# antonilo/unsupervised_detection

Measured on AMD Instinct MI355X. Metric: frame-pairs/sec per adversarial step, DAVIS 480p batch4, 1/2/4/8 GPU, higher is better.
Workload: dtype f32

## Files before the change

### include/udet.h

```cpp
#ifndef UDET_H
#define UDET_H
#include <stddef.h>
#ifdef __cplusplus
extern "C" {
#endif

#define UDET_OK 0
#define UDET_ERR_SHAPE (-1)
#define UDET_ERR_ALIGN (-2)
#define UDET_ERR_HIP (-3)
#define UDET_ERR_UNSUPPORTED (-4)
#define UDET_ERR_ARG (-5)
#define UDET_ERR_OVERFLOW (-6)

#define UDET_ACT_NONE 0
#define UDET_ACT_LEAKY 1
#define UDET_ACT_ELU 2

int udet_version(void);
const char* udet_last_error(void);


int udet_warp(const float* image, const float* flow, float flow_scale, float* out, int n, int h, int w, int c,
              void* stream);
// ... 108 lines not shown
                        int radius, float* q, void* workspace, size_t workspace_bytes, void* stream);

size_t udet_post_propagate_workspace_bytes(int total_frames, int n_seq);
int udet_post_propagate_sequences(const float* masks, const float* flow_prev, const float* flow_next, int n_seq, const int* seq_first,
                                  const int* seq_len, int total_frames, int h, int w, float w_s, float w_r, float* avg_f, float* avg_b,
                                  void* workspace, size_t workspace_bytes, void* stream);
int udet_post_select_unary(const float* pred, const float* avg_f, const float* avg_b, const float* gt, int n, int hw, int* choice,
                           double* scores, float* soft, float* unary, void* stream);

#define UDET_SOFT_SCORE_GEOM 16
size_t udet_post_soft_score_workspace_bytes(int n, int ns, int nc, int h, int w);
int udet_post_soft_score_batch(const float* masks, int n, int ns, int nc, int h, int w, const int* geom, const int* coef, double san_t,
                               double* pred_mask, void* workspace, size_t workspace_bytes, void* stream);

#define UDET_HISTOGRAM_BUCKETS 1551
size_t udet_flow_to_image_workspace_bytes(int n);
int udet_flow_to_image(const float* flow, const float* mask, const double* stats8, float threshold, int n, int h, int w,
                       unsigned char* rgb, void* workspace, size_t workspace_bytes, void* stream);
int udet_overlay_mask(const float* image, const float* mask, const double* stats8, float threshold, int n, int h, int w,
                      unsigned char* out, int oh, int ow, void* stream);
int udet_histogram_limits(double* limits, int n);
size_t udet_grad_histogram_workspace_bytes(int nseg);
int udet_grad_histogram(const float* g, const long long* seg_offsets, int nseg, double* stats, unsigned* counts, void* workspace,
                        size_t workspace_bytes, void* stream);

#define UDET_OVERLAY_MAX_EDGE 8
int udet_overlay_native_ragged(const unsigned char* image_rgb, const unsigned char* mask, int n, const long long* offsets,
                               const int* hw, int max_h, int max_w, size_t total_pixels, float alpha, float beta,
                               unsigned mask_rgb, int edge, unsigned edge_rgb, unsigned char* out_rgb, void* stream);

size_t udet_conv2d_workspace_bytes(int n, int h, int w, int cin, int cout, int kh, int kw, int upsample2x);
int udet_conv2d(const float* x, const float* w_hwio, const float* bias, float* y, int n, int h, int w, int cin, int cout,
                int kh, int kw, int stride, int dilation, int upsample2x, int act, float alpha, void* workspace,
                size_t workspace_bytes, void* stream);
int udet_conv2d_backward_data(const float* dy, const float* y_saved, const float* w_hwio, float* dx, int n, int h, int w,
                              int cin, int cout, int kh, int kw, int stride, int dilation, int act, float alpha,
                              void* workspace, size_t workspace_bytes, void* stream);
int udet_conv2d_backward_filter(const float* x, const float* dy, const float* y_saved, float* dw_hwio, float* dbias, int n,
                                int h, int w, int cin, int cout, int kh, int kw, int stride, int dilation, int upsample2x,
                                int act, float alpha, void* workspace, size_t workspace_bytes, void* stream);
int udet_conv2d_transpose4x4s2(const float* x, const float* w_hwoi, const float* bias, float* y, int n, int h, int w,
                               int cin, int cout, void* workspace, size_t workspace_bytes, void* stream);


size_t udet_stage_workspace_bytes(int n);
int udet_flow_normalize(const float* flow, float* out, int n, int h, int w, void* workspace, size_t workspace_bytes, void* stream);
int udet_charbonnier_loss(const float* gt_flows, const float* pred_flows, const float* masks, int mask_channels, int n, int h, int w,
                          float cbn, float* out, void* workspace, size_t workspace_bytes, void* stream);
int udet_losses_forward(const float* flow, const float* mask, const float* pred3, int b, int h, int w, float cbn, float epsilon,
                        float* losses8, float* coef, void* workspace, size_t workspace_bytes, void* stream);
int udet_losses_backward(const float* flow, const float* mask, const float* pred3, const float* coef, int which, int b, int h, int w,
                         float cbn, float* dpred, float* dmask, void* stream);
int udet_clip_or_noise(float* g, size_t n, float clip, const float* flag2, unsigned long long seed, long step, void* stream);
int udet_adam_step(float* w, const float* g, float* m, float* v, size_t n, float lr, float beta1, float beta2, float eps, long t,
                   void* stream);

typedef struct udet_plan udet_plan;
typedef struct {
  int batch;
  int in_h, in_w;
  int img_h, img_w;
  float flow_normalizer;
  float cbn;
  float epsilon;
  float lr, beta1, beta2, adam_eps;
  float clip;
  unsigned long long noise_seed;
  int conv_fp16;
} udet_config;

int udet_plan_create(const udet_config* cfg, udet_plan** out);
void udet_plan_destroy(udet_plan* plan);
size_t udet_workspace_bytes(const udet_plan* plan);
int udet_plan_init(udet_plan* plan, void* workspace, void* stream);

int udet_param_count(int net);
size_t udet_param_total(int net);
int udet_param_info(int net, int index, const char** name, int* rank, int* shape4, size_t* offset_floats);
int udet_buffer_count(const udet_plan* plan);
int udet_buffer_info(const udet_plan* plan, int index, const char** name, size_t* offset_bytes, int* dims_nhw_ld);

int udet_pack_pwc(udet_plan* plan, const float* w_pwc, void* workspace, void* stream);
int udet_pack_trainable(udet_plan* plan, const float* w_gen, const float* w_rec, void* workspace, void* stream);

int udet_pwc_forward(udet_plan* plan, const float* img1, const float* img2, void* workspace, void* stream);
int udet_forward(udet_plan* plan, const float* img1, const float* img2, int ncalls, void* workspace, void* stream);
int udet_prefetch_flow(udet_plan* plan, const float* img1, const float* img2, void* workspace, void* stream);
int udet_forward_prefetched(udet_plan* plan, int ncalls, void* workspace, void* stream);
int udet_prefetch_consume(udet_plan* plan, void* workspace, void* stream);
int udet_forward_from_flow(udet_plan* plan, int ncalls, void* workspace, void* stream);
int udet_generator_forward(udet_plan* plan, void* workspace, void* stream);
int udet_generator_layers(udet_plan* plan, void* workspace, void* stream);
int udet_recover_forward(udet_plan* plan, int n, void* workspace, void* stream);
int udet_backward(udet_plan* plan, int which, const float* w_gen, const float* w_rec, float* g_gen, float* g_rec,
                  void* workspace, void* stream);
int udet_stream_wait_grads(udet_plan* plan, int net, void* stream);
int udet_generator_backward(udet_plan* plan, const float* w_gen, float* g_gen, void* workspace, void* stream);
int udet_recover_backward(udet_plan* plan, const float* w_rec, float* g_rec, void* workspace, void* stream);
int udet_grad_absmean(udet_plan* plan, int net, const float* g, float* out2, void* workspace, void* stream);
int udet_apply(udet_plan* plan, int net, float* w, float* g, float* m, float* v, void* workspace, void* stream);
long udet_fp16_overflow_count(udet_plan* plan);
long udet_get_adam_step(const udet_plan* plan);
void udet_set_adam_step(udet_plan* plan, long t);
int udet_train_step(udet_plan* plan, int which, const float* img1, const float* img2, float* w_gen, float* w_rec,
                    float* g_gen, float* g_rec, float* m_gen, float* v_gen, float* m_rec, float* v_rec, void* workspace,
                    void* stream);

int udet_autotune(udet_plan* plan, const float* w_gen, const float* w_rec, float* g_gen, float* g_rec, void* workspace,
                  void* stream);
int udet_tuned_shapes(void);
int udet_tune_save(const char* path);
int udet_tune_load(const char* path);
int udet_tune_rejected(void);
int udet_profile_begin(udet_plan* plan);
int udet_profile_end(udet_plan* plan, double* out, int ncat, void* stream);

int udet_plan_set_concurrent(udet_plan* plan, int on);

int udet_plan_lane_queues(udet_plan* plan, void* stream, int* queue);
int udet_plan_pin_lanes(udet_plan* plan, void* stream, void* const* side_streams, int n);

#define UDET_INSTANCE_WRAP 252
#define UDET_INSTANCE_UNASSIGNED 255
size_t udet_track_instance_maps_workspace_bytes(size_t total_pixels, int n, int k);
int udet_track_instance_maps_ragged(const int* labels, int n, const long long* offsets, const int* hw, int max_h, int max_w,
                                    size_t total_pixels, const long long* dets, const long long* counts, int k, const int* ids,
                                    const unsigned char* gt, unsigned char* map, long long* row_gt, long long* frame_stats,
                                    void* workspace, size_t workspace_bytes, void* stream);

int udet_overlay_instances_ragged(const unsigned char* image_rgb, const unsigned char* map, int n, const long long* offsets, const int* hw,
                                  int max_h, int max_w, size_t total_pixels, float alpha, float beta, const unsigned* palette,
                                  int palette_size, unsigned other_rgb, int edge, unsigned char* out_rgb, void* stream);

size_t udet_follow_tracks_workspace_bytes(size_t total_pixels, int n, int k);
int udet_follow_tracks_ragged(const int* labels, int n, const long long* offsets, const int* hw, int max_h, int max_w,
                              long long total_pixels, const long long* dets, const long long* counts, int k,
                              const unsigned long long* keep, const unsigned char* gt, unsigned char* selected, long long* stats,
                              void* workspace, size_t workspace_bytes, void* stream);

#define UDET_MAX_OBJECTS 32
size_t udet_track_object_overlaps_workspace_bytes(size_t total_pixels, int n, int k);
int udet_track_object_overlaps_ragged(const int* labels, int n, const long long* offsets, const int* hw, int max_h, int max_w,
                                      size_t total_pixels, const long long* dets, const long long* counts, int k,
                                      const unsigned char* objects, int num_objects, long long* row_obj, long long* obj_area,
                                      long long* frame_stats, void* workspace, size_t workspace_bytes, void* stream);

#ifdef __cplusplus
}
#endif
#endif
```

### include/udet_debug.h

```cpp
#ifndef UDET_DEBUG_H
#define UDET_DEBUG_H
#include <stddef.h>
#ifdef __cplusplus
extern "C" {
#endif
void udet_debug_force_conv(int bm, int bn, int ks);
void udet_debug_conv_fp16(int on);
void udet_debug_conv_fp16_grad_scale(float s);
void udet_debug_force_wgrad(int nsplit, int dma);
int udet_debug_last_wgrad(void);
int udet_debug_last_wgrad_reduce(void);
int udet_debug_conv2d_backward_filter_ex(const float* x, int ldx, int x_coff, const float* dy, int ldy, int y_coff, const float* y_saved, int act,
                                         float alpha, const float* w, const float* b, const float* gamma, float bn_c, float* dw, float* db,
                                         float* dgamma, float* dbeta, int n, int h, int wd, int cin, int cout, int k, int stride, int dilation,
                                         int up, void* workspace, size_t workspace_bytes, void* stream);
void udet_debug_upb_min_pixels(long v);
void udet_debug_set_tuning(int on);
void udet_debug_force_pair(int on);
int udet_debug_last_pair(void);
int udet_debug_conv2d_pair(const float* xa, const float* xb, const float* wa, const float* wb, const float* ba, const float* bb, float* ya, float* yb,
                           int na, int nb, int h, int w, int cin, int cout, int k, int stride, int dilation, int act, float alpha, void* workspace,
                           size_t workspace_bytes, void* stream);
#define UDET_DEBUG_UPCONV_WSETS_OFFSET 6400
size_t udet_debug_upconv_lowres_workspace_bytes(int ldx, int cin, int cout);
int udet_debug_upconv_lowres_fwd(const float* x, int ldx, const float* w, const float* bias, int act, float alpha, float* y, int ldy, int y_coff,
                                 float* xhat, int n, int h, int wd, int cin, int cout, int split, void* workspace, size_t workspace_bytes,
                                 void* stream);
int udet_debug_upconv_lowres_bwd(const float* dy, int ldy, int y_coff, const float* w, float* dx, int ldx, float* dxhat, int n, int h, int wd,
                                 int cin, int cout, void* workspace, size_t workspace_bytes, void* stream);
int udet_debug_upconv_tables(int h, int w, int backward, int* nseg, int* seg, int* seg_tap, int* taps, int taps_cap, int* ntaps);
int udet_debug_max_segs(void);
int udet_debug_launch_resize_bilinear_fwd(const float* x, int ldx, int x_coff, int n, int h, int w, float* y, int ldy, int y_coff, int oh, int ow,
                                          int c, float mul, float div, void* stream);
int udet_debug_launch_resize_bilinear_bwd(const float* dy, int ldy, int y_coff, int n, int oh, int ow, float* dx, int ldx, int x_coff, int h, int w,
                                          int c, int accumulate, void* stream);
int udet_debug_launch_share_samples(float* buf, long p, int ld, int coff, int c, int copies, void* stream);
int udet_debug_launch_fold_samples(float* buf, long p, int ld, int coff, int c, int copies, void* stream);
int udet_debug_launch_emit_du(const float* d, const float* a, float* u, long p, int ld, int coff, int c, int act, float alpha, void* stream);
int udet_debug_launch_pack_pwc_input(const float* i1, const float* i2, float* x8, long p, void* stream);
size_t udet_debug_gen_input_workspace_bytes(int b);
int udet_debug_launch_gen_input(const float* img, const float* f, float* gin, int b, long hw, void* workspace, size_t workspace_bytes, void* stream);
int udet_debug_launch_mask_rec_inputs(const float* logits, const float* f, float* mask, float* fin, long p, int ncalls, void* stream);
int udet_debug_launch_pack_imgin(const float* img, float* imgin, long p, int ncalls, void* stream);
int udet_debug_launch_mask_bwd(const float* dmask, const float* dfin, const float* f, const float* mask, float* dlogits, long p, void* stream);
typedef struct udet_debug_conv_ex {
  int form;
  int n, h, wd, cin, cout, k, stride, dilation, up;
  int kc, k_split, k_gap;
  const float* x;
  int ldx, x_coff;
  const float* xa;
  int xact;
  float xalpha;
  const float* w;
  const float* bias;
  int act;
  float alpha;
  float* y;
  int ldy, y_coff;
  const float* res;
  int ldres, res_coff;
  float* y2;
  int ldy2, y2_coff;
  int accumulate;
  float* uo;
  int ldu, u_coff;
  const float* ua;
  int ldua, ua_coff, uact;
  float ualpha;
  int u_c0, u_c1;
  int pack_job;
} udet_debug_conv_ex;
size_t udet_debug_conv2d_ex_workspace_bytes(const udet_debug_conv_ex* args);
int udet_debug_conv2d_ex(const udet_debug_conv_ex* args, void* workspace, size_t workspace_bytes, void* stream);
size_t udet_debug_conv2d_pair_ex_workspace_bytes(const udet_debug_conv_ex* a, const udet_debug_conv_ex* b);
int udet_debug_conv2d_pair_ex(const udet_debug_conv_ex* a, const udet_debug_conv_ex* b, void* workspace, size_t workspace_bytes, void* stream);
int udet_debug_last_conv(void);
#ifdef __cplusplus
}
#endif
#endif
```

### unsupervised_detection_amd/_devel.py

```python
from __future__ import annotations

import ctypes
import os

from ._ffi import check as _check, lib as _lib

_PATH = os.path.join(os.path.dirname(os.path.abspath(__file__)), "libudet_debug.so")
if not os.path.exists(_PATH):
    raise RuntimeError(f"{_PATH} is missing: build it with `make -C unsupervised_detection_amd/csrc`")
dbg = ctypes.CDLL(_PATH, mode=ctypes.RTLD_GLOBAL)
dbg.udet_debug_force_conv.restype = None
dbg.udet_debug_force_conv.argtypes = [ctypes.c_int, ctypes.c_int, ctypes.c_int]
dbg.udet_debug_last_conv.restype = ctypes.c_int
dbg.udet_debug_last_conv.argtypes = []
dbg.udet_debug_conv_fp16.restype = None
dbg.udet_debug_conv_fp16.argtypes = [ctypes.c_int]
dbg.udet_debug_conv_fp16_grad_scale.restype = None
dbg.udet_debug_conv_fp16_grad_scale.argtypes = [ctypes.c_float]
dbg.udet_debug_force_wgrad.restype = None
dbg.udet_debug_force_wgrad.argtypes = [ctypes.c_int, ctypes.c_int]
dbg.udet_debug_upb_min_pixels.restype = None
dbg.udet_debug_upb_min_pixels.argtypes = [ctypes.c_long]
dbg.udet_debug_set_tuning.restype = None
dbg.udet_debug_set_tuning.argtypes = [ctypes.c_int]
dbg.udet_debug_last_wgrad.restype = ctypes.c_int
dbg.udet_debug_last_wgrad.argtypes = []
dbg.udet_debug_force_pair.restype = None
dbg.udet_debug_force_pair.argtypes = [ctypes.c_int]
dbg.udet_debug_last_pair.restype = ctypes.c_int
dbg.udet_debug_last_pair.argtypes = []
dbg.udet_debug_conv2d_pair.restype = ctypes.c_int
dbg.udet_debug_conv2d_pair.argtypes = [ctypes.c_void_p] * 8 + [ctypes.c_int] * 10 + [ctypes.c_float, ctypes.c_void_p, ctypes.c_size_t, ctypes.c_void_p]
dbg.udet_debug_last_wgrad_reduce.restype = ctypes.c_int
dbg.udet_debug_last_wgrad_reduce.argtypes = []
_p, _i, _f = ctypes.c_void_p, ctypes.c_int, ctypes.c_float
dbg.udet_debug_conv2d_backward_filter_ex.restype = ctypes.c_int
dbg.udet_debug_conv2d_backward_filter_ex.argtypes = ([_p, _i, _i, _p, _i, _i, _p, _i, _f, _p, _p, _p, _f, _p, _p, _p, _p] + [_i] * 9
                                                     + [_p, ctypes.c_size_t, _p])
UPCONV_WSETS_OFFSET = 6400
dbg.udet_debug_upconv_lowres_workspace_bytes.restype = ctypes.c_size_t
dbg.udet_debug_upconv_lowres_workspace_bytes.argtypes = [_i, _i, _i]
dbg.udet_debug_upconv_lowres_fwd.restype = ctypes.c_int
dbg.udet_debug_upconv_lowres_fwd.argtypes = [_p, _i, _p, _p, _i, _f, _p, _i, _i, _p] + [_i] * 6 + [_p, ctypes.c_size_t, _p]
dbg.udet_debug_upconv_lowres_bwd.restype = ctypes.c_int
dbg.udet_debug_upconv_lowres_bwd.argtypes = [_p, _i, _i, _p, _p, _i, _p] + [_i] * 5 + [_p, ctypes.c_size_t, _p]
dbg.udet_debug_upconv_tables.restype = ctypes.c_int
dbg.udet_debug_upconv_tables.argtypes = [_i, _i, _i] + [_p] * 4 + [_i, _p]
dbg.udet_debug_max_segs.restype = ctypes.c_int
dbg.udet_debug_max_segs.argtypes = []
_l = ctypes.c_long
for _name, _args in (("resize_bilinear_fwd", [_p, _i, _i, _i, _i, _i, _p, _i, _i, _i, _i, _i, _f, _f, _p]),
                     ("resize_bilinear_bwd", [_p, _i, _i, _i, _i, _i, _p, _i, _i, _i, _i, _i, _i, _p]),
                     ("share_samples", [_p, _l, _i, _i, _i, _i, _p]),
                     ("fold_samples", [_p, _l, _i, _i, _i, _i, _p]),
                     ("emit_du", [_p, _p, _p, _l, _i, _i, _i, _i, _f, _p]),
                     ("pack_pwc_input", [_p, _p, _p, _l, _p]),
                     ("gen_input", [_p, _p, _p, _i, _l, _p, ctypes.c_size_t, _p]),
                     ("mask_rec_inputs", [_p, _p, _p, _p, _l, _i, _p]),
                     ("pack_imgin", [_p, _p, _l, _i, _p]),
                     ("mask_bwd", [_p, _p, _p, _p, _p, _l, _p])):
    _fn = getattr(dbg, "udet_debug_launch_" + _name)
    _fn.restype = ctypes.c_int
    _fn.argtypes = _args
dbg.udet_debug_gen_input_workspace_bytes.restype = ctypes.c_size_t
dbg.udet_debug_gen_input_workspace_bytes.argtypes = [_i]


class ConvEx(ctypes.Structure):
    _fields_ = ([("form", _i)] + [(k, _i) for k in ("n", "h", "wd", "cin", "cout", "k", "stride", "dilation", "up", "kc", "k_split", "k_gap")]
                + [("x", _p), ("ldx", _i), ("x_coff", _i), ("xa", _p), ("xact", _i), ("xalpha", _f), ("w", _p), ("bias", _p), ("act", _i),
                   ("alpha", _f), ("y", _p), ("ldy", _i), ("y_coff", _i), ("res", _p), ("ldres", _i), ("res_coff", _i), ("y2", _p),
                   ("ldy2", _i), ("y2_coff", _i), ("accumulate", _i), ("uo", _p), ("ldu", _i), ("u_coff", _i), ("ua", _p), ("ldua", _i),
                   ("ua_coff", _i), ("uact", _i), ("ualpha", _f), ("u_c0", _i), ("u_c1", _i), ("pack_job", _i)])


dbg.udet_debug_conv2d_ex_workspace_bytes.restype = ctypes.c_size_t
dbg.udet_debug_conv2d_ex_workspace_bytes.argtypes = [ctypes.POINTER(ConvEx)]
dbg.udet_debug_conv2d_ex.restype = ctypes.c_int
dbg.udet_debug_conv2d_ex.argtypes = [ctypes.POINTER(ConvEx), _p, ctypes.c_size_t, _p]


dbg.udet_debug_conv2d_pair_ex_workspace_bytes.restype = ctypes.c_size_t
dbg.udet_debug_conv2d_pair_ex_workspace_bytes.argtypes = [ctypes.POINTER(ConvEx), ctypes.POINTER(ConvEx)]
dbg.udet_debug_conv2d_pair_ex.restype = ctypes.c_int
dbg.udet_debug_conv2d_pair_ex.argtypes = [ctypes.POINTER(ConvEx), ctypes.POINTER(ConvEx), _p, ctypes.c_size_t, _p]


def _workspace_and_stream(workspace, stream):
    if workspace is None or isinstance(workspace, tuple):
        ptr, nbytes = workspace or (None, 0)
    else:
        ptr, nbytes = workspace.data_ptr(), workspace.numel() * workspace.element_size()
    if stream is None:
        import torch
        stream = torch.cuda.current_stream().cuda_stream if torch.cuda.is_available() else None
    return ptr, nbytes, stream


def conv2d_pair_ex(a_fields, b_fields, workspace=None, stream=None):
    a, b = (None if f is None else ctypes.byref(conv_ex_args(**f)) for f in (a_fields, b_fields))
    _check(dbg.udet_debug_conv2d_pair_ex(a, b, *_workspace_and_stream(workspace, stream)))


def conv2d_pair_ex_workspace_bytes(a_fields, b_fields) -> int:
    a, b = (None if f is None else ctypes.byref(conv_ex_args(**f)) for f in (a_fields, b_fields))
    return int(dbg.udet_debug_conv2d_pair_ex_workspace_bytes(a, b))


def conv2d_ex(workspace=None, stream=None, **fields):
    a = conv_ex_args(**fields)
    _check(dbg.udet_debug_conv2d_ex(ctypes.byref(a), *_workspace_and_stream(workspace, stream)))


def conv_ex_args(**fields) -> ConvEx:
    a = ConvEx()
    for k, v in fields.items():
        if isinstance(v, tuple):
            v = v[0].data_ptr() + v[1] * v[0].element_size()
        elif hasattr(v, "data_ptr"):
            v = v.data_ptr()
        setattr(a, k, v)
    return a


def conv2d_ex_workspace_bytes(**fields) -> int:
    return int(dbg.udet_debug_conv2d_ex_workspace_bytes(ctypes.byref(conv_ex_args(**fields))))


def launch(name: str, *args):
    import torch
    raw = [a.data_ptr() if isinstance(a, torch.Tensor) else a for a in args]
    _check(getattr(dbg, "udet_debug_launch_" + name)(*raw, torch.cuda.current_stream().cuda_stream))


def upconv_tables(h: int, w: int, backward: bool):
    cap = 1024
    nseg, ntaps = ctypes.c_int(0), ctypes.c_int(0)
    seg, seg_tap, taps = (ctypes.c_int * 64)(), (ctypes.c_int * 17)(), (ctypes.c_int * (3 * cap))()
    st = dbg.udet_debug_upconv_tables(h, w, 1 if backward else 0, ctypes.addressof(nseg), ctypes.addressof(seg), ctypes.addressof(seg_tap),
                                      ctypes.addressof(taps), cap, ctypes.addressof(ntaps))
    _check(st)
    ns, nt = nseg.value, ntaps.value
    return dict(nseg=ns, seg=[tuple(seg[4 * s:4 * s + 4]) for s in range(ns)], seg_tap=list(seg_tap[:ns + 1]),
                taps=[tuple(taps[3 * t:3 * t + 3]) for t in range(nt)])
```

### unsupervised_detection_amd/csrc/api_plan.hip

```cpp
#include <stdlib.h>
#include <string.h>

#include "conv_host.h"
#include "elementwise.h"
#include "plan.h"

using namespace udet;

struct udet_plan {
  Plan* p;
};

extern "C" {

int udet_plan_create(const udet_config* c, udet_plan** out) {
  if (!c || !out) { set_error("plan_create: null argument"); return UDET_ERR_ARG; }
  Config k;
  k.batch = c->batch; k.in_h = c->in_h; k.in_w = c->in_w; k.img_h = c->img_h; k.img_w = c->img_w;
  k.flow_normalizer = c->flow_normalizer; k.cbn = c->cbn; k.epsilon = c->epsilon;
  k.lr = c->lr; k.beta1 = c->beta1; k.beta2 = c->beta2; k.adam_eps = c->adam_eps; k.clip = c->clip;
  k.noise_seed = c->noise_seed;
  k.conv_fp16 = c->conv_fp16 ? 1 : 0;
  Plan* P = plan_build(k);
  if (!P) return UDET_ERR_SHAPE;
  *out = new udet_plan{P};
  return UDET_OK;
}
void udet_plan_destroy(udet_plan* h) {
  if (h) { delete h->p; delete h; }
}
size_t udet_workspace_bytes(const udet_plan* h) { return h->p->arena_floats * sizeof(float); }
int udet_plan_init(udet_plan* h, void* ws, void* stream) { return plan_init_workspace(h->p, (float*)ws, (hipStream_t)stream); }

int udet_param_count(int net) { return (net < 0 || net > 2) ? 0 : (int)net_params(net).p.size(); }
size_t udet_param_total(int net) { return (net < 0 || net > 2) ? 0 : net_params(net).total; }
int udet_param_info(int net, int i, const char** name, int* rank, int* shape, size_t* offset) {
  if (net < 0 || net > 2 || i < 0 || i >= (int)net_params(net).p.size()) { set_error("param_info: out of range"); return UDET_ERR_ARG; }
  const ParamDesc& d = net_params(net).p[i];
  *name = d.name.c_str(); *rank = d.rank; *offset = d.offset;
  for (int k = 0; k < 4; ++k) shape[k] = d.shape[k];
  return UDET_OK;
}
int udet_buffer_count(const udet_plan* h) { return (int)h->p->bufs.size(); }
int udet_buffer_info(const udet_plan* h, int i, const char** name, size_t* offset_bytes, int* dims) {
  if (i < 0 || i >= (int)h->p->bufs.size()) { set_error("buffer_info: out of range"); return UDET_ERR_ARG; }
  const Buf& b = h->p->bufs[i];
  *name = b.name.c_str(); *offset_bytes = b.off * sizeof(float);
  dims[0] = b.n; dims[1] = b.h; dims[2] = b.w; dims[3] = b.ld;
  return UDET_OK;
}
int udet_plan_set_concurrent(udet_plan* h, int on) {
  if (!h) { set_error("plan_set_concurrent: null plan"); return UDET_ERR_ARG; }
  if (on)
    if (h->p->cand.empty()) { set_error("plan_set_concurrent: the plan has no side streams"); return UDET_ERR_UNSUPPORTED; }
  h->p->concurrent = on != 0;
  return UDET_OK;
}
int udet_plan_lane_queues(udet_plan* h, void* stream, int* queue) {
  if (!h || !queue) { set_error("plan_lane_queues: null argument"); return UDET_ERR_ARG; }
  return plan_lane_queues(h->p, (hipStream_t)stream, queue);
}
int udet_plan_pin_lanes(udet_plan* h, void* stream, void* const* side_streams, int n) {
  if (!h || (n > 0 && !side_streams)) { set_error("plan_pin_lanes: null argument"); return UDET_ERR_ARG; }
  return plan_pin_lanes(h->p, (hipStream_t)stream, reinterpret_cast<hipStream_t const*>(side_streams), n);
}
long udet_fp16_overflow_count(udet_plan* h) {
  if (!h) return 0;
  (void)plan_check_overflow(h->p, true);
  return h->p->ovf_skipped;
}
long udet_get_adam_step(const udet_plan* h) {
  plan_settle_adam_step(h->p);
  return h->p->adam_t;
}
void udet_set_adam_step(udet_plan* h, long t) {
  plan_settle_adam_step(h->p);
  h->p->adam_t = t;
}

int udet_pack_pwc(udet_plan* h, const float* w_pwc, void* ws, void* stream) {
  return plan_pack_pwc(h->p, w_pwc, (float*)ws, (hipStream_t)stream);
}
int udet_pack_trainable(udet_plan* h, const float* w_gen, const float* w_rec, void* ws, void* stream) {
  return plan_pack_trainable(h->p, w_gen, w_rec, (float*)ws, (hipStream_t)stream);
}
int udet_pwc_forward(udet_plan* h, const float* img1, const float* img2, void* ws, void* stream) {
  return plan_pwc_forward(h->p, img1, img2, (float*)ws, (hipStream_t)stream);
}
int udet_forward_from_flow(udet_plan* h, int ncalls, void* ws, void* stream) {
  UDET_TRY(plan_check_overflow(h->p, false));
  if (ncalls < 0 || ncalls > 3) { set_error("forward: ncalls must be 0..3"); return UDET_ERR_ARG; }
  return plan_forward(h->p, nullptr, nullptr, ncalls, (float*)ws, (hipStream_t)stream);
}
int udet_generator_forward(udet_plan* h, void* ws, void* stream) {
  UDET_TRY(plan_generator_forward(h->p, (float*)ws, (hipStream_t)stream));
  return plan_recover_forward(h->p, 0, (float*)ws, (hipStream_t)stream);
}
int udet_generator_layers(udet_plan* h, void* ws, void* stream) {
  h->p->ev_next = 0;
  UDET_TRY(plan_generator_layers(h->p, (float*)ws, (hipStream_t)stream));
  return plan_recover_forward(h->p, 0, (float*)ws, (hipStream_t)stream);
}
int udet_recover_forward(udet_plan* h, int n, void* ws, void* stream) {
  if (n < 1 || n > 3) { set_error("recover_forward: n must be 1..3 (multiples of the plan batch)"); return UDET_ERR_ARG; }
  return plan_recover_forward(h->p, n, (float*)ws, (hipStream_t)stream, true);
}
int udet_forward(udet_plan* h, const float* img1, const float* img2, int ncalls, void* ws, void* stream) {
  UDET_TRY(plan_check_overflow(h->p, false));
  if (ncalls < 0 || ncalls > 3) { set_error("forward: ncalls must be 0..3"); return UDET_ERR_ARG; }
  if (!img1 || !img2) { set_error("forward: null image pointer"); return UDET_ERR_ARG; }
  return plan_forward(h->p, img1, img2, ncalls, (float*)ws, (hipStream_t)stream);
}
int udet_prefetch_flow(udet_plan* h, const float* img1, const float* img2, void* ws, void* stream) {
  if (!img1 || !img2) { set_error("prefetch_flow: null image pointer"); return UDET_ERR_ARG; }
  return plan_prefetch(h->p, img1, img2, (float*)ws, (hipStream_t)stream);
}
int udet_prefetch_consume(udet_plan* h, void* ws, void* stream) {
  return plan_prefetch_consume(h->p, (float*)ws, (hipStream_t)stream);
}
int udet_forward_prefetched(udet_plan* h, int ncalls, void* ws, void* stream) {
  UDET_TRY(plan_check_overflow(h->p, false));
  if (ncalls < 0 || ncalls > 3) { set_error("forward: ncalls must be 0..3"); return UDET_ERR_ARG; }
  return plan_forward(h->p, nullptr, nullptr, ncalls, (float*)ws, (hipStream_t)stream, true);
}
int udet_backward(udet_plan* h, int which, const float* w_gen, const float* w_rec, float* g_gen, float* g_rec, void* ws,
                  void* stream) {
  UDET_TRY(plan_check_overflow(h->p, false));
  if (which < 1 || which > 3) { set_error("backward: which must be 1 (generator), 2 (recover) or 3 (both)"); return UDET_ERR_ARG; }
  return plan_backward(h->p, which, w_gen, w_rec, g_gen, g_rec, (float*)ws, (hipStream_t)stream);
}
int udet_apply(udet_plan* h, int net, float* w, float* g, float* m, float* v, void* ws, void* stream) {
  return plan_apply(h->p, net, w, g, m, v, (float*)ws, (hipStream_t)stream);
}
int udet_train_step(udet_plan* h, int which, const float* img1, const float* img2, float* w_gen, float* w_rec, float* g_gen,
                    float* g_rec, float* m_gen, float* v_gen, float* m_rec, float* v_rec, void* ws, void* stream) {
  UDET_TRY(udet_pack_trainable(h, w_gen, w_rec, ws, stream));
  UDET_TRY(udet_forward(h, img1, img2, 3, ws, stream));
  UDET_TRY(udet_backward(h, which, w_gen, w_rec, g_gen, g_rec, ws, stream));
  if (which & 1) UDET_TRY(udet_apply(h, NET_GEN, w_gen, g_gen, m_gen, v_gen, ws, stream));
  if (which & 2) UDET_TRY(udet_apply(h, NET_REC, w_rec, g_rec, m_rec, v_rec, ws, stream));
  return UDET_OK;
}

int udet_autotune(udet_plan* h, const float* w_gen, const float* w_rec, float* g_gen, float* g_rec, void* ws_, void* stream) {
  Plan* P = h->p;
  float* ws = (float*)ws_;
  hipStream_t s = (hipStream_t)stream;
  if (!P->pwc_packed) { set_error("autotune: pack the PWC-Net and trainable weights first"); return UDET_ERR_ARG; }
  const size_t lo = P->packed_floats, hi = P->small_off;
  UDET_TRY(launch_fill_uniform(ws + lo, (long)(hi - lo), 0x5eedull, -0.5f, 0.5f, s));
  const size_t img_floats = (size_t)P->cfg.batch * P->cfg.in_h * P->cfg.in_w * 3;
  if (P->wgrad_floats < 2 * img_floats) { set_error("autotune: workspace too small for the probe images"); return UDET_ERR_ARG; }
  const float* img1 = ws + P->wgrad_off[0];
  const float* img2 = img1 + img_floats;
  const bool was_concurrent = P->concurrent;
  P->concurrent = false;
  conv_set_tuning(1);
  wgrad_set_tuning(1);
  int rc = udet_forward(h, img1, img2, 3, ws_, stream);
  if (rc == UDET_OK) rc = udet_backward(h, 3, w_gen, w_rec, g_gen, g_rec, ws_, stream);
  conv_set_tuning(0);
  wgrad_set_tuning(0);
  P->concurrent = was_concurrent;
  UDET_HIP(hipMemsetAsync(ws + lo, 0, (hi - lo) * sizeof(float), s));
  UDET_HIP(hipStreamSynchronize(s));
  return rc;
}
int udet_tuned_shapes(void) { return tuned_shapes(); }
int udet_tune_save(const char* path) {
  FILE* f = path ? fopen(path, "w") : nullptr;
  if (!f) { set_error("tune_save: cannot open %s", path ? path : "(null)"); return UDET_ERR_ARG; }
  fprintf(f, "udet-tune 2 abi %d\n", UDET_TUNE_ABI);
  tune_dump(f);
  fclose(f);
  return UDET_OK;
}
int udet_tune_load(const char* path) {
  FILE* f = path ? fopen(path, "r") : nullptr;
  if (!f) { set_error("tune_load: cannot open %s", path ? path : "(null)"); return UDET_ERR_ARG; }
  char line[256];
  int n = 0, ver = 0, abi = -1;
  if (!fgets(line, sizeof(line), f) || sscanf(line, "udet-tune %d abi %d", &ver, &abi) != 2 || ver != 2 || abi != UDET_TUNE_ABI) {
    fclose(f);
    set_error("tune_load: %s is not a udet-tune 2 file of this build (abi %d)", path, UDET_TUNE_ABI);
    return UDET_ERR_ARG;
  }
  while (fgets(line, sizeof(line), f)) n += tune_put_line(line) ? 1 : 0;
  fclose(f);
  return n;
}

int udet_profile_begin(udet_plan* h) {
  for (auto* r : h->p->prof) delete r;
  h->p->prof.clear();
  h->p->profiling = true;
  return UDET_OK;
}
int udet_profile_end(udet_plan* h, double* out, int ncat, void* stream) {
  Plan* P = h->p;
  P->profiling = false;
  g_launch_sink = nullptr;
  UDET_HIP(hipStreamSynchronize((hipStream_t)stream));
  for (int i = 0; i < ncat * 5; ++i) out[i] = 0.0;
  FILE* dump = nullptr;
  if (const char* path = getenv("UDET_PROF_DUMP")) dump = fopen(path, "a");
  for (auto* r : P->prof) {
    float wall = 0.f;
    (void)hipEventElapsedTime(&wall, r->a, r->b);
    double kern = 0.0;
    std::string each;
    for (int k = 0; k < r->sink.n; ++k) {
      float ms = 0.f;
      if (hipEventElapsedTime(&ms, r->kev[2 * k], r->kev[2 * k + 1]) == hipSuccess) kern += ms;
      char buf[32];
      snprintf(buf, sizeof(buf), "%s%.1f", k ? "+" : "", ms * 1e3f);
      each += buf;
      (void)hipEventDestroy(r->kev[2 * k]);
      (void)hipEventDestroy(r->kev[2 * k + 1]);
    }
    if (r->sink.n == 0) kern = wall;
    if (dump)
      fprintf(dump, "%d,%s,%.4f,%.4f,%.4f,%.4f,%d,%s,%.4f\n", r->cat, r->name.c_str(), kern, r->flops * 1e-9, r->bytes * 1e-6, wall, r->sink.n,
              each.c_str(), r->flops * r->mfma_scale * 1e-9);
    if (r->cat < ncat) {
      out[r->cat * 5 + 0] += 1.0;
      out[r->cat * 5 + 1] += kern;
      out[r->cat * 5 + 2] += r->flops;
      out[r->cat * 5 + 3] += r->bytes;
      out[r->cat * 5 + 4] += wall;
    }
    (void)hipEventDestroy(r->a);
    (void)hipEventDestroy(r->b);
    delete r;
  }
  if (dump) fclose(dump);
  P->prof.clear();
  return UDET_OK;
}

int udet_generator_backward(udet_plan* h, const float* w_gen, float* g_gen, void* ws, void* stream) {
  if (!w_gen || !g_gen) { set_error("generator_backward: null argument"); return UDET_ERR_ARG; }
  return plan_backward(h->p, 1, w_gen, nullptr, g_gen, nullptr, (float*)ws, (hipStream_t)stream);
}
int udet_recover_backward(udet_plan* h, const float* w_rec, float* g_rec, void* ws, void* stream) {
  if (!w_rec || !g_rec) { set_error("recover_backward: null argument"); return UDET_ERR_ARG; }
  return plan_backward(h->p, 2, nullptr, w_rec, nullptr, g_rec, (float*)ws, (hipStream_t)stream);
}
int udet_grad_absmean(udet_plan* h, int net, const float* g, float* out2, void* ws_, void* stream) {
  if ((net != NET_GEN && net != NET_REC) || !g || !out2) { set_error("grad_absmean: net must be 1 or 2, g / out2 non-null"); return UDET_ERR_ARG; }
  Plan* P = h->p;
  float* ws = (float*)ws_;
  const NetParams& np = net_params(net);
  const long* tab = reinterpret_cast<const long*>(ws + P->seg_off[net]);
  return launch_grad_absmean(g, tab, tab + np.p.size(), (int)np.p.size(), ws + P->small_off + 2048, 1e-5f, out2, (hipStream_t)stream);
}
int udet_stream_wait_grads(udet_plan* h, int net, void* stream) {
  if (net != NET_GEN && net != NET_REC) { set_error("stream_wait_grads: net must be 1 or 2"); return UDET_ERR_ARG; }
  if (!h->p->grad_ev[net]) { set_error("stream_wait_grads: no udet_backward has produced that gradient yet"); return UDET_ERR_ARG; }
  UDET_HIP(hipStreamWaitEvent((hipStream_t)stream, h->p->grad_ev[net], 0));
  return UDET_OK;
}
int udet_tune_rejected(void) { return conv_tune_rejected(); }

}
```

### unsupervised_detection_amd/csrc/common.h

```cpp
#pragma once
#include <hip/hip_runtime.h>
#include <hip/hip_ext.h>
#include <stdint.h>
#include <stdio.h>
#include <string>

#include "../../include/udet.h"

namespace udet {

void set_error(const char* fmt, ...);
int hip_fail(hipError_t e, const char* what);
#define UDET_HIP(x)                                   \
  do {                                                \
    hipError_t _e = (x);                              \
    if (_e != hipSuccess) return udet::hip_fail(_e, #x); \
  } while (0)
#define UDET_TRY(x)            \
  do {                         \
    int _s = (x);              \
    if (_s != 0) return _s;    \
  } while (0)

struct LaunchSink {
// ... 60 lines not shown
  for (int b = 0; b < nwg; ++b) {
    const int l = xcd_tile_order(b, nwg);
    if (l < 0 || l >= nwg || ((seen >> l) & 1)) return false;
    seen |= 1ull << l;
  }
  return true;
}
static_assert(xcd_tile_order_permutes(1) && xcd_tile_order_permutes(7) && xcd_tile_order_permutes(8), "xcd_tile_order");
static_assert(xcd_tile_order_permutes(9) && xcd_tile_order_permutes(13) && xcd_tile_order_permutes(64), "xcd_tile_order");
static_assert(xcd_tile_order(1, 13) == 2 && xcd_tile_order(8, 13) == 1 && xcd_tile_order(5, 13) == 10, "xcd 0..4 of 13 hold two tiles, 5..7 one");

struct ConvSeg {
  int oy, ox;
  int h, w;
  int prow0;
  FastDiv fd_hw, fd_w;
};
#define UDET_MAX_SEGS 16

struct ConvParams {
  const float* x;
  int ldx, x_coff;
  int N, H, W;
  int up_shift;
  const float* xa;
  int xact;
  float xalpha;
  const float* wp;
  int Kc, ldw;
  const float* bias;
  float* y;
  int ldy, y_coff, Cout;
  int OH, OW;
  int OHq, OWq;
  int osy, osx, ooy, oox;
  int isy, isx;
  int ntaps;
  ConvTap taps[UDET_MAX_TAPS];
  int ncls;
  int cls_tap[5];
  int nseg;
  ConvSeg seg[UDET_MAX_SEGS];
  int seg_tap[UDET_MAX_SEGS + 1];
  const ConvTap* tap_tab;
  int Mall;
  FastDiv fd_ohw, fd_ow;
  int kfast;
  const float* zero16;
  int act;
  float alpha;
  const float* res;
  int ldres, res_coff;
  float* y2;
  int ldy2, y2_coff;
  int accumulate;
  float* uo;
  int ldu, u_coff;
  const float* ua;
  int ldua, ua_coff, uact;
  float ualpha;
  int u_c0, u_c1;
  int ksplit;
  float* partial;
  size_t partial_cap;
  int ldp;
  int fold;
  int* tickets;
  int tail_full, tail_ks, tail_prow0;
  int f16;
  float f16_xscale;
  const float* wino_u;
  int wino_np;
  int kreal;
};
#define UDET_MAX_TICKETS 4096

int launch_conv(ConvParams& p, hipStream_t stream);
int launch_conv_pair(ConvParams& a, ConvParams& b, hipStream_t stream);
int launch_tap_gather(const ConvParams& g, const float* z, int ldz, hipStream_t stream);

struct PackJob {
  long src_off, dst_off, gamma_off, beta_off;
  long total;
  int T, R, C, Kc, ldw, k_split, k_gap, mode;
};

struct WgradParams {
  const float* x;
  int ldx, x_coff;
  int N, H, W, up_shift;
  int Cin;
  const float* dy;
  const float* ya;
  int ldy, y_coff, Cout;
  int yact;
  float yalpha;
  int OH, OW, isy, isx;
  int ycls, OHf, OWf;
  int ntaps;
  ConvTap taps[UDET_MAX_TAPS];
  float* dw;
  float* db;
  float* partial;
  size_t partial_floats;
  const float* zero16;
  int swapped, oCin, oCout, bias_m;
  int Cin4, Mpad;
  float* pbias;
  FastDiv fd_ohw, fd_ow;
  const float* w;
  const float* b;
  const float* gamma;
  float* dgamma;
  float* dbeta;
  float bn_c;
  int f16;
  float f16_yscale;
};
int launch_wgrad_T(WgradParams& p, int T, hipStream_t stream);
int launch_wgrad_up_T(const WgradParams& q, int H, int W, hipStream_t stream);
int launch_bn_finalize(float* dw, int T, int Cin, int Cout, const float* w, const float* b, const float* gamma, float bn_c, float* pd,
                       float* db, float* dgamma, float* dbeta, hipStream_t stream);
int launch_wgrad_up_combine(const float* deff, float* dw, int Cin, int Cout, hipStream_t stream);
size_t wgrad_partial_floats_needed(int T, int Cin, int Cout);

}
```

### unsupervised_detection_amd/csrc/conv_host.h

```cpp
#pragma once
#include "common.h"
namespace udet {
void same_pad(int in, int k, int s, int d, int* before, int* out);
void conv_setup_fwd(ConvParams& p, int N, int H, int W, int kh, int kw, int s, int d);
int conv_dgrad_classes(int s, int H, int W);
void conv_force_config(int bm, int bn, int ks);
bool conv_thin_n_ok(const ConvParams& p);
bool conv_thin_k_ok(const ConvParams& p);
int launch_conv_thin_n(const ConvParams& p, hipStream_t stream);
int launch_conv_thin_k(const ConvParams& p, hipStream_t stream);
bool conv_wino_geometry(const ConvParams& p, int* dil, int widx_at[9]);
bool conv_wino_ok(const ConvParams& p);
bool conv_wino_variant_ok(const ConvParams& p, int variant);
int conv_wino_np(int cout);
size_t conv_wino_floats(int Kc, int cout);
long conv_wino_workgroups(const ConvParams& p, int variant);
int conv_wino_max_ksplit(const ConvParams& p, int variant);
int launch_conv_wino(ConvParams& p, int variant, int ks, hipStream_t stream);
int launch_splitk_second_pass(const ConvParams& p, hipStream_t stream);
int launch_wino_pack(const float* src, float* dst, int R, int C, int Kc, int np, int k_split, int k_gap, int transposed, hipStream_t stream);
int launch_wino_from_packed(const ConvParams& p, float* dst, int np, hipStream_t stream);
void conv_debug_f16(int on);
int conv_debug_f16_on();
void conv_debug_f16_grad_scale(float s);
float conv_debug_f16_grad_scale_now();
int conv_last_config();
void conv_set_tuning(int on);
int tuned_shapes();
void tune_dump(FILE* f);
bool tune_put_line(const char* line);
int conv_tune_rejected();
void wgrad_set_tuning(int on);
bool wgrad_wino_ok(const WgradParams& p);
int wgrad_wino_slices(const WgradParams& p, int wanted);
int launch_wgrad_wino(const WgradParams& q, int slices, int ldn, hipStream_t stream);
int wgrad_last_config();
enum { WGRAD_RED_FUSED_BN = 1 << 26, WGRAD_RED_SEPARATE_BN = 1 << 27, WGRAD_RED_SWAPPED = 1 << 28, WGRAD_RED_CLASSES = 1 << 29 };
int wgrad_last_reduce();
void setup_up_fwd(ConvParams& p, int N, int H, int W);
void setup_up_dgrad(ConvParams& p, int N, int H, int W);
void wgrad_force(int nsplit, int dma);
void conv_force_pair(int on);
int conv_last_pair();
#define UDET_TUNE_ABI 6
bool conv_setup_dgrad(ConvParams& p, int cls, int N, int H, int W, int kh, int kw, int s, int d);
int launch_pack_weights(const float* src, float* dst, int T, int R, int C, int Kc, int ldw, int k_split, int k_gap,
                        int mode, const float* scale, hipStream_t stream);
int launch_pack_taps_into_n(const float* src, float* dst, int T, int R, int C, int Kc, int ldz, int k_split, int k_gap,
                            int transposed, hipStream_t stream);
int launch_pack_jobs(const PackJob* jobs_dev, int njobs, const float* wsrc, float* ws, float bn_c, hipStream_t stream);
int launch_fold_bn(const float* b, const float* gamma, const float* beta, float c, float* scale, float* bias_f, int n,
                   hipStream_t stream);
int launch_copy_channels(const float* src, int lds, int s_coff, float* dst, int ldd, int d_coff, long P, int C, float mul,
                         float add, hipStream_t stream);
int launch_warp(const float* img, const float* flow, int ldf, int f_coff, float flow_scale, float* out, int N, int H,
                int W, int C, int* dbg_idx, float* dbg_alpha, hipStream_t stream);
int launch_cost_volume(const float* c1, const float* wr, float* out, int ldo, int o_coff, int N, int H, int W, int C,
                       hipStream_t stream);
int launch_warp_cost_volume(const float* c1, const float* c2, const float* flow, int ldf, int f_coff, float flow_scale, float* out,
                            int ldo, int corr_coff, int c1_coff, float* warped_dbg, int N, int H, int W, int C, hipStream_t stream);
inline int round_up(int v, int m) { return (v + m - 1) / m * m; }
}
```

### unsupervised_detection_amd/csrc/conv_host.hip

```cpp
#include <string.h>

#include <stdint.h>

#include "common.h"
#include "conv_host.h"
#include "wino_pack.h"

namespace udet {

void same_pad(int in, int k, int s, int d, int* before, int* out) {
  const int o = (in + s - 1) / s;
  int total = (o - 1) * s + (k - 1) * d + 1 - in;
  if (total < 0) total = 0;
  *before = total / 2;
  *out = o;
}

static inline int floordiv2(int v) { return v >= 0 ? v / 2 : -((-v + 1) / 2); }

static void push_tap(ConvParams& p, int dy, int dx, int widx) {
  const int ymax = (p.OHq - 1) * p.isy + dy, xmax = (p.OWq - 1) * p.isx + dx;
  if (dy >= p.H || ymax < 0 || dx >= p.W || xmax < 0) return;
  p.taps[p.ntaps].dy = dy;
  p.taps[p.ntaps].dx = dx;
  p.taps[p.ntaps].widx = widx;
  ++p.ntaps;
}

void conv_setup_fwd(ConvParams& p, int N, int H, int W, int kh, int kw, int s, int d) {
  int pt, pl, oh, ow;
  same_pad(H, kh, s, d, &pt, &oh);
  same_pad(W, kw, s, d, &pl, &ow);
  p.N = N; p.H = H; p.W = W;
  p.OH = oh; p.OW = ow; p.OHq = oh; p.OWq = ow;
  p.osy = p.osx = 1; p.ooy = p.oox = 0;
  p.isy = p.isx = s;
  p.ntaps = 0;
  for (int ky = 0; ky < kh; ++ky)
    for (int kx = 0; kx < kw; ++kx) push_tap(p, ky * d - pt, kx * d - pl, ky * kw + kx);
}

int conv_dgrad_classes(int s, int H, int W) { return s == 1 ? 1 : ((H % 2 == 0 && W % 2 == 0) ? 1 : s * s); }

bool conv_setup_dgrad(ConvParams& p, int cls, int N, int H, int W, int kh, int kw, int s, int d) {
  int pt, pl, ohf, owf;
  same_pad(H, kh, s, d, &pt, &ohf);
  same_pad(W, kw, s, d, &pl, &owf);
  p.N = N; p.H = ohf; p.W = owf;
  p.OH = H; p.OW = W;
  p.isy = p.isx = 1;
  p.ntaps = 0;
  p.ncls = 1;
  if (s == 1) {
    p.OHq = H; p.OWq = W; p.osy = p.osx = 1; p.ooy = p.oox = 0;
    for (int ky = 0; ky < kh; ++ky)
      for (int kx = 0; kx < kw; ++kx) push_tap(p, pt - ky * d, pl - kx * d, ky * kw + kx);
    return p.ntaps > 0;
  }
  const bool merged = (H % 2 == 0 && W % 2 == 0);
  p.osy = p.osx = s;
  const int c_lo = merged ? 0 : cls, c_hi = merged ? 4 : cls + 1;
  for (int c = c_lo; c < c_hi; ++c) {
    const int py = c / s, px = c % s;
    p.ooy = py; p.oox = px;
    p.OHq = (H - py + s - 1) / s;
    p.OWq = (W - px + s - 1) / s;
    if (merged) p.cls_tap[c] = p.ntaps;
    if (p.OHq <= 0 || p.OWq <= 0) {
      if (!merged) return false;
      continue;
    }
    for (int ky = 0; ky < kh; ++ky) {
      const int vy = py + pt - ky * d;
      if (((vy % 2) + 2) % 2) continue;
      for (int kx = 0; kx < kw; ++kx) {
        const int vx = px + pl - kx * d;
        if (((vx % 2) + 2) % 2) continue;
        push_tap(p, floordiv2(vy), floordiv2(vx), ky * kw + kx);
      }
    }
  }
  if (merged) {
    p.ncls = 4;
    p.cls_tap[4] = p.ntaps;
    p.ooy = p.oox = 0;
    p.OHq = H / 2; p.OWq = W / 2;
  }
  return true;
}

__global__ __launch_bounds__(256) void pack_weights_kernel(const float* __restrict__ src, float* __restrict__ dst, int T,
                                                           int R, int C, int Kc, int ldw, int k_split, int k_gap,
                                                           int mode, const float* __restrict__ scale) {
  const long total = (long)T * Kc * ldw;
  for (long e = (long)blockIdx.x * 256 + threadIdx.x; e < total; e += (long)gridDim.x * 256) {
    const int n = (int)(e % ldw);
    const int k = (int)((e / ldw) % Kc);
    const int t = (int)(e / ((long)ldw * Kc));
    float v = 0.f;
    int ks = k;
    if (k >= k_split) ks = (k < k_split + k_gap) ? -1 : k - k_gap;
    const int r = mode == 0 ? ks : n, c = mode == 0 ? n : ks;
    if (r >= 0 && r < R && c >= 0 && c < C) {
      v = src[((long)t * R + r) * C + c];
      if (scale) v *= scale[c];
    }
    dst[e] = v;
  }
}

int launch_pack_weights(const float* src, float* dst, int T, int R, int C, int Kc, int ldw, int k_split, int k_gap,
                        int mode, const float* scale, hipStream_t stream) {
  const long total = (long)T * Kc * ldw;
  int nb = (int)((total + 255) / 256);
  if (nb > 2048) nb = 2048;
  UDET_LAUNCH(pack_weights_kernel, dim3(nb), dim3(256), 0, stream, src, dst, T, R, C, Kc, ldw, k_split, k_gap,
                     mode, scale);
  UDET_HIP(hipGetLastError());
  return UDET_OK;
}

__constant__ float UPB_MERGE[2][3][3][4] = {
    {{{.5f, 0.f, 0.f, 0.f}, {.5f, 1.f, .5f, 0.f}, {0.f, 0.f, .5f, 1.f}},
     {{.5f, 0.f, 0.f, 0.f}, {.5f, 1.f, 1.f, 0.f}, {0.f, 0.f, 0.f, 0.f}},
     {{0.f, 0.f, 0.f, 0.f}, {0.f, 0.f, .5f, 0.f}, {0.f, 0.f, -.5f, -1.f}}},
    {{{1.f, .5f, 0.f, 0.f}, {0.f, .5f, 1.f, .5f}, {0.f, 0.f, 0.f, .5f}},
     {{1.f, 1.f, 0.f, 0.f}, {0.f, 0.f, 0.f, 0.f}, {0.f, 0.f, 0.f, 0.f}},
     {{0.f, .5f, 0.f, 0.f}, {0.f, -.5f, -1.f, -.5f}, {0.f, 0.f, 0.f, -.5f}}}};

__global__ __launch_bounds__(256) void pack_jobs_kernel(const PackJob* __restrict__ jobs, const float* __restrict__ wsrc,
                                                        float* __restrict__ ws, float bn_c) {
  const PackJob j = jobs[blockIdx.y];
  const float* src = wsrc + j.src_off;
  float* dst = ws + j.dst_off;
  const float* gamma = j.gamma_off >= 0 ? wsrc + j.gamma_off : nullptr;
  if (j.mode == 2) {
    for (long e = (long)blockIdx.x * 256 + threadIdx.x; e < j.total; e += (long)gridDim.x * 256)
      dst[e] = gamma ? src[e] * (gamma[e] * bn_c) + wsrc[j.beta_off + e] : src[e];
    return;
  }
  if (j.mode == 9 || j.mode == 10) {
    const int rv = (int)(j.beta_off / 3), cv = (int)(j.beta_off % 3);
    for (long e = (long)blockIdx.x * 256 + threadIdx.x; e < j.total; e += (long)gridDim.x * 256) {
      const int n = (int)(e % j.ldw), k = (int)(e / j.ldw);
      int ks = k;
      if (k >= j.k_split) ks = (k < j.k_split + j.k_gap) ? -1 : k - j.k_gap;
      const int ci = j.mode == 9 ? ks : n, co = j.mode == 9 ? n : ks;
      const bool real = ci >= 0 && ci < j.R && co >= 0 && co < j.C;
      float w[4][4];
#pragma unroll
      for (int kk = 0; kk < 4; ++kk)
#pragma unroll
        for (int ll = 0; ll < 4; ++ll) w[kk][ll] = real ? src[((long)(kk * 4 + ll) * j.R + ci) * j.C + co] : 0.f;
      const long plane = (long)j.Kc * j.ldw;
#pragma unroll
      for (int py = 0; py < 2; ++py) {
        float t1[3][4];
#pragma unroll
        for (int a = 0; a < 3; ++a)
#pragma unroll
          for (int ll = 0; ll < 4; ++ll) {
            float v = 0.f;
#pragma unroll
            for (int kk = 0; kk < 4; ++kk) v += UPB_MERGE[py][rv][a][kk] * w[kk][ll];
            t1[a][ll] = v;
          }
#pragma unroll
        for (int px = 0; px < 2; ++px)
#pragma unroll
          for (int a = 0; a < 3; ++a)
#pragma unroll
            for (int bb = 0; bb < 3; ++bb) {
              float v = 0.f;
#pragma unroll
              for (int ll = 0; ll < 4; ++ll) v += UPB_MERGE[px][cv][bb][ll] * t1[a][ll];
              dst[(long)((py * 2 + px) * 9 + a * 3 + bb) * plane + e] = v;
            }
      }
    }
    return;
  }
  if (j.mode == 7 || j.mode == 8) {
    for (long e = (long)blockIdx.x * 256 + threadIdx.x; e < j.total; e += (long)gridDim.x * 256) wino_pack_item(j, src, gamma, bn_c, dst, e);
    return;
  }
  for (long e = (long)blockIdx.x * 256 + threadIdx.x; e < j.total; e += (long)gridDim.x * 256) {
    const int n = (int)(e % j.ldw);
    const int k = (int)((e / j.ldw) % j.Kc);
    int t = (int)(e / ((long)j.ldw * j.Kc));
    float v = 0.f;
    int ks = k;
    if (k >= j.k_split) ks = (k < j.k_split + j.k_gap) ? -1 : k - j.k_gap;
    int r = j.mode == 0 ? ks : n, c = j.mode == 0 ? n : ks;
    if (j.mode == 3 || j.mode == 4) {
      t = n / j.C;
      c = n - t * j.C;
      r = ks;
      if (t >= j.T) r = -1;
    }
    if (j.mode >= 5) {
      const int cls = t >> 2, ty = (t >> 1) & 1, tx = t & 1, py = cls >> 1, px = cls & 1;
      const int y0 = py == 0 ? (ty == 0 ? 0 : 1) : (ty == 0 ? 0 : 2), y1 = py == 0 ? (ty == 0 ? 0 : 2) : (ty == 0 ? 1 : 2);
      const int x0 = px == 0 ? (tx == 0 ? 0 : 1) : (tx == 0 ? 0 : 2), x1 = px == 0 ? (tx == 0 ? 0 : 2) : (tx == 0 ? 1 : 2);
      const int ci = j.mode == 5 ? ks : n, co = j.mode == 5 ? n : ks;
      if (ci >= 0 && ci < j.R && co >= 0 && co < j.C) {
        for (int ky = y0; ky <= y1; ++ky)
          for (int kx = x0; kx <= x1; ++kx) v += src[((long)(ky * 3 + kx) * j.R + ci) * j.C + co];
        if (gamma) v *= gamma[co] * bn_c;
      }
      dst[e] = v;
      continue;
    }
    if (r >= 0 && r < j.R && c >= 0 && c < j.C) {
      v = j.mode == 4 ? src[((long)t * j.C + c) * j.R + r] : src[((long)t * j.R + r) * j.C + c];
      if (gamma) v *= gamma[c] * bn_c;
    }
    dst[e] = v;
  }
}
int launch_pack_jobs(const PackJob* jobs_dev, int njobs, const float* wsrc, float* ws, float bn_c, hipStream_t stream) {
  if (njobs < 1) return UDET_OK;
  UDET_LAUNCH(pack_jobs_kernel, dim3(48, njobs), dim3(256), 0, stream, jobs_dev, wsrc, ws, bn_c);
  UDET_HIP(hipGetLastError());
  return UDET_OK;
}

__global__ __launch_bounds__(256) void pack_job_kernel(const PackJob j, const float* __restrict__ wsrc, float* __restrict__ ws) {
  const float* src = wsrc + j.src_off;
  float* dst = ws + j.dst_off;
  for (long e = (long)blockIdx.x * 256 + threadIdx.x; e < j.total; e += (long)gridDim.x * 256) {
    const int n = (int)(e % j.ldw);
    const int k = (int)((e / j.ldw) % j.Kc);
    int ks = k;
    if (k >= j.k_split) ks = (k < j.k_split + j.k_gap) ? -1 : k - j.k_gap;
    const int t = n / j.C, c = n - t * j.C;
    float v = 0.f;
    if (ks >= 0 && ks < j.R && t < j.T) v = j.mode == 4 ? src[((long)t * j.C + c) * j.R + ks] : src[((long)t * j.R + ks) * j.C + c];
    dst[e] = v;
  }
}
int launch_pack_taps_into_n(const float* src, float* dst, int T, int R, int C, int Kc, int ldz, int k_split, int k_gap,
                            int transposed, hipStream_t stream) {
  PackJob j;
  memset(&j, 0, sizeof(j));
  j.T = T; j.R = R; j.C = C; j.Kc = Kc; j.ldw = ldz; j.k_split = k_split; j.k_gap = k_gap;
  j.mode = transposed ? 4 : 3; j.total = (long)Kc * ldz; j.gamma_off = -1;
  int nb = (int)((j.total + 255) / 256);
  if (nb > 1024) nb = 1024;
  UDET_LAUNCH(pack_job_kernel, dim3(nb), dim3(256), 0, stream, j, src, dst);
  UDET_HIP(hipGetLastError());
  return UDET_OK;
}

__global__ __launch_bounds__(256) void tap_gather_kernel(const ConvParams g, const float* __restrict__ z, int ldz) {
  const long total = (long)g.N * g.OH * g.OW * g.Cout;
  for (long e = (long)blockIdx.x * 256 + threadIdx.x; e < total; e += (long)gridDim.x * 256) {
    const int co = (int)(e % g.Cout);
    const long pix = e / g.Cout;
    const int ox = (int)(pix % g.OW), oy = (int)((pix / g.OW) % g.OH), n = (int)(pix / ((long)g.OW * g.OH));
    int cls = 0, qy = oy, qx = ox;
    if (g.ncls > 1) {
      cls = (oy & 1) * 2 + (ox & 1);
      qy = oy >> 1;
      qx = ox >> 1;
    }
    float v = g.bias ? g.bias[co] : 0.f;
    const int t1 = g.cls_tap[cls + 1];
    for (int t0 = g.cls_tap[cls]; t0 < t1; t0 += 8) {
      float a[8];
#pragma unroll
      for (int u = 0; u < 8; ++u) {
        const int t = t0 + u < t1 ? t0 + u : t1 - 1;
        const int iy = qy + g.taps[t].dy, ix = qx + g.taps[t].dx;
        const bool ok = t0 + u < t1 && (unsigned)iy < (unsigned)g.H && (unsigned)ix < (unsigned)g.W;
        a[u] = ok ? z[((size_t)(n * g.H + iy) * g.W + ix) * ldz + g.taps[t].widx * g.Cout + co] : 0.f;
      }
#pragma unroll
      for (int u = 0; u < 8; ++u) v += a[u];
    }
    g.y[(size_t)pix * g.ldy + g.y_coff + co] = v;
  }
}
__global__ __launch_bounds__(256) void tap_gather2_kernel(const ConvParams g, const float* __restrict__ z, int ldz) {
  const long total = (long)g.N * g.OH * g.OW;
  for (long pix = (long)blockIdx.x * 256 + threadIdx.x; pix < total; pix += (long)gridDim.x * 256) {
    const int ox = (int)(pix % g.OW), oy = (int)((pix / g.OW) % g.OH), n = (int)(pix / ((long)g.OW * g.OH));
    int cls = 0, qy = oy, qx = ox;
    if (g.ncls > 1) {
      cls = (oy & 1) * 2 + (ox & 1);
      qy = oy >> 1;
      qx = ox >> 1;
    }
    float2 v = g.bias ? make_float2(g.bias[0], g.bias[1]) : make_float2(0.f, 0.f);
    const int t1 = g.cls_tap[cls + 1];
    for (int t0 = g.cls_tap[cls]; t0 < t1; t0 += 8) {
      float2 a[8];
#pragma unroll
      for (int u = 0; u < 8; ++u) {
        const int t = t0 + u < t1 ? t0 + u : t1 - 1;
        const int iy = qy + g.taps[t].dy, ix = qx + g.taps[t].dx;
        const bool ok = t0 + u < t1 && (unsigned)iy < (unsigned)g.H && (unsigned)ix < (unsigned)g.W;
        a[u] = ok ? *reinterpret_cast<const float2*>(z + ((size_t)(n * g.H + iy) * g.W + ix) * ldz + g.taps[t].widx * 2)
                  : make_float2(0.f, 0.f);
      }
#pragma unroll
      for (int u = 0; u < 8; ++u) {
        v.x += a[u].x;
// ... 65 lines not shown
```

### unsupervised_detection_amd/csrc/devel/api_debug.hip

```cpp
#include <string.h>

#include <vector>

#include "../../../include/udet_debug.h"
#include "../conv_host.h"
#include "../elementwise.h"
#include "../plan_run.h"

using namespace udet;

extern "C" {
int udet_debug_last_conv(void) { return conv_last_config(); }
void udet_debug_force_conv(int bm, int bn, int ks) { conv_force_config(bm, bn, ks); }
void udet_debug_conv_fp16(int on) { conv_debug_f16(on); }
void udet_debug_conv_fp16_grad_scale(float s) { conv_debug_f16_grad_scale(s); }
void udet_debug_force_wgrad(int nsplit, int dma) { wgrad_force(nsplit, dma); }
int udet_debug_last_wgrad(void) { return wgrad_last_config(); }
int udet_debug_last_wgrad_reduce(void) { return wgrad_last_reduce(); }
int udet_debug_conv2d_backward_filter_ex(const float* x, int ldx, int x_coff, const float* dy, int ldy, int y_coff, const float* y_saved, int act,
                                         float alpha, const float* w, const float* b, const float* gamma, float bn_c, float* dw, float* db,
                                         float* dgamma, float* dbeta, int n, int h, int wd, int cin, int cout, int k, int stride, int dilation,
                                         int up, void* workspace, size_t workspace_bytes, void* stream_) {
  hipStream_t stream = (hipStream_t)stream_;
  if (!x || !dy || !dw || n < 1 || h < 1 || wd < 1 || cin < 1 || cout < 1 || k < 1 || k * k > UDET_MAX_TAPS || dilation < 1 ||
// ... 437 lines not shown
  return glue_align(who, "buf", buf, v4 ? 16 : 4);
}
}
extern "C" {
int udet_debug_launch_resize_bilinear_fwd(const float* x, int ldx, int x_coff, int n, int h, int w, float* y, int ldy, int y_coff, int oh, int ow,
                                          int c, float mul, float div, void* stream) {
  const char* who = "debug_launch_resize_bilinear_fwd";
  if (!(div != 0.f)) { set_error("%s: div must not be 0", who); return UDET_ERR_ARG; }
  UDET_TRY(glue_resize_check(who, x, ldx, x_coff, y, ldy, y_coff, n, h, w, oh, ow, c));
  return launch_resize_bilinear_fwd(x, ldx, x_coff, n, h, w, y, ldy, y_coff, oh, ow, c, mul, div, (hipStream_t)stream);
}
int udet_debug_launch_resize_bilinear_bwd(const float* dy, int ldy, int y_coff, int n, int oh, int ow, float* dx, int ldx, int x_coff, int h, int w,
                                          int c, int accumulate, void* stream) {
  const char* who = "debug_launch_resize_bilinear_bwd";
  if (accumulate != 0 && accumulate != 1) { set_error("%s: accumulate must be 0 or 1", who); return UDET_ERR_ARG; }
  UDET_TRY(glue_resize_check(who, dy, ldy, y_coff, dx, ldx, x_coff, n, oh, ow, h, w, c));
  return launch_resize_bilinear_bwd(dy, ldy, y_coff, n, oh, ow, dx, ldx, x_coff, h, w, c, accumulate, (hipStream_t)stream);
}
int udet_debug_launch_share_samples(float* buf, long p, int ld, int coff, int c, int copies, void* stream) {
  UDET_TRY(glue_share_fold_check("debug_launch_share_samples", buf, p, ld, coff, c, copies));
  return launch_share_samples(buf, p, ld, coff, c, copies, (hipStream_t)stream);
}
int udet_debug_launch_fold_samples(float* buf, long p, int ld, int coff, int c, int copies, void* stream) {
  UDET_TRY(glue_share_fold_check("debug_launch_fold_samples", buf, p, ld, coff, c, copies));
  return launch_fold_samples(buf, p, ld, coff, c, copies, (hipStream_t)stream);
}
int udet_debug_launch_emit_du(const float* d, const float* a, float* u, long p, int ld, int coff, int c, int act, float alpha, void* stream) {
  const char* who = "debug_launch_emit_du";
  if (!d || !a || !u || (act != UDET_ACT_NONE && act != UDET_ACT_LEAKY && act != UDET_ACT_ELU)) { set_error("%s: bad argument", who); return UDET_ERR_ARG; }
  UDET_TRY(glue_window(who, "d / a / u", ld, coff, c));
  UDET_TRY(glue_pixels(who, p));
  if (glue_misaligned(d, 4) || glue_misaligned(a, 4) || glue_misaligned(u, 4)) { set_error("%s: misaligned pointer", who); return UDET_ERR_ALIGN; }
  return launch_emit_du(d, a, u, p, ld, coff, c, act, alpha, (hipStream_t)stream);
}
int udet_debug_launch_pack_pwc_input(const float* i1, const float* i2, float* x8, long p, void* stream) {
  const char* who = "debug_launch_pack_pwc_input";
  if (!i1 || !i2 || !x8) { set_error("%s: bad argument", who); return UDET_ERR_ARG; }
  UDET_TRY(glue_pixels(who, 2 * p));
  if (glue_misaligned(i1, 4) || glue_misaligned(i2, 4)) { set_error("%s: misaligned image pointer", who); return UDET_ERR_ALIGN; }
  UDET_TRY(glue_align(who, "x8", x8, 16));
  return launch_pack_pwc_input(i1, i2, x8, p, (hipStream_t)stream);
}
size_t udet_debug_gen_input_workspace_bytes(int b) { return b < 1 ? 0 : flow_stats_doubles(b) * sizeof(double); }
int udet_debug_launch_gen_input(const float* img, const float* f, float* gin, int b, long hw, void* workspace, size_t workspace_bytes, void* stream) {
  const char* who = "debug_launch_gen_input";
  if (!img || !f || !gin || b < 1 || b > 65535 || !workspace || workspace_bytes < udet_debug_gen_input_workspace_bytes(b)) {
    set_error("%s: bad argument (workspace: udet_debug_gen_input_workspace_bytes)", who);
    return UDET_ERR_ARG;
  }
  if (hw < 1) { set_error("%s: pixel count must be positive", who); return UDET_ERR_ARG; }
  if (hw >= GLUE_MAX_PIXELS / b) { set_error("%s: pixel count too large", who); return UDET_ERR_SHAPE; }
  UDET_TRY(glue_align(who, "img", img, 4));
  UDET_TRY(glue_align(who, "f", f, 8));
  UDET_TRY(glue_align(who, "gin", gin, 16));
  UDET_TRY(glue_align(who, "workspace", workspace, 8));
  return launch_gen_input(img, f, reinterpret_cast<double*>(workspace), gin, b, hw, (hipStream_t)stream);
}
int udet_debug_launch_mask_rec_inputs(const float* logits, const float* f, float* mask, float* fin, long p, int ncalls, void* stream) {
  const char* who = "debug_launch_mask_rec_inputs";
  if (!logits || !f || !mask || !fin || ncalls < 0 || ncalls > 3) { set_error("%s: bad argument (ncalls 0..3)", who); return UDET_ERR_ARG; }
  UDET_TRY(glue_pixels(who, 3 * p));
  if (glue_misaligned(logits, 4) || glue_misaligned(mask, 4)) { set_error("%s: misaligned pointer", who); return UDET_ERR_ALIGN; }
  UDET_TRY(glue_align(who, "f", f, 8));
  UDET_TRY(glue_align(who, "fin", fin, 16));
  return launch_mask_rec_inputs(logits, f, mask, fin, p, ncalls, (hipStream_t)stream);
}
int udet_debug_launch_pack_imgin(const float* img, float* imgin, long p, int ncalls, void* stream) {
  const char* who = "debug_launch_pack_imgin";
  if (!img || !imgin || ncalls < 0 || ncalls > 3) { set_error("%s: bad argument (ncalls 0..3)", who); return UDET_ERR_ARG; }
  UDET_TRY(glue_pixels(who, 3 * p));
  UDET_TRY(glue_align(who, "img", img, 4));
  UDET_TRY(glue_align(who, "imgin", imgin, 16));
  return launch_pack_imgin(img, imgin, p, ncalls, (hipStream_t)stream);
}
int udet_debug_launch_mask_bwd(const float* dmask, const float* dfin, const float* f, const float* mask, float* dlogits, long p, void* stream) {
  const char* who = "debug_launch_mask_bwd";
  if (!dmask || !dfin || !f || !mask || !dlogits) { set_error("%s: bad argument", who); return UDET_ERR_ARG; }
  UDET_TRY(glue_pixels(who, 2 * p));
  if (glue_misaligned(dmask, 4) || glue_misaligned(mask, 4) || glue_misaligned(dlogits, 4)) { set_error("%s: misaligned pointer", who); return UDET_ERR_ALIGN; }
  UDET_TRY(glue_align(who, "dfin", dfin, 16));
  UDET_TRY(glue_align(who, "f", f, 8));
  return launch_mask_bwd(dmask, dfin, f, mask, dlogits, p, (hipStream_t)stream);
}

void udet_debug_set_tuning(int on) {
  conv_set_tuning(on);
  wgrad_set_tuning(on);
}
}
```

### unsupervised_detection_amd/csrc/elementwise.h

```cpp
#pragma once
#include "common.h"
namespace udet {
int launch_resize_bilinear_fwd(const float* x, int ldx, int x_coff, int N, int H, int W, float* y, int ldy, int y_coff,
                               int OH, int OW, int C, float mul, float div, hipStream_t s);
int launch_resize_bilinear_bwd(const float* dy, int ldy, int y_coff, int N, int OH, int OW, float* dx, int ldx, int x_coff,
                               int H, int W, int C, int accumulate, hipStream_t s);
int launch_upb_ring(const float* x, int ld, int N, int H, int W, float* xh, hipStream_t s);
int launch_upb_ring_fold(const float* dxh, int ld, int N, int H, int W, float* dx, hipStream_t s);
int launch_share_samples(float* buf, long P, int ld, int coff, int C, int copies, hipStream_t s);
int launch_fold_samples(float* buf, long P, int ld, int coff, int C, int copies, hipStream_t s);
int launch_emit_du(const float* d, const float* a, float* u, long P, int ld, int coff, int C, int act, float alpha, hipStream_t s);
int launch_pack_pwc_input(const float* i1, const float* i2, float* x8, long P, hipStream_t s);
int launch_gen_input(const float* img, const float* f, double* part, float* gin, int B, long HW, hipStream_t s);
size_t flow_stats_doubles(int B);
int launch_mask_rec_inputs(const float* logits, const float* f, float* mask, float* fin, long P, int ncalls, hipStream_t s);
int launch_pack_imgin(const float* img, float* imgin, long P, int ncalls, hipStream_t s);
int launch_losses(const float* f, const float* mask, const float* pred, long HW, int B, float cbn, float eps,
                  float num_pixels, float* part, float* losses, float* coef, float* sums, hipStream_t s);
size_t loss_part_floats(int B);
int launch_rec_loss_bwd(const float* f, const float* mask, const float* pred, float* dpred, long BHW, float cbn,
                        float inv_np, hipStream_t s);
int launch_gen_loss_bwd(const float* f, const float* mask, const float* pred, const float* coef, float* dpred,
                        float* dmask, long HW, int B, float cbn, hipStream_t s);
int launch_mask_bwd(const float* dmask, const float* dfin, const float* f, const float* mask, float* dlogits, long P,
                    hipStream_t s);
int launch_grad_absmean(const float* g, const long* seg_off, const long* seg_len, int nvars, float* vmean, float thresh,
                        float* out, hipStream_t s);
int launch_adam(float* w, float* g, float* m, float* v, long n, float lr_t, float b1, float b2, float eps, float clip,
                const float* flag, uint64_t seed, uint64_t step, hipStream_t s, int mode = 0, const int* skip = nullptr);
int launch_nonfinite_count(const float* g, long n, int* out, hipStream_t s);
int launch_flow_normalize(const float* f, double* part, float* out, int B, long HW, hipStream_t s);
int launch_charbonnier(const float* gt, const float* pred, const float* mask, int mc, int B, long HW, float cbn, float* part,
                       float* out, hipStream_t s);
int launch_crop_flip_resize(const void* src, int src_u8, int nearest, int N, int H, int W, int C, const int* prm, float* dst, int OH,
                            int OW, float div, float add, hipStream_t s);
int launch_crop_flip_resize_ragged(const void* src, int src_u8, int nearest, int N, int C, const long long* offsets, const int* hw,
                                   const int* prm, float* dst, int OH, int OW, float div, float add, hipStream_t s);
int launch_mask_stats(const float* pred, const float* gt, int N, int H, int W, float threshold, float gt_threshold, double* out,
                      hipStream_t s);
int launch_boundary_stats(const float* pred, const float* gt, const double* stats8, int N, int H, int W, float threshold,
                          float gt_threshold, int radius, unsigned long long* counts4, unsigned char* bmap_pred,
                          unsigned char* bmap_gt, hipStream_t s);
size_t restore_workspace_bytes(int n);
int launch_restore_masks_ragged(const float* masks, int n, int mh, int mw, const long long* offsets, const int* tab, const int* coef,
                                int max_h, int max_w, unsigned char* out, int* amax, unsigned char* binary, double threshold,
                                void* workspace, hipStream_t s);
size_t components_workspace_bytes(size_t total_pixels, int n);
int launch_select_components_ragged(const unsigned char* binary, const unsigned char* gt, int n, const long long* offsets, const int* hw,
                                    int max_h, int max_w, size_t total_pixels, int connectivity, int mode, int* labels,
                                    unsigned char* selected, long long* info, void* workspace, hipStream_t s);
size_t component_boxes_workspace_bytes(size_t total_pixels, int n);
int launch_component_boxes_ragged(const int* labels, const unsigned char* score, int n, const long long* offsets, const int* hw, int max_h,
                                  int max_w, size_t total_pixels, int min_area, int k, long long* dets, long long* counts, void* workspace,
                                  hipStream_t s);
int launch_draw_boxes_ragged(unsigned char* rgb, int n, const long long* offsets, const int* hw, const long long* dets,
                             const long long* counts, int k, int thickness, unsigned colour, hipStream_t s);
size_t link_detections_workspace_bytes(size_t total_pixels, int carry_h, int carry_w);
int launch_link_detections_ragged(const int* labels, int n, const long long* offsets, const int* hw, int max_h, int max_w,
                                  size_t total_pixels, const long long* dets, const long long* counts, int k, const int* link,
                                  const int* carry_labels, int carry_h, int carry_w, const long long* carry_dets,
                                  const long long* carry_counts, const int* carry_ids, const int* carry_next_id, int min_iou_permille,
                                  long long* inter, int* match, int* ids, int* linked, int* seq_tracks, int* next_id, const int* disp,
                                  void* workspace, hipStream_t s);
size_t link_detections_gap_workspace_bytes(size_t total_pixels, int m, int hist_h, int hist_w);
int launch_link_detections_gap_ragged(const int* labels, int n, const long long* offsets, const int* hw, int max_h, int max_w,
                                      size_t total_pixels, const long long* dets, const long long* counts, int k, const int* link,
                                      int max_gap, int m, const int* hist_labels, int hist_h, int hist_w, const long long* hist_dets,
                                      const long long* hist_counts, const int* hist_ids, int* hist_open, const int* hist_next_id,
                                      int min_iou_permille, long long* inter, int* match, int* ids, int* linked, int* seq_tracks,
                                      int* next_id, long long* gap_inter, int* back, int* prev, int* open, const int* disp,
                                      void* workspace, hipStream_t s);
int launch_draw_track_boxes_ragged(unsigned char* rgb, int n, const long long* offsets, const int* hw, const long long* dets,
                                   const long long* counts, int k, const int* ids, int thickness, const unsigned* palette,
                                   int palette_size, hipStream_t s);
int launch_fill_uniform(float* x, long n, uint64_t seed, float lo, float hi, hipStream_t s);
}
```

### unsupervised_detection_amd/csrc/elementwise.hip

```cpp
#include "common.h"
#include "elementwise.h"

namespace udet {

static inline int grid_for(long total, int cap = 4096) {
  long nb = (total + 255) / 256;
  if (nb > cap) nb = cap;
  if (nb < 1) nb = 1;
  return (int)nb;
}

template <typename T>
__device__ __forceinline__ T wave_sum(T v) {
#pragma unroll
  for (int o = 32; o > 0; o >>= 1) v += __shfl_down(v, o, 64);
  return v;
}
template <typename T>
__device__ __forceinline__ T block_sum(T v, T* sm ) {
  v = wave_sum(v);
  __syncthreads();
  if ((threadIdx.x & 63) == 0) sm[threadIdx.x >> 6] = v;
  __syncthreads();
  return sm[0] + sm[1] + sm[2] + sm[3];
// ... 376 lines not shown
  for (long p = (long)blockIdx.x * 256 + threadIdx.x; p < HW; p += (long)gridDim.x * 256) {
    const long q = (long)n * HW + p;
    const float2 v = *reinterpret_cast<const float2*>(f + q * 2);
    *reinterpret_cast<float4*>(gin + q * 8) = make_float4(img[q * 3], img[q * 3 + 1], img[q * 3 + 2], (v.x - m0) / d0);
    *reinterpret_cast<float4*>(gin + q * 8 + 4) = make_float4((v.y - m1) / d1, 0.f, 0.f, 0.f);
  }
}
int launch_gen_input(const float* img, const float* f, double* part, float* gin, int B, long HW, hipStream_t s) {
  hipLaunchKernelGGL(flow_stats_kernel, dim3(FS_BLOCKS, B), dim3(256), 0, s, f, HW, part);
  hipLaunchKernelGGL(pack_gen_input_kernel, dim3(grid_for(HW, 256), B), dim3(256), 0, s, img, f, part, gin, HW);
  UDET_HIP(hipGetLastError());
  return UDET_OK;
}
size_t flow_stats_doubles(int B) { return (size_t)B * FS_BLOCKS * 4; }
__global__ __launch_bounds__(256) void flow_normalize_kernel(const float* __restrict__ f, const double* __restrict__ part,
                                                             float* __restrict__ out, long HW) {
  __shared__ float st[4];
  const int n = blockIdx.y;
  if (threadIdx.x < 2) {
    double s = 0, q = 0;
    for (int b = 0; b < FS_BLOCKS; ++b) {
      s += part[((long)n * FS_BLOCKS + b) * 4 + threadIdx.x];
      q += part[((long)n * FS_BLOCKS + b) * 4 + 2 + threadIdx.x];
    }
    const double mean = s / (double)HW, var = q / (double)HW - mean * mean;
    st[threadIdx.x] = (float)mean;
    st[2 + threadIdx.x] = sqrtf((float)var);
  }
  __syncthreads();
  const float m0 = st[0], m1 = st[1], d0 = st[2], d1 = st[3];
  for (long p = (long)blockIdx.x * 256 + threadIdx.x; p < HW; p += (long)gridDim.x * 256) {
    const long q = (long)n * HW + p;
    const float2 v = *reinterpret_cast<const float2*>(f + q * 2);
    *reinterpret_cast<float2*>(out + q * 2) = make_float2((v.x - m0) / d0, (v.y - m1) / d1);
  }
}
int launch_flow_normalize(const float* f, double* part, float* out, int B, long HW, hipStream_t s) {
  hipLaunchKernelGGL(flow_stats_kernel, dim3(FS_BLOCKS, B), dim3(256), 0, s, f, HW, part);
  hipLaunchKernelGGL(flow_normalize_kernel, dim3(grid_for(HW, 256), B), dim3(256), 0, s, f, part, out, HW);
  UDET_HIP(hipGetLastError());
  return UDET_OK;
}

__global__ __launch_bounds__(256) void mask_rec_inputs_kernel(const float* __restrict__ logits ,
                                                              const float* __restrict__ f, float* __restrict__ mask,
                                                              float* __restrict__ fin, long P, int ncalls) {
  for (long q = (long)blockIdx.x * 256 + threadIdx.x; q < P; q += (long)gridDim.x * 256) {
    const float l0 = logits[q * 8] / 10.f, l1 = logits[q * 8 + 1] / 10.f;
    const float mx = fmaxf(l0, l1);
    const float e0 = expf(l0 - mx), e1 = expf(l1 - mx);
    const float m = e0 / (e0 + e1);
    mask[q] = m;
    const float cm = 1.f - m;
    const float2 v = *reinterpret_cast<const float2*>(f + q * 2);
    const float a0 = 1.f - m, a1 = 1.f - cm;
    if (ncalls > 0) {
      *reinterpret_cast<float4*>(fin + q * 4) = make_float4(v.x * a0, v.y * a0, 1.f, a0);
    }
    if (ncalls > 1) {
      *reinterpret_cast<float4*>(fin + (P + q) * 4) = make_float4(v.x * a1, v.y * a1, 1.f, a1);
    }
    if (ncalls > 2) {
      *reinterpret_cast<float4*>(fin + (2 * P + q) * 4) = make_float4(0.f, 0.f, 1.f, 0.f);
    }
  }
}
int launch_mask_rec_inputs(const float* logits, const float* f, float* mask, float* fin, long P, int ncalls, hipStream_t s) {
  hipLaunchKernelGGL(mask_rec_inputs_kernel, dim3(grid_for(P)), dim3(256), 0, s, logits, f, mask, fin, P, ncalls);
  UDET_HIP(hipGetLastError());
  return UDET_OK;
}
__global__ __launch_bounds__(256) void pack_imgin_kernel(const float* __restrict__ img, float* __restrict__ imgin, long P,
                                                         int ncalls) {
  for (long q = (long)blockIdx.x * 256 + threadIdx.x; q < P; q += (long)gridDim.x * 256) {
    const float4 im = make_float4(img[q * 3], img[q * 3 + 1], img[q * 3 + 2], 0.f);
    for (int k = 0; k < ncalls; ++k) *reinterpret_cast<float4*>(imgin + (k * P + q) * 4) = im;
  }
}
int launch_pack_imgin(const float* img, float* imgin, long P, int ncalls, hipStream_t s) {
  hipLaunchKernelGGL(pack_imgin_kernel, dim3(grid_for(P)), dim3(256), 0, s, img, imgin, P, ncalls);
  UDET_HIP(hipGetLastError());
  return UDET_OK;
}

__device__ __forceinline__ float charb(float e, float cbn) {
  const float s = e * e + 0.001f * 0.001f;
  return cbn == 0.5f ? sqrtf(s) : powf(s, cbn);
}
__device__ __forceinline__ float charb_d(float e, float cbn) {
  const float s = e * e + 0.001f * 0.001f;
  return cbn == 0.5f ? e / sqrtf(s) : cbn * powf(s, cbn - 1.f) * 2.f * e;
}
#define LS_BLOCKS 64
__global__ __launch_bounds__(256) void loss_sums_kernel(const float* __restrict__ f, const float* __restrict__ mask,
                                                        const float* __restrict__ pred , long HW, int B,
                                                        float cbn, float* __restrict__ part ) {
  __shared__ float sm[4];
  const int n = blockIdx.y;
  float R = 0, Rc = 0, Pp = 0, Dr = 0, Dc = 0;
  for (long p = (long)blockIdx.x * 256 + threadIdx.x; p < HW; p += (long)gridDim.x * 256) {
    const long q = (long)n * HW + p;
    const float2 fl = *reinterpret_cast<const float2*>(f + q * 2);
    const float2 a = *reinterpret_cast<const float2*>(pred + q * 2);
    const float2 b = *reinterpret_cast<const float2*>(pred + ((long)B * HW + q) * 2);
    const float2 c = *reinterpret_cast<const float2*>(pred + ((long)2 * B * HW + q) * 2);
    const float m = mask[q], cm = 1.f - m;
    const float pa = charb(fl.x - a.x, cbn) + charb(fl.y - a.y, cbn);
    const float pb = charb(fl.x - b.x, cbn) + charb(fl.y - b.y, cbn);
    const float pc = charb(fl.x - c.x, cbn) + charb(fl.y - c.y, cbn);
    R += pa * m; Rc += pb * cm; Pp += pc; Dr += pc * m; Dc += pc * cm;
  }
  R = block_sum(R, sm); Rc = block_sum(Rc, sm); Pp = block_sum(Pp, sm); Dr = block_sum(Dr, sm); Dc = block_sum(Dc, sm);
  if (threadIdx.x == 0) {
    float* o = part + ((long)n * LS_BLOCKS + blockIdx.x) * 5;
    o[0] = R; o[1] = Rc; o[2] = Pp; o[3] = Dr; o[4] = Dc;
  }
}
__global__ void loss_finish_kernel(const float* __restrict__ part, int B, float eps, float num_pixels,
                                   float* __restrict__ losses, float* __restrict__ coef, float* __restrict__ sums) {
  if (threadIdx.x != 0 || blockIdx.x != 0) return;
  float red = 0.f, redc = 0.f, rs = 0.f;
  for (int b = 0; b < B; ++b) {
    float v[5] = {0, 0, 0, 0, 0};
    for (int k = 0; k < LS_BLOCKS; ++k)
      for (int j = 0; j < 5; ++j) v[j] += part[((long)b * LS_BLOCKS + k) * 5 + j];
    const float D = v[3] + eps, Dc = v[4] + eps;
    red += 1.f - v[0] / D;
    redc += 1.f - v[1] / Dc;
    rs += v[0] + v[1] + v[2];
    coef[b * 4 + 0] = -1.f / (B * D);
    coef[b * 4 + 1] = v[0] / (B * D * D);
    coef[b * 4 + 2] = -1.f / (B * Dc);
    coef[b * 4 + 3] = v[1] / (B * Dc * Dc);
    for (int j = 0; j < 5; ++j) sums[b * 5 + j] = v[j];
    if (b == 0) { losses[4] = v[0]; losses[5] = v[1]; losses[6] = D; losses[7] = Dc; }
  }
  red /= B; redc /= B;
  losses[0] = red + redc;
  losses[1] = rs / num_pixels;
  losses[2] = red;
  losses[3] = redc;
}
int launch_losses(const float* f, const float* mask, const float* pred, long HW, int B, float cbn, float eps,
                  float num_pixels, float* part, float* losses, float* coef, float* sums, hipStream_t s) {
  hipLaunchKernelGGL(loss_sums_kernel, dim3(LS_BLOCKS, B), dim3(256), 0, s, f, mask, pred, HW, B, cbn, part);
  hipLaunchKernelGGL(loss_finish_kernel, dim3(1), dim3(64), 0, s, part, B, eps, num_pixels, losses, coef, sums);
  UDET_HIP(hipGetLastError());
  return UDET_OK;
}
size_t loss_part_floats(int B) { return (size_t)B * LS_BLOCKS * 5; }

__global__ __launch_bounds__(256) void charbonnier_sum_kernel(const float* __restrict__ gt, const float* __restrict__ pred,
                                                              const float* __restrict__ mask, int mc, long HW, float cbn,
                                                              float* __restrict__ part ) {
  __shared__ float sm[4];
  const int n = blockIdx.y;
  float acc = 0.f;
  for (long p = (long)blockIdx.x * 256 + threadIdx.x; p < HW; p += (long)gridDim.x * 256) {
    const long q = (long)n * HW + p;
    const float2 a = *reinterpret_cast<const float2*>(gt + q * 2);
    const float2 b = *reinterpret_cast<const float2*>(pred + q * 2);
    const float m0 = mask ? mask[q * mc] : 1.f, m1 = mask ? mask[q * mc + (mc - 1)] : 1.f;
    acc += charb(a.x - b.x, cbn) * m0 + charb(a.y - b.y, cbn) * m1;
  }
  acc = block_sum(acc, sm);
  if (threadIdx.x == 0) part[(long)n * LS_BLOCKS + blockIdx.x] = acc;
}
__global__ void charbonnier_finish_kernel(const float* __restrict__ part, int B, float* __restrict__ out) {
  const int b = blockIdx.x * blockDim.x + threadIdx.x;
  if (b >= B) return;
  float v = 0.f;
  for (int k = 0; k < LS_BLOCKS; ++k) v += part[(long)b * LS_BLOCKS + k];
  out[b] = v;
}
int launch_charbonnier(const float* gt, const float* pred, const float* mask, int mc, int B, long HW, float cbn, float* part,
                       float* out, hipStream_t s) {
  hipLaunchKernelGGL(charbonnier_sum_kernel, dim3(LS_BLOCKS, B), dim3(256), 0, s, gt, pred, mask, mc, HW, cbn, part);
  hipLaunchKernelGGL(charbonnier_finish_kernel, dim3((B + 63) / 64), dim3(64), 0, s, part, B, out);
  UDET_HIP(hipGetLastError());
  return UDET_OK;
}

__global__ __launch_bounds__(256) void rec_loss_bwd_kernel(const float* __restrict__ f, const float* __restrict__ mask,
                                                           const float* __restrict__ pred, float* __restrict__ dpred,
                                                           long BHW, float cbn, float inv_np) {
  for (long q = (long)blockIdx.x * 256 + threadIdx.x; q < BHW; q += (long)gridDim.x * 256) {
    const float2 fl = *reinterpret_cast<const float2*>(f + q * 2);
    const float m = mask[q], cm = 1.f - m;
    const float2 a = *reinterpret_cast<const float2*>(pred + q * 2);
    const float2 b = *reinterpret_cast<const float2*>(pred + (BHW + q) * 2);
    const float2 c = *reinterpret_cast<const float2*>(pred + (2 * BHW + q) * 2);
    *reinterpret_cast<float2*>(dpred + q * 2) = make_float2(-charb_d(fl.x - a.x, cbn) * m * inv_np, -charb_d(fl.y - a.y, cbn) * m * inv_np);
    *reinterpret_cast<float2*>(dpred + (BHW + q) * 2) = make_float2(-charb_d(fl.x - b.x, cbn) * cm * inv_np, -charb_d(fl.y - b.y, cbn) * cm * inv_np);
    *reinterpret_cast<float2*>(dpred + (2 * BHW + q) * 2) = make_float2(-charb_d(fl.x - c.x, cbn) * inv_np, -charb_d(fl.y - c.y, cbn) * inv_np);
  }
}
int launch_rec_loss_bwd(const float* f, const float* mask, const float* pred, float* dpred, long BHW, float cbn,
                        float inv_np, hipStream_t s) {
  hipLaunchKernelGGL(rec_loss_bwd_kernel, dim3(grid_for(BHW)), dim3(256), 0, s, f, mask, pred, dpred, BHW, cbn, inv_np);
  UDET_HIP(hipGetLastError());
  return UDET_OK;
}

__global__ __launch_bounds__(256) void gen_loss_bwd_kernel(const float* __restrict__ f, const float* __restrict__ mask,
                                                           const float* __restrict__ pred, const float* __restrict__ coef,
                                                           float* __restrict__ dpred, float* __restrict__ dmask, long HW,
                                                           int B, float cbn) {
  const long BHW = (long)B * HW;
  for (long q = (long)blockIdx.x * 256 + threadIdx.x; q < BHW; q += (long)gridDim.x * 256) {
    const int n = (int)(q / HW);
    const float cR = coef[n * 4], cD = coef[n * 4 + 1], cRc = coef[n * 4 + 2], cDc = coef[n * 4 + 3];
    const float2 fl = *reinterpret_cast<const float2*>(f + q * 2);
    const float m = mask[q], cm = 1.f - m;
    const float2 a = *reinterpret_cast<const float2*>(pred + q * 2);
    const float2 b = *reinterpret_cast<const float2*>(pred + (BHW + q) * 2);
    const float2 c = *reinterpret_cast<const float2*>(pred + (2 * BHW + q) * 2);
    *reinterpret_cast<float2*>(dpred + q * 2) = make_float2(-cR * charb_d(fl.x - a.x, cbn) * m, -cR * charb_d(fl.y - a.y, cbn) * m);
    *reinterpret_cast<float2*>(dpred + (BHW + q) * 2) = make_float2(-cRc * charb_d(fl.x - b.x, cbn) * cm, -cRc * charb_d(fl.y - b.y, cbn) * cm);
    const float pa = charb(fl.x - a.x, cbn) + charb(fl.y - a.y, cbn);
    const float pb = charb(fl.x - b.x, cbn) + charb(fl.y - b.y, cbn);
    const float pc = charb(fl.x - c.x, cbn) + charb(fl.y - c.y, cbn);
    dmask[q] = cR * pa + cD * pc - cRc * pb - cDc * pc;
  }
}
int launch_gen_loss_bwd(const float* f, const float* mask, const float* pred, const float* coef, float* dpred,
                        float* dmask, long HW, int B, float cbn, hipStream_t s) {
  hipLaunchKernelGGL(gen_loss_bwd_kernel, dim3(grid_for((long)B * HW)), dim3(256), 0, s, f, mask, pred, coef, dpred, dmask,
                     HW, B, cbn);
  UDET_HIP(hipGetLastError());
  return UDET_OK;
}

__global__ __launch_bounds__(256) void mask_bwd_kernel(const float* __restrict__ dmask, const float* __restrict__ dfin,
                                                       const float* __restrict__ f, const float* __restrict__ mask,
                                                       float* __restrict__ dlogits , long P) {
  for (long q = (long)blockIdx.x * 256 + threadIdx.x; q < P; q += (long)gridDim.x * 256) {
    const float4 g0 = *reinterpret_cast<const float4*>(dfin + q * 4);
    const float4 g1 = *reinterpret_cast<const float4*>(dfin + (P + q) * 4);
    const float2 fl = *reinterpret_cast<const float2*>(f + q * 2);
    float dm = dmask[q];
    dm -= g0.x * fl.x + g0.y * fl.y + g0.w;
    dm += g1.x * fl.x + g1.y * fl.y + g1.w;
    const float m = mask[q];
    const float d0 = dm * m * (1.f - m) / 10.f;
    dlogits[q * 8] = d0;
    dlogits[q * 8 + 1] = -d0;
  }
}
int launch_mask_bwd(const float* dmask, const float* dfin, const float* f, const float* mask, float* dlogits, long P,
                    hipStream_t s) {
  hipLaunchKernelGGL(mask_bwd_kernel, dim3(grid_for(P)), dim3(256), 0, s, dmask, dfin, f, mask, dlogits, P);
  UDET_HIP(hipGetLastError());
  return UDET_OK;
}

#define GA_SPLIT 8
__global__ __launch_bounds__(256) void grad_absmean_kernel(const float* __restrict__ g, const long* __restrict__ seg_off,
                                                           const long* __restrict__ seg_len, float* __restrict__ vpart) {
  __shared__ float sm[4];
  const long off = seg_off[blockIdx.x], len = seg_len[blockIdx.x];
  const long b = len * blockIdx.y / GA_SPLIT, e = len * (blockIdx.y + 1) / GA_SPLIT;
  float s0 = 0.f, s1 = 0.f, s2 = 0.f, s3 = 0.f;
  long i = b + threadIdx.x;
  for (; i + 768 < e; i += 1024) {
    s0 += fabsf(g[off + i]);
    s1 += fabsf(g[off + i + 256]);
    s2 += fabsf(g[off + i + 512]);
    s3 += fabsf(g[off + i + 768]);
  }
  for (; i < e; i += 256) s0 += fabsf(g[off + i]);
  const float s = block_sum((s0 + s1) + (s2 + s3), sm);
  if (threadIdx.x == 0) vpart[blockIdx.x * GA_SPLIT + blockIdx.y] = s;
}
__global__ void grad_flag_kernel(const float* __restrict__ vpart, const long* __restrict__ seg_len, int nvars, float thresh,
                                 float* __restrict__ out ) {
  if (threadIdx.x == 0 && blockIdx.x == 0) {
    float s = 0.f;
    for (int i = 0; i < nvars; ++i) {
      float v = 0.f;
      for (int j = 0; j < GA_SPLIT; ++j) v += vpart[i * GA_SPLIT + j];
      s += v / (float)seg_len[i];
    }
    s /= (float)nvars;
    out[0] = s;
    out[1] = s < thresh ? 1.f : 0.f;
  }
}
int launch_grad_absmean(const float* g, const long* seg_off, const long* seg_len, int nvars, float* vmean, float thresh,
                        float* out, hipStream_t s) {
  hipLaunchKernelGGL(grad_absmean_kernel, dim3(nvars, GA_SPLIT), dim3(256), 0, s, g, seg_off, seg_len, vmean);
  hipLaunchKernelGGL(grad_flag_kernel, dim3(1), dim3(64), 0, s, vmean, seg_len, nvars, thresh, out);
  UDET_HIP(hipGetLastError());
  return UDET_OK;
}

__device__ __host__ __forceinline__ float udet_uniform01(uint64_t seed, uint64_t step, uint64_t idx) {
  uint64_t z = seed * 0x9E3779B97F4A7C15ull + step * 0xBF58476D1CE4E5B9ull + idx + 0x94D049BB133111EBull;
  z = (z ^ (z >> 30)) * 0xBF58476D1CE4E5B9ull;
  z = (z ^ (z >> 27)) * 0x94D049BB133111EBull;
  z = z ^ (z >> 31);
  return (float)(z >> 40) * (1.0f / 16777216.0f);
}

__global__ __launch_bounds__(256) void adam_kernel(float* __restrict__ w, float* __restrict__ g, float* __restrict__ m,
                                                   float* __restrict__ v, long n, float lr_t, float b1, float b2, float eps,
                                                   float clip, const float* __restrict__ flag, uint64_t seed,
                                                   uint64_t step, int mode, const int* __restrict__ skip) {
  if (skip && *skip != 0) return;
  const bool noise = flag && flag[1] != 0.f;
  for (long i = (long)blockIdx.x * 256 + threadIdx.x; i < n; i += (long)gridDim.x * 256) {
    float gi = g[i];
    if (mode != 2) {
      if (noise) gi = fabsf((udet_uniform01(seed, step, (uint64_t)i) * 2.f - 1.f) * clip);
      else gi = fminf(fmaxf(gi, -clip), clip);
      g[i] = gi;
      if (mode == 1) continue;
    }
    const float mi = m[i] + (gi - m[i]) * (1.f - b1);
    const float vi = v[i] + (gi * gi - v[i]) * (1.f - b2);
    m[i] = mi;
    v[i] = vi;
    w[i] = w[i] - lr_t * mi / (sqrtf(vi) + eps);
  }
}
__global__ __launch_bounds__(256) void fill_uniform_kernel(float* __restrict__ x, long n, uint64_t seed, float lo, float hi) {
  for (long i = (long)blockIdx.x * 256 + threadIdx.x; i < n; i += (long)gridDim.x * 256)
    x[i] = lo + (hi - lo) * udet_uniform01(seed, 0, (uint64_t)i);
}
int launch_fill_uniform(float* x, long n, uint64_t seed, float lo, float hi, hipStream_t s) {
  hipLaunchKernelGGL(fill_uniform_kernel, dim3(grid_for(n, 8192)), dim3(256), 0, s, x, n, seed, lo, hi);
  UDET_HIP(hipGetLastError());
  return UDET_OK;
}
__global__ __launch_bounds__(256) void mask_stats_kernel(const float* __restrict__ pred, const float* __restrict__ gt, int H, int W,
                                                         float threshold, float gt_threshold, double* __restrict__ out) {
  __shared__ double sm[4];
  const int n = blockIdx.x;
  const long HW = (long)H * W;
  double v[8] = {0, 0, 0, 0, 0, 0, 0, 0};
  for (long q = threadIdx.x; q < HW; q += 256) {
    const int y = (int)(q / W), x = (int)(q - (long)y * W);
    const float g = gt[n * HW + q];
    const bool pr = pred[n * HW + q] > threshold, gb = g > gt_threshold;
    const int strips = (y < 2) + (y >= H - 2) + (x < 2) + (x >= W - 2);
    const double a1 = fabs((double)g - 1.0), a0 = fabs((double)g);
    if (pr) {
      v[0] += strips; v[1] += 1.0; v[4] += a1; v[7] += a0;
      if (gb) v[3] += 1.0;
    } else {
      v[5] += a0; v[6] += a1;
    }
    if (gb) v[2] += 1.0;
  }
  for (int k = 0; k < 8; ++k) {
    const double s = block_sum(v[k], sm);
    if (threadIdx.x == 0) out[(long)n * 8 + k] = s;
    __syncthreads();
  }
}
int launch_mask_stats(const float* pred, const float* gt, int N, int H, int W, float threshold, float gt_threshold, double* out,
                      hipStream_t s) {
  hipLaunchKernelGGL(mask_stats_kernel, dim3(N), dim3(256), 0, s, pred, gt, H, W, threshold, gt_threshold, out);
  UDET_HIP(hipGetLastError());
  return UDET_OK;
}
int launch_adam(float* w, float* g, float* m, float* v, long n, float lr_t, float b1, float b2, float eps, float clip,
                const float* flag, uint64_t seed, uint64_t step, hipStream_t s, int mode, const int* skip) {
  hipLaunchKernelGGL(adam_kernel, dim3(grid_for(n, 2048)), dim3(256), 0, s, w, g, m, v, n, lr_t, b1, b2, eps, clip, flag, seed,
                     step, mode, skip);
  UDET_HIP(hipGetLastError());
  return UDET_OK;
}
__global__ __launch_bounds__(256) void nonfinite_count_kernel(const float* __restrict__ g, long n, int* __restrict__ out) {
  int c = 0;
  for (long i = (long)blockIdx.x * 256 + threadIdx.x; i < n; i += (long)gridDim.x * 256) c += !(fabsf(g[i]) <= 3.402823466e38f);
#pragma unroll
// ... 74 lines not shown
```

### unsupervised_detection_amd/csrc/plan.h

```cpp
#pragma once
#include <map>
#include <string>
#include <vector>

#include "common.h"

namespace udet {

struct ParamDesc {
  std::string name;
  int rank;
  int shape[4];
  size_t offset, count;
};
struct NetParams {
  std::vector<ParamDesc> p;
  size_t total = 0;
  int add(const std::string& name, int a, int b = 0, int c = 0, int d = 0);
  int find(const std::string& name) const;
};
enum { NET_PWC = 0, NET_GEN = 1, NET_REC = 2 };
const NetParams& net_params(int net);

struct Buf {
// ... 13 lines not shown
  float alpha = 0.f;
  int w_idx = -1, b_idx = -1, g_idx = -1, be_idx = -1;
  int Kc = 0, ldw = 0, k_split = 0, k_gap = 0;
  size_t wp_off = 0;
  int KcT = 0, ldwT = 0;
  size_t wpT_off = 0;
  size_t bias_f_off = 0, scale_off = 0;
  size_t wu_off = 0, wuT_off = 0;
  size_t wino_off = 0, winoT_off = 0;
  int wino_np = 0, winoT_np = 0;
  bool upb = false;
  bool upb_bwd = false;
  bool upb_split = false;
  int xhat = -1, src = -1;
  size_t wupb_off = 0, wupbT_off = 0;
  struct SegLaunch {
    int nseg = 0;
    ConvSeg seg[UDET_MAX_SEGS];
    int seg_tap[UDET_MAX_SEGS + 1];
    std::vector<ConvTap> taps;
    size_t tab_off = 0;
  } upb_f, upb_b;
  int x = -1, x_coff = 0, y = -1, y_coff = 0;
  int res = -1, res_coff = 0, y2 = -1;
  int H = 0, W = 0;
  bool col2im = false;
  int ldz = 0, zbuf = -1;
  size_t wz_off = 0;
  bool x_in_slab = false, y_fanned_out = false;
  std::string pair_name;
};

struct Resolved {
  struct {
    int pyr[7][3];
    int est[7][5], flow[7], ctx[7][7];
    int up_feat[7], up_flow[7];
  } pwc;
  struct {
    int enc[2][9];
    int deconv[6], flow[6], upflow[6];
  } rec;
  int image, flow, mask, pred, image_next, flow_next, d_mask, flow_full;
  int pwc_x8, pwc_rflow2, pwc_c[7], pwc_slab[7];
  int gen_in, gen_a17, gen_d[18], gen_u[18];
  int rec_imgin, rec_fin, rec_conv6, rec_concat[6], rec_r[7], rec_rf[6], rec_flow[6];
  struct Grad {
    int pred, fin, conv6, u_conv6;
    int flow[6], concat[6], u_concat[6], r[7], rf[6];
    int p[6];
    int enc_du[2][9];
    int enc_dx[2][9], enc_ux[2][9];
  } grad[2];
};

struct Config {
  int batch, in_h, in_w, img_h, img_w;
  float flow_normalizer, cbn, epsilon;
  float lr, beta1, beta2, adam_eps, clip;
  unsigned long long noise_seed;
  int conv_fp16 = 0;
};

struct Plan {
  Config cfg;
  std::vector<Buf> bufs;
  std::map<std::string, int> buf_by_name;
  std::vector<Layer> pwc, gen, rec;
  size_t packed_floats = 0;
  size_t arena_floats = 0;
  enum { NLANE = 6, NCAND = 8, MAXCAND = 32 };
  std::vector<hipStream_t> cand;
  struct Placement {
    hipStream_t main = nullptr;
    hipStream_t lane[NLANE] = {};
    int queue[NLANE] = {};
    int nqueues = 1;
  };
  std::vector<Placement> placements;
  int placed = -1;
  hipEvent_t prefetch_ev = nullptr;
  hipEvent_t grad_ev[3] = {nullptr, nullptr, nullptr};
  bool prefetch_pending = false;
  std::vector<hipEvent_t> ev_pool, ev_pool_prefetch;
  size_t ev_next = 0, ev_next_prefetch = 0;
  bool in_prefetch = false;
  bool concurrent = true;
  bool enc_a_shared = false;
  size_t scratch_off[NLANE] = {}, scratch_floats = 0;
  size_t wgrad_off[NLANE] = {}, wgrad_floats = 0;
  ~Plan();
  size_t small_off = 0;
  size_t ticket_off = 0;
  size_t seg_off[3] = {0, 0, 0};
  size_t jobs_off[3] = {0, 0, 0};
  int njobs[3] = {0, 0, 0};
  struct ProfRec {
    int cat; double flops, bytes; hipEvent_t a, b; std::string name;
    double mfma_scale = 1.0;
    enum { MAXK = 16 };
    hipEvent_t kev[2 * MAXK];
    LaunchSink sink;
  };
  bool profiling = false;
  std::vector<ProfRec*> prof;
  long adam_t = 0;
  int* ovf_host = nullptr;
  hipEvent_t ovf_ev[3] = {nullptr, nullptr, nullptr};
  bool ovf_pending[3] = {false, false, false};
  long ovf_skipped = 0;
  int ovf_report_values = 0, ovf_report_nets = 0;
  bool pwc_packed = false;
  Resolved R;
  int add_buf(const std::string& name, int n, int h, int w, int ld);
  const Buf& buf(int id) const { return bufs[id]; }
  int bid(const std::string& name) const;
};

#define UDET_PACKJOB_CAP(layers) (8 * (layers) + 32)
#define UDET_SMALL_NOISE 256
#define UDET_SMALL_OVF 300
#define UDET_SMALL_SUMS 1024
Plan* plan_build(const Config& cfg);
void plan_debug_upb_min_pixels(long v);
void build_upb_launches(Layer& L, int h, int w);
void upb_pack_jobs(const Layer& L, const PackJob& base, std::vector<PackJob>& jobs);
enum { UDET_KNOB_ENC_A_LANE = 0, UDET_KNOB_REC_DEC_WGRAD_LANE = 1, UDET_KNOB_REC_ENC_WGRAD_LANE = 2, UDET_KNOB_GEN_WGRAD_LATE = 3, UDET_KNOB_NO_WGRAD_WINO = 6, UDET_KNOB_SKIP = 7, UDET_KNOB_NO_PAIRS = 8, UDET_KNOB_COUNT = 12 };
#ifdef UDET_EXPERIMENT
void plan_debug_knob(int id, long v);
long plan_knob(int id);
#else
constexpr long plan_knob(int) { return 0; }
#endif

int plan_init_workspace(Plan* P, float* ws, hipStream_t s);
int plan_pack_pwc(Plan* P, const float* w_pwc, float* ws, hipStream_t s);
int plan_pack_trainable(Plan* P, const float* w_gen, const float* w_rec, float* ws, hipStream_t s);
int plan_pwc_forward(Plan* P, const float* img1, const float* img2, float* ws, hipStream_t s);
int plan_forward(Plan* P, const float* img1, const float* img2, int ncalls, float* ws, hipStream_t s, bool prefetched = false);
int plan_prefetch(Plan* P, const float* img1, const float* img2, float* ws, hipStream_t s);
int plan_prefetch_consume(Plan* P, float* ws, hipStream_t s);
int plan_generator_forward(Plan* P, float* ws, hipStream_t s);
int plan_generator_layers(Plan* P, float* ws, hipStream_t s);
int plan_recover_forward(Plan* P, int ncalls, float* ws, hipStream_t s, bool inputs_prepacked = false, bool skip_enc_a = false, bool enc_a_input_packed = false);
int plan_losses(Plan* P, float* ws, hipStream_t s);
int plan_backward(Plan* P, int which, const float* w_gen, const float* w_rec, float* g_gen, float* g_rec, float* ws, hipStream_t s);
int plan_apply(Plan* P, int net, float* w, float* g, float* m, float* v, float* ws, hipStream_t s);
int plan_check_overflow(Plan* P, bool wait);
void plan_settle_adam_step(Plan* P);
int plan_lane_queues(Plan* P, hipStream_t s, int* queue);
int plan_pin_lanes(Plan* P, hipStream_t main, hipStream_t const* streams, int n);
enum { PROF_CONV_FWD = 0, PROF_CONV_DGRAD = 1, PROF_CONV_WGRAD = 2, PROF_WARP = 3, PROF_CORR = 4, PROF_NCAT = 5 };
void prof_begin(Plan* P, int cat, double flops, double bytes, hipStream_t s, const char* name = "");
void prof_end(Plan* P, hipStream_t s);

}
```

### unsupervised_detection_amd/csrc/plan_build.hip

```cpp
#include <stdarg.h>
#include <stdlib.h>
#include <string.h>

#include "conv_host.h"
#include "elementwise.h"
#include "plan.h"

namespace udet {

int NetParams::add(const std::string& name, int a, int b, int c, int d) {
  ParamDesc q;
  q.name = name;
  q.shape[0] = a; q.shape[1] = b; q.shape[2] = c; q.shape[3] = d;
  q.rank = d ? 4 : (c ? 3 : (b ? 2 : 1));
  q.count = (size_t)a * (b ? b : 1) * (c ? c : 1) * (d ? d : 1);
  q.offset = total;
  total += q.count;
  p.push_back(q);
  return (int)p.size() - 1;
}
int NetParams::find(const std::string& name) const {
  for (size_t i = 0; i < p.size(); ++i)
    if (p[i].name == name) return (int)i;
  return -1;
// ... 61 lines not shown
    {"conv13_upsample", 128, 64, 3, 1, 1, true, ACT_ELU}, {"conv14", 64, 64, 3, 1, 1, false, ACT_ELU},
    {"conv15_upsample", 64, 32, 3, 1, 1, true, ACT_ELU},  {"conv16", 32, 16, 3, 1, 1, false, ACT_ELU},
    {"conv17", 16, 2, 3, 1, 1, false, ACT_NONE}};

static NetParams build_gen_params() {
  NetParams n;
  for (int i = 0; i < 17; ++i) {
    const GenSpec& g = GEN[i];
    const std::string pre = g.up ? S("MaskNet/%s/%s_conv", g.name, g.name) : S("MaskNet/%s", g.name);
    n.add(pre + "/kernel", g.k, g.k, g.cin, g.cout);
    n.add(pre + "/bias", g.cout);
    n.add(S("MaskNet/%s/bn/gamma", g.name), g.cout);
    n.add(S("MaskNet/%s/bn/beta", g.name), g.cout);
  }
  return n;
}

struct EncSpec { const char* suf; int cin, cout, k, s; };
static const EncSpec ENC[9] = {{"conv1", 0, 16, 7, 2},   {"conv2", 16, 32, 5, 2},   {"conv3", 32, 64, 5, 2},
                               {"conv31", 64, 64, 3, 1}, {"conv4", 64, 128, 3, 2},  {"conv41", 128, 128, 3, 1},
                               {"conv5", 128, 128, 3, 2}, {"conv51", 128, 128, 3, 1}, {"conv6", 128, 128, 3, 2}};
struct DecSpec { const char* name; int k, cin, cout; };
static const DecSpec DEC[14] = {{"deconv5", 4, 256, 128}, {"flow5", 3, 384, 2},   {"deconv4", 4, 384, 128}, {"upflow4", 4, 2, 2},
                                {"flow4", 3, 386, 2},     {"deconv3", 4, 386, 64}, {"upflow3", 4, 2, 2},     {"flow3", 3, 194, 2},
                                {"deconv2", 4, 194, 32},  {"upflow2", 4, 2, 2},    {"flow2", 3, 98, 2},      {"deconv1", 4, 98, 16},
                                {"upflow1", 4, 2, 2},     {"flow1", 5, 50, 2}};

static NetParams build_rec_params() {
  NetParams n;
  for (int e = 0; e < 2; ++e)
    for (int i = 0; i < 9; ++i) {
      const int ci = ENC[i].cin ? ENC[i].cin : (e == 0 ? 3 : 4);
      n.add(S("FlownetS/%c%s/weights", e == 0 ? 'a' : 'b', ENC[i].suf), ENC[i].k, ENC[i].k, ci, ENC[i].cout);
      n.add(S("FlownetS/%c%s/biases", e == 0 ? 'a' : 'b', ENC[i].suf), ENC[i].cout);
    }
  for (int i = 0; i < 14; ++i) {
    n.add(S("FlownetS/%s/weights", DEC[i].name), DEC[i].k, DEC[i].k, DEC[i].cin, DEC[i].cout);
    n.add(S("FlownetS/%s/biases", DEC[i].name), DEC[i].cout);
  }
  return n;
}

const NetParams& net_params(int net) {
  static const NetParams pwc = build_pwc_params(), gen = build_gen_params(), rec = build_rec_params();
  return net == NET_PWC ? pwc : (net == NET_GEN ? gen : rec);
}

int Plan::add_buf(const std::string& name, int n, int h, int w, int ld) {
  Buf b;
  b.name = name; b.n = n; b.h = h; b.w = w; b.ld = ld; b.off = 0;
  bufs.push_back(b);
  buf_by_name[name] = (int)bufs.size() - 1;
  return (int)bufs.size() - 1;
}
int Plan::bid(const std::string& name) const {
  auto it = buf_by_name.find(name);
  return it == buf_by_name.end() ? -1 : it->second;
}

static Layer mk_layer(int net, const std::string& name, const std::string& wname, const std::string& bname, int k, int cin,
                      int cout, int stride, int dil, int act, float alpha) {
  Layer L;
  L.name = name; L.net = net;
  L.kh = L.kw = k; L.cin = cin; L.cout = cout; L.stride = stride; L.dil = dil;
  L.act = act; L.alpha = alpha;
  const NetParams& np = net_params(net);
  L.w_idx = np.find(wname);
  L.b_idx = np.find(bname);
  L.Kc = round_up(cin, cin <= 4 ? 4 : 8);
  L.ldw = round_up(cout, 4);
  L.k_split = L.Kc;
  L.k_gap = 0;
  return L;
}

static size_t align64(size_t v) { return (v + 63) & ~(size_t)63; }

Plan::~Plan() {
  for (auto& st : cand)
    if (st) (void)hipStreamDestroy(st);
  for (auto& e : ev_pool) (void)hipEventDestroy(e);
  for (auto& e : ev_pool_prefetch) (void)hipEventDestroy(e);
  if (prefetch_ev) (void)hipEventDestroy(prefetch_ev);
  for (auto* r : prof) delete r;
  for (auto& ev : grad_ev)
    if (ev) (void)hipEventDestroy(ev);
  for (auto& ev : ovf_ev)
    if (ev) (void)hipEventDestroy(ev);
  if (ovf_host) (void)hipHostFree(ovf_host);
}

static long g_upb_bwd_min = 8192;
void plan_debug_upb_min_pixels(long v) { g_upb_bwd_min = v < 0 ? 8192 : v; }
#ifdef UDET_EXPERIMENT
static long g_knob[UDET_KNOB_COUNT] = {};
void plan_debug_knob(int id, long v) { if (id >= 0 && id < UDET_KNOB_COUNT) g_knob[id] = v; }
long plan_knob(int id) { return id >= 0 && id < UDET_KNOB_COUNT ? g_knob[id] : 0; }
extern "C" void udet_exp_knob(int id, long v) { plan_debug_knob(id, v); }
#endif

static inline bool upb_used(int parity, int last, int a) { return !last || (parity == 0 ? a < 2 : a < 1); }
void build_upb_launches(Layer& L, int h, int w) {
  Layer::SegLaunch& F = L.upb_f;
  F.nseg = 0; F.taps.clear();
  for (int r = 0; r < 4; ++r) {
    const int rv = r & 1, cv = r >> 1;
    const int r0 = rv ? h - 1 : 0, c0 = cv ? w - 1 : 0, nr = rv ? 1 : h - 1, nc = cv ? 1 : w - 1;
    for (int c = 0; c < 4; ++c) {
      const int py = c >> 1, px = c & 1;
      ConvSeg& g = F.seg[F.nseg];
      memset(&g, 0, sizeof(g));
      g.oy = 2 * r0 + py; g.ox = 2 * c0 + px; g.h = nr; g.w = nc;
      F.seg_tap[F.nseg++] = (int)F.taps.size();
      for (int a = 0; a < 3; ++a)
        for (int b = 0; b < 3; ++b) {
          if (!upb_used(py, rv, a) || !upb_used(px, cv, b)) continue;
          F.taps.push_back(ConvTap{r0 + a + py, c0 + b + px, r * 36 + 9 * c + 3 * a + b});
        }
    }
  }
  F.seg_tap[F.nseg] = (int)F.taps.size();
  Layer::SegLaunch& B = L.upb_b;
  B.nseg = 0; B.taps.clear();
  struct Combo { int p, a, last; };
  auto combos = [](int grp, std::vector<Combo>& out) {
    out.clear();
    for (int p = 0; p < 2; ++p)
      for (int a = 0; a < 3; ++a) {
        int last = 0;
        if (grp > 0) {
          const int rp = grp - 1;
          if (p + a < rp) continue;
          last = (p + a == rp);
        }
        if (upb_used(p, last, a)) out.push_back(Combo{p, a, last});
      }
  };
  std::vector<Combo> rc, cc;
  for (int gr = 0; gr < 4; ++gr)
    for (int gc = 0; gc < 4; ++gc) {
      const int R0 = gr == 0 ? 0 : h - 2 + gr, C0 = gc == 0 ? 0 : w - 2 + gc;
      ConvSeg& g = B.seg[B.nseg];
      memset(&g, 0, sizeof(g));
      g.oy = R0; g.ox = C0; g.h = gr == 0 ? h - 1 : 1; g.w = gc == 0 ? w - 1 : 1;
      B.seg_tap[B.nseg++] = (int)B.taps.size();
      combos(gr, rc);
      combos(gc, cc);
      for (const Combo& y : rc)
        for (const Combo& x : cc)
          B.taps.push_back(ConvTap{2 * R0 - y.p - 2 * y.a, 2 * C0 - x.p - 2 * x.a, (y.last + 2 * x.last) * 36 + 9 * (2 * y.p + x.p) + 3 * y.a + x.a});
    }
  B.seg_tap[B.nseg] = (int)B.taps.size();
}

namespace {
struct Lookup {
  const Plan* P;
  bool ok = true;
  int miss(const char* kind, const std::string& name) {
    if (ok) set_error("plan_build: no %s '%s'", kind, name.c_str());
    ok = false;
    return -1;
  }
  int buf(const std::string& name) {
    const int id = P->bid(name);
    return id >= 0 ? id : miss("buffer", name);
// ... 425 lines not shown
```

### unsupervised_detection_amd/csrc/plan_pack.hip

```cpp
#include <string.h>

#include "conv_host.h"
#include "plan_run.h"

namespace udet {

void upb_pack_jobs(const Layer& L, const PackJob& base, std::vector<PackJob>& jobs) {
  PackJob j = base;
  for (int r = 0; r < 4; ++r) {
    j.T = 36; j.gamma_off = -1;
    j.dst_off = (long)(L.wupb_off + (size_t)r * 36 * L.Kc * L.ldw); j.R = L.cin; j.C = L.cout; j.Kc = L.Kc; j.ldw = L.ldw; j.k_split = L.k_split; j.k_gap = L.k_gap;
    j.mode = 9; j.beta_off = (long)((r & 1) * 3 + (r >> 1)); j.total = (long)L.Kc * L.ldw;
    jobs.push_back(j);
    if (L.upb_bwd) {
      j.dst_off = (long)(L.wupbT_off + (size_t)r * 36 * L.KcT * L.ldwT); j.Kc = L.KcT; j.ldw = L.ldwT; j.k_split = L.KcT; j.k_gap = 0;
      j.mode = 10; j.total = (long)L.KcT * L.ldwT;
      jobs.push_back(j);
    }
  }
}

int plan_init_workspace(Plan* P, float* ws, hipStream_t s) {
  UDET_HIP(hipMemsetAsync(ws, 0, P->arena_floats * sizeof(float), s));
  for (int net = 1; net <= 2; ++net) {
    const NetParams& np = net_params(net);
    std::vector<long> tab(2 * np.p.size());
    for (size_t i = 0; i < np.p.size(); ++i) {
      tab[i] = (long)np.p[i].offset;
      tab[np.p.size() + i] = (long)np.p[i].count;
    }
    UDET_HIP(hipMemcpyAsync(ws + P->seg_off[net], tab.data(), tab.size() * sizeof(long), hipMemcpyHostToDevice, s));
    UDET_HIP(hipStreamSynchronize(s));
  }
  for (int net = 1; net <= 2; ++net) {
    const NetParams& np = net_params(net);
    const std::vector<Layer>& layers = net == NET_GEN ? P->gen : P->rec;
    std::vector<PackJob> jobs;
    for (const auto& L : layers) {
      const int T = L.kh * L.kw;
      const long goff = L.g_idx >= 0 ? (long)np.p[L.g_idx].offset : -1, beoff = L.be_idx >= 0 ? (long)np.p[L.be_idx].offset : -1;
      PackJob j;
      memset(&j, 0, sizeof(j));
      j.src_off = (long)np.p[L.w_idx].offset; j.gamma_off = goff; j.beta_off = beoff;
      j.T = T;
      j.dst_off = (long)L.wp_off; j.R = L.cin; j.C = L.cout; j.Kc = L.Kc; j.ldw = L.ldw; j.k_split = L.k_split; j.k_gap = L.k_gap;
      j.mode = 0; j.total = (long)T * L.Kc * L.ldw;
      jobs.push_back(j);
      j.dst_off = (long)L.wpT_off; j.Kc = L.KcT; j.ldw = L.ldwT; j.k_split = L.KcT; j.k_gap = 0;
      j.mode = 1; j.total = (long)T * L.KcT * L.ldwT;
      jobs.push_back(j);
      if (L.col2im) {
        j.dst_off = (long)L.wz_off; j.R = L.cin; j.C = L.cout; j.Kc = L.Kc; j.ldw = L.ldz; j.k_split = L.k_split; j.k_gap = L.k_gap;
        j.mode = 3; j.total = (long)L.Kc * L.ldz;
        jobs.push_back(j);
      }
      if (L.up) {
        j.T = 16;
        j.dst_off = (long)L.wu_off; j.R = L.cin; j.C = L.cout; j.Kc = L.Kc; j.ldw = L.ldw; j.k_split = L.Kc; j.k_gap = 0;
        j.mode = 5; j.total = (long)16 * L.Kc * L.ldw;
        jobs.push_back(j);
        j.dst_off = (long)L.wuT_off; j.Kc = L.KcT; j.ldw = L.ldwT; j.k_split = L.KcT; j.k_gap = 0;
        j.mode = 6; j.total = (long)16 * L.KcT * L.ldwT;
        jobs.push_back(j);
        j.T = T;
      }
      if (L.upb) upb_pack_jobs(L, j, jobs);
      if (L.wino_off) {
        j.dst_off = (long)L.wino_off; j.R = L.cin; j.C = L.cout; j.Kc = L.Kc; j.ldw = L.wino_np; j.k_split = L.k_split; j.k_gap = L.k_gap;
        j.mode = 7; j.total = (long)(L.Kc / 8) * 2 * L.wino_np;
        jobs.push_back(j);
      }
      if (L.winoT_off) {
        j.dst_off = (long)L.winoT_off; j.R = L.cin; j.C = L.cout; j.Kc = L.KcT; j.ldw = L.winoT_np; j.k_split = L.KcT; j.k_gap = 0;
        j.mode = 8; j.total = (long)(L.KcT / 8) * 2 * L.winoT_np;
        jobs.push_back(j);
      }
      j.src_off = (long)np.p[L.b_idx].offset; j.dst_off = (long)L.bias_f_off; j.mode = 2; j.total = L.cout;
      jobs.push_back(j);
    }
    if (jobs.size() > UDET_PACKJOB_CAP(layers.size())) {
      set_error("plan_init: %zu weight re-layout jobs for %zu layers exceed the table's %zu entries", jobs.size(), layers.size(),
                (size_t)UDET_PACKJOB_CAP(layers.size()));
      return UDET_ERR_ARG;
    }
    P->njobs[net] = (int)jobs.size();
    UDET_HIP(hipMemcpyAsync(ws + P->jobs_off[net], jobs.data(), jobs.size() * sizeof(PackJob), hipMemcpyHostToDevice, s));
    UDET_HIP(hipStreamSynchronize(s));
  }
  for (const auto& L : P->rec)
    if (L.upb)
      for (const Layer::SegLaunch* g : {&L.upb_f, &L.upb_b})
        if (g == &L.upb_f || L.upb_bwd)
          UDET_HIP(hipMemcpyAsync(ws + g->tab_off, g->taps.data(), g->taps.size() * sizeof(ConvTap), hipMemcpyHostToDevice, s));
  UDET_HIP(hipStreamSynchronize(s));
  P->pwc_packed = false;
  return UDET_OK;
}

static int pack_layer(const Layer& L, const float* w_flat, float* ws, const float* scale, bool trainable, hipStream_t s) {
  const NetParams& np = net_params(L.net);
  const float* w = w_flat + np.p[L.w_idx].offset;
  const int T = L.kh * L.kw;
  if (L.transposed)
    UDET_TRY(launch_pack_weights(w, ws + L.wp_off, T, L.cout, L.cin, L.Kc, L.ldw, L.k_split, L.k_gap, 1, nullptr, s));
  else
    UDET_TRY(launch_pack_weights(w, ws + L.wp_off, T, L.cin, L.cout, L.Kc, L.ldw, L.k_split, L.k_gap, 0, scale, s));
  if (trainable)
    UDET_TRY(launch_pack_weights(w, ws + L.wpT_off, T, L.cin, L.cout, L.KcT, L.ldwT, L.KcT, 0, 1, scale, s));
  if (L.col2im)
    UDET_TRY(launch_pack_taps_into_n(w, ws + L.wz_off, T, L.cin, L.cout, L.Kc, L.ldz, L.k_split, L.k_gap, L.transposed ? 1 : 0, s));
  if (L.wino_off && !trainable)
    UDET_TRY(launch_wino_pack(w, ws + L.wino_off, L.cin, L.cout, L.Kc, L.wino_np, L.k_split, L.k_gap, 0, s));
  return UDET_OK;
}

int plan_pack_pwc(Plan* P, const float* w, float* ws, hipStream_t s) {
  const NetParams& np = net_params(NET_PWC);
  for (const auto& L : P->pwc) {
    UDET_TRY(pack_layer(L, w, ws, nullptr, false, s));
    UDET_TRY(launch_copy_channels(w + np.p[L.b_idx].offset, L.cout, 0, ws + L.bias_f_off, L.cout, 0, 1, L.cout, 1.f, 0.f, s));
  }
  P->pwc_packed = true;
  return UDET_OK;
}

int plan_pack_trainable(Plan* P, const float* w_gen, const float* w_rec, float* ws, hipStream_t s) {
  if (w_gen)
    UDET_TRY(launch_pack_jobs(reinterpret_cast<const PackJob*>(ws + P->jobs_off[NET_GEN]), P->njobs[NET_GEN], w_gen, ws, BN_C, s));
  if (w_rec)
    UDET_TRY(launch_pack_jobs(reinterpret_cast<const PackJob*>(ws + P->jobs_off[NET_REC]), P->njobs[NET_REC], w_rec, ws, BN_C, s));
  return UDET_OK;
}

}
```

### unsupervised_detection_amd/csrc/plan_step.hip

```cpp
#include "conv_host.h"
#include "elementwise.h"
#include "plan_run.h"

namespace udet {

static const int PWC_CH[7] = {0, 16, 32, 64, 96, 128, 196};
static const char* const WARP_NAME[7] = {"", "", "warp_costvol2", "warp_costvol3", "warp_costvol4", "warp_costvol5", "warp_costvol6"};

static int pwc_forward_on(Plan* P, const float* img1, const float* img2, float* ws, const Lane& L0, const Lane& LH) {
  if (!P->pwc_packed) {
    set_error("pwc_forward: call udet_pack_pwc first");
    return UDET_ERR_ARG;
  }
  const Config& c = P->cfg;
  const Resolved& R = P->R;
  const int B = c.batch;
  hipStream_t s = L0.s;
  auto fwd = [&](int layer, int N, const Lane& ln) { return run_fwd(P, P->pwc[layer], N, ws, ln); };
  UDET_TRY(launch_pack_pwc_input(img1, img2, ws + P->buf(R.pwc_x8).off, (long)B * c.in_h * c.in_w, s));
  for (int l = 1; l <= 6; ++l)
    for (int j = 0; j < 3; ++j) UDET_TRY(fwd(R.pwc.pyr[l][j], 2 * B, L0));
  for (int l = 6; l >= 2; --l) {
    const int h = c.in_h >> l, w = c.in_w >> l, C = PWC_CH[l];
    const Buf& cb = P->buf(R.pwc_c[l]);
// ... 75 lines not shown
}
static int dec_src(const Resolved& R, int k) { return k == 5 ? R.rec_conv6 : R.rec_concat[k + 1]; }

static int share_enc_a_output(Plan* P, const Layer& L, int ncalls, float* ws, hipStream_t s) {
  const Buf& y = P->buf(L.y);
  if (ncalls > 1 && L.y_fanned_out) return launch_share_samples(ws + y.off, (long)P->cfg.batch * y.h * y.w, y.ld, L.y_coff, L.cout, ncalls, s);
  return UDET_OK;
}
static int plan_rec_image_branch(Plan* P, int ncalls, float* ws, const Lane& ln, bool with_layers = true) {
  const Config& c = P->cfg;
  if (ncalls < 1) return UDET_OK;
  const long Ppix = (long)c.batch * c.img_h * c.img_w;
  UDET_TRY(launch_pack_imgin(ws + P->buf(P->R.image).off, ws + P->buf(P->R.rec_imgin).off, Ppix, 1, ln.s));
  if (!with_layers) return UDET_OK;
  for (int i = 0; i < 9; ++i) {
    const Layer& L = P->rec[P->R.rec.enc[0][i]];
    UDET_TRY(run_fwd(P, L, c.batch, ws, ln));
    UDET_TRY(share_enc_a_output(P, L, ncalls, ws, ln.s));
  }
  P->enc_a_shared = true;
  return UDET_OK;
}

int plan_recover_forward(Plan* P, int ncalls, float* ws, hipStream_t s, bool inputs_prepacked, bool skip_enc_a, bool enc_a_input_packed) {
  const Config& c = P->cfg;
  const Resolved& R = P->R;
  const int B = c.batch, N = ncalls * B;
  const long Ppix = (long)B * c.img_h * c.img_w;
  const Lane L0 = lane_of(P, s, 0);
  if (!inputs_prepacked)
    UDET_TRY(launch_mask_rec_inputs(ws + P->buf(R.gen_a17).off, ws + P->buf(R.flow).off, ws + P->buf(R.mask).off, ws + P->buf(R.rec_fin).off,
                                    Ppix, ncalls, s));
  if (ncalls < 1) return UDET_OK;
  auto enc = [&](int e, int i) -> const Layer& { return P->rec[R.rec.enc[e][i]]; };
  if (!skip_enc_a && pairs_on(P)) {
    if (!inputs_prepacked && !enc_a_input_packed) UDET_TRY(plan_rec_image_branch(P, ncalls, ws, L0, false));
    for (int i = 0; i < 9; ++i) {
      const Layer& La = enc(0, i);
      UDET_TRY(run_fwd_pair(P, La, inputs_prepacked ? N : B, enc(1, i), N, ws, L0));
      if (!inputs_prepacked) UDET_TRY(share_enc_a_output(P, La, ncalls, ws, s));
    }
    P->enc_a_shared = !inputs_prepacked;
  } else {
    if (!skip_enc_a) {
      if (inputs_prepacked) {
        for (int i = 0; i < 9; ++i) UDET_TRY(run_fwd(P, enc(0, i), N, ws, L0));
        P->enc_a_shared = false;
      } else {
        UDET_TRY(plan_rec_image_branch(P, ncalls, ws, L0));
      }
    }
    for (int i = 0; i < 9; ++i) UDET_TRY(run_fwd(P, enc(1, i), N, ws, L0));
  }
  for (int k = 5; k >= 1; --k) {
    const Layer& dcl = P->rec[R.rec.deconv[k]];
    if (!dcl.upb) UDET_TRY(rec_resize(P, dec_src(R, k), R.rec_r[k + 1], N, ws, s));
    UDET_TRY(run_fwd(P, dcl, N, ws, L0));
    if (k < 5) {
      UDET_TRY(rec_resize(P, R.rec_flow[k + 1], R.rec_rf[k + 1], N, ws, s));
      UDET_TRY(run_fwd(P, P->rec[R.rec.upflow[k]], N, ws, L0));
    }
    UDET_TRY(run_fwd(P, P->rec[R.rec.flow[k]], N, ws, L0));
  }
  const Buf& f1 = P->buf(R.rec_flow[1]);
  return launch_resize_bilinear_fwd(ws + f1.off, f1.ld, 0, N, f1.h, f1.w, ws + P->buf(R.pred).off, 2, 0, c.img_h, c.img_w, 2, 1.f, 1.f, s);
}

int plan_losses(Plan* P, float* ws, hipStream_t s) {
  const Config& c = P->cfg;
  float* sm = ws + P->small_off;
  const long HW = (long)c.img_h * c.img_w;
  return launch_losses(ws + P->buf(P->R.flow).off, ws + P->buf(P->R.mask).off, ws + P->buf(P->R.pred).off, HW,
                       c.batch, c.cbn, c.epsilon, (float)(c.img_w * c.img_h * c.batch), sm + 8192, sm, sm + 16, sm + UDET_SMALL_SUMS, s);
}

int plan_prefetch_consume(Plan* P, float* ws, hipStream_t s) {
  if (!P->prefetch_pending) {
    set_error("forward_prefetched: no udet_prefetch_flow is pending");
    return UDET_ERR_ARG;
  }
  (void)hipStreamWaitEvent(s, P->prefetch_ev, 0);
  P->prefetch_pending = false;
  const Buf &fn = P->buf(P->R.flow_next), &in = P->buf(P->R.image_next);
  UDET_HIP(hipMemcpyAsync(ws + P->buf(P->R.flow).off, ws + fn.off, fn.floats() * sizeof(float), hipMemcpyDeviceToDevice, s));
  UDET_HIP(hipMemcpyAsync(ws + P->buf(P->R.image).off, ws + in.off, in.floats() * sizeof(float), hipMemcpyDeviceToDevice, s));
  return UDET_OK;
}

int plan_forward(Plan* P, const float* img1, const float* img2, int ncalls, float* ws, hipStream_t s, bool prefetched) {
  P->ev_next = 0;
  const Lane L0 = lane_of(P, s, 0), LI = lane_of(P, s, 1);
  if (prefetched) {
    UDET_TRY(plan_prefetch_consume(P, ws, s));
    img1 = img2 = nullptr;
  } else if (img1 && P->prefetch_pending) {
    (void)hipStreamWaitEvent(s, P->prefetch_ev, 0);
  }
  order_after(P, L0, LI);
  if (img1) UDET_TRY(plan_prepare_image(P, img1, P->R.image, ws, LI.s));
  hipEvent_t e_img = nullptr;
  if (LI.s != L0.s) {
    e_img = next_event(P);
    (void)hipEventRecord(e_img, LI.s);
  }
  const bool paired = pairs_on(P);
  UDET_TRY(plan_rec_image_branch(P, ncalls, ws, LI, !paired));
  if (img1) {
    UDET_TRY(pwc_forward_on(P, img1, img2, ws, L0, lane_of(P, s, 2)));
    UDET_TRY(plan_prepare_flow(P, P->R.flow, ws, s));
  }
  if (e_img) (void)hipStreamWaitEvent(s, e_img, 0);
  UDET_TRY(plan_generator_forward(P, ws, s));
  order_after(P, LI, L0);
  UDET_TRY(plan_recover_forward(P, ncalls, ws, s, false, !paired, paired));
  if (ncalls == 3) UDET_TRY(plan_losses(P, ws, s));
  return UDET_OK;
}

static int rec_backward(Plan* P, int N, const Resolved::Grad& G, bool with_wgrad, bool need_dfin, const float* w_rec, float* g_rec, float* ws,
                        const Lane& LD, const Lane& LW, const Lane* LAp = nullptr, const Lane* LWdecp = nullptr) {
  const Config& c = P->cfg;
  const Resolved& R = P->R;
  hipStream_t s = LD.s;
  const Lane LWdec = LWdecp ? *LWdecp : LW;
  auto wgrad_on = [&](const Lane& lw, const Layer& L, int dy, bool is_du, int n) -> int {
    order_after(P, LD, lw);
    return run_wgrad(P, L, n < 0 ? N : n, dy, is_du, w_rec, g_rec, ws, lw);
  };
  auto wgrad = [&](const Layer& L, int dy, bool is_du, int n = -1) -> int { return wgrad_on(LW, L, dy, is_du, n); };
  auto wgrad_dec = [&](const Layer& L, int dy, bool is_du) -> int { return wgrad_on(LWdec, L, dy, is_du, -1); };
  const Lane LA = LAp ? *LAp : LD;
  const bool a_own_lane = LA.s != LD.s;
  const int ncopies = N / c.batch;
  const bool a_shared = P->enc_a_shared && ncopies > 1;
  const Emit none;
  const float LEAK = 0.2f;
  {
    const Buf& df1 = P->buf(G.flow[1]);
    UDET_TRY(launch_resize_bilinear_bwd(ws + P->buf(G.pred).off, 2, 0, N, c.img_h, c.img_w, ws + df1.off, df1.ld, 0, df1.h, df1.w, 2, 0, s));
  }
  for (int k = 1; k <= 5; ++k) {
    const int dconcat = G.concat[k], uconcat = G.u_concat[k];
    const Layer* fl = &P->rec[R.rec.flow[k]];
    const Layer* dc = &P->rec[R.rec.deconv[k]];
    Emit em;
    em.ubuf = uconcat; em.abuf = fl->x; em.c0 = 0; em.c1 = dc->cout; em.act = ACT_LEAKY; em.alpha = LEAK;
    UDET_TRY(run_dgrad(P, *fl, N, G.flow[k], false, dconcat, 0, k == 1 ? 0 : 1, -1, em, ws, LD));
    if (with_wgrad) UDET_TRY(wgrad_dec(*fl, G.flow[k], false));
    if (k < 5) {
      const Layer* uf = &P->rec[R.rec.upflow[k]];
      if (with_wgrad) UDET_TRY(wgrad_dec(*uf, dconcat, false));
      UDET_TRY(run_dgrad(P, *uf, N, dconcat, false, G.rf[k + 1], 0, 0, -1, none, ws, LD));
      const Buf &drf = P->buf(G.rf[k + 1]), &dfn = P->buf(G.flow[k + 1]);
      UDET_TRY(launch_resize_bilinear_bwd(ws + drf.off, drf.ld, 0, N, drf.h, drf.w, ws + dfn.off, dfn.ld, 0, dfn.h, dfn.w, drf.ld, 0, s));
    }
    if (with_wgrad) {
      if (dc->upb) {
        order_after(P, LD, LWdec);
        UDET_TRY(rec_resize(P, dec_src(R, k), R.rec_r[k + 1], N, ws, LWdec.s));
      }
      UDET_TRY(wgrad_dec(*dc, uconcat, true));
    }
    if (dc->upb_bwd) {
      UDET_TRY(run_dgrad_upb(P, *dc, N, uconcat, G.p[k + 1], G.concat[k + 1], ws, LD));
      continue;
    }
    const int dr = G.r[k + 1];
    UDET_TRY(run_dgrad(P, *dc, N, uconcat, true, dr, 0, 0, -1, none, ws, LD));
    const Buf& bdr = P->buf(dr);
    const Buf& dsrc = P->buf(k == 5 ? G.conv6 : G.concat[k + 1]);
    UDET_TRY(launch_resize_bilinear_bwd(ws + bdr.off, bdr.ld, 0, N, bdr.h, bdr.w, ws + dsrc.off, dsrc.ld, 0, dsrc.h, dsrc.w,
                                        bdr.ld, 0, s));
  }
  {
    const Buf &d6 = P->buf(G.conv6), &a6 = P->buf(R.rec_conv6), &u6 = P->buf(G.u_conv6);
    UDET_TRY(launch_emit_du(ws + d6.off, ws + a6.off, ws + u6.off, (long)N * d6.h * d6.w, d6.ld, 0, d6.ld, ACT_LEAKY, LEAK, s));
  }
  if (a_own_lane) order_after(P, LD, LA);
  const bool pair_enc = pairs_on(P, 1) && with_wgrad && !a_own_lane;
  for (int i = 8; i >= 0; --i) {
    DgradJob job[2];
    int njob = 0;
    for (int e = 0; e < 2; ++e) {
      if (e == 0 && !with_wgrad) continue;
      const Layer* L = &P->rec[R.rec.enc[e][i]];
      const int du = G.enc_du[e][i];
      const bool shared = e == 0 && a_shared;
      const int Ne = shared ? c.batch : N;
      const bool own = e == 0 && a_own_lane;
      const Lane& LE = own ? LA : LD;
      hipStream_t se = LE.s;
      if (shared && i == 8) {
        const Buf& u = P->buf(du);
        UDET_TRY(launch_fold_samples(ws + u.off, (long)c.batch * u.h * u.w, u.ld, L->y_coff, L->cout, ncopies, se));
      }
      if (with_wgrad) {
// ... 114 lines not shown
```

### unsupervised_detection_amd/engine.py

```python
from __future__ import annotations

import ctypes
from dataclasses import dataclass

import torch

from ._ffi import c_f, c_i, c_p, c_sz, check, lib
from .weights import NET_GEN, NET_REC


class _Cfg(ctypes.Structure):
    _fields_ = [("batch", c_i), ("in_h", c_i), ("in_w", c_i), ("img_h", c_i), ("img_w", c_i), ("flow_normalizer", c_f),
                ("cbn", c_f), ("epsilon", c_f), ("lr", c_f), ("beta1", c_f), ("beta2", c_f), ("adam_eps", c_f), ("clip", c_f),
                ("noise_seed", ctypes.c_ulonglong), ("conv_fp16", c_i)]


lib.udet_plan_create.restype = c_i
lib.udet_plan_create.argtypes = [ctypes.POINTER(_Cfg), ctypes.POINTER(c_p)]
lib.udet_plan_destroy.restype = None
lib.udet_plan_destroy.argtypes = [c_p]
lib.udet_workspace_bytes.restype = c_sz
lib.udet_workspace_bytes.argtypes = [c_p]
lib.udet_plan_init.restype = c_i
lib.udet_plan_init.argtypes = [c_p, c_p, c_p]
lib.udet_buffer_count.restype = c_i
lib.udet_buffer_count.argtypes = [c_p]
lib.udet_buffer_info.restype = c_i
lib.udet_buffer_info.argtypes = [c_p, c_i, ctypes.POINTER(ctypes.c_char_p), ctypes.POINTER(c_sz), ctypes.POINTER(c_i)]
lib.udet_plan_set_concurrent.restype = c_i
lib.udet_plan_set_concurrent.argtypes = [c_p, c_i]
lib.udet_plan_lane_queues.restype = c_i
lib.udet_plan_lane_queues.argtypes = [c_p, c_p, ctypes.POINTER(c_i)]
lib.udet_plan_pin_lanes.restype = c_i
lib.udet_plan_pin_lanes.argtypes = [c_p, c_p, ctypes.POINTER(c_p), c_i]
lib.udet_fp16_overflow_count.restype = ctypes.c_long
lib.udet_fp16_overflow_count.argtypes = [c_p]
lib.udet_get_adam_step.restype = ctypes.c_long
lib.udet_get_adam_step.argtypes = [c_p]
lib.udet_set_adam_step.restype = None
lib.udet_set_adam_step.argtypes = [c_p, ctypes.c_long]
for _n, _a in (("udet_pack_pwc", [c_p, c_p, c_p, c_p]), ("udet_pack_trainable", [c_p, c_p, c_p, c_p, c_p]),
               ("udet_pwc_forward", [c_p, c_p, c_p, c_p, c_p]), ("udet_forward", [c_p, c_p, c_p, c_i, c_p, c_p]),
               ("udet_forward_from_flow", [c_p, c_i, c_p, c_p]), ("udet_generator_forward", [c_p, c_p, c_p]),
               ("udet_recover_forward", [c_p, c_i, c_p, c_p]),
               ("udet_prefetch_flow", [c_p, c_p, c_p, c_p, c_p]), ("udet_forward_prefetched", [c_p, c_i, c_p, c_p]),
               ("udet_prefetch_consume", [c_p, c_p, c_p]),
               ("udet_backward", [c_p, c_i, c_p, c_p, c_p, c_p, c_p, c_p]),
               ("udet_apply", [c_p, c_i, c_p, c_p, c_p, c_p, c_p, c_p]),
               ("udet_train_step", [c_p, c_i] + [c_p] * 12)):
    getattr(lib, _n).restype = c_i
    getattr(lib, _n).argtypes = _a

lib.udet_autotune.restype = c_i
lib.udet_autotune.argtypes = [c_p] * 7
lib.udet_tuned_shapes.restype = c_i
lib.udet_tuned_shapes.argtypes = []
lib.udet_profile_begin.restype = c_i
lib.udet_profile_begin.argtypes = [c_p]
lib.udet_profile_end.restype = c_i
lib.udet_profile_end.argtypes = [c_p, ctypes.POINTER(ctypes.c_double), c_i, c_p]

GEN, REC, BOTH = 1, 2, 3
LOSS_KEYS = ("generator", "recover", "red_rate", "red_rate_compl", "reconstruction_loss", "reconstruction_compl_loss",
             "denominator_red_rate", "denominator_red_rate_compl")


@dataclass
class EngineConfig:
    batch_size: int = 4
    in_height: int = 384
    in_width: int = 640
    img_height: int = 192
    img_width: int = 384
    flow_normalizer: float = 80.0
    cbn: float = 0.5
    epsilon: float = 75.0
    beta1: float = 0.9
    lr: float = 1e-4
    beta2: float = 0.999
    adam_eps: float = 1e-8
    clip: float = 0.2
    noise_seed: int = 8964
    conv_fp16: bool = False


def _ptr(t):
    if t is None:
        return None
    if not (t.is_cuda and t.dtype == torch.float32 and t.is_contiguous()):
        raise ValueError("expected a contiguous float32 CUDA(HIP) tensor")
    return t.data_ptr()


class Engine:
    def __init__(self, cfg: EngineConfig, device="cuda"):
        if not torch.cuda.is_available():
            raise RuntimeError("unsupervised_detection_amd needs an MI355X (no CPU fallback exists)")
        self.cfg = cfg
        self.device = torch.device(device)
        c = _Cfg(cfg.batch_size, cfg.in_height, cfg.in_width, cfg.img_height, cfg.img_width, cfg.flow_normalizer, cfg.cbn,
                 cfg.epsilon, cfg.lr, cfg.beta1, cfg.beta2, cfg.adam_eps, cfg.clip, cfg.noise_seed, 1 if cfg.conv_fp16 else 0)
        h = c_p()
        check(lib.udet_plan_create(ctypes.byref(c), ctypes.byref(h)))
        self._h = h
        self.workspace_bytes = int(lib.udet_workspace_bytes(h))
        self.ws = torch.empty(self.workspace_bytes, dtype=torch.uint8, device=self.device)
        self._bufs = {}
        for i in range(lib.udet_buffer_count(h)):
            name = ctypes.c_char_p()
            off = c_sz()
            dims = (c_i * 4)()
            check(lib.udet_buffer_info(h, i, ctypes.byref(name), ctypes.byref(off), dims))
            self._bufs[name.value.decode()] = (off.value, tuple(dims))
        check(lib.udet_plan_init(h, self.ws.data_ptr(), self._stream()))

    def __del__(self):
        h = getattr(self, "_h", None)
        if h:
            lib.udet_plan_destroy(h)
            self._h = None

    @staticmethod
    def _stream():
        return torch.cuda.current_stream().cuda_stream

    def buffer_names(self):
        return list(self._bufs)

    def buffer(self, name: str) -> torch.Tensor:
        off, (n, h, w, ld) = self._bufs[name]
        cnt = n * h * w * ld
        return self.ws[off:off + 4 * cnt].view(torch.float32).view(n, h, w, ld)

    def pack_pwc(self, w_pwc):
        check(lib.udet_pack_pwc(self._h, _ptr(w_pwc), self.ws.data_ptr(), self._stream()))

    def pack_trainable(self, w_gen=None, w_rec=None):
        check(lib.udet_pack_trainable(self._h, _ptr(w_gen), _ptr(w_rec), self.ws.data_ptr(), self._stream()))

    def _check_pair(self, img1, img2):
        c = self.cfg
        want = (c.batch_size, c.in_height, c.in_width, 3)
        for name, t in (("img1", img1), ("img2", img2)):
            if tuple(t.shape) != want:
                raise ValueError("%s has shape %s, this plan takes %s (pad the last batch of a one-pass reader: "
                                 "learner.pad_batch)" % (name, tuple(t.shape), want))

    def pwc_forward(self, img1, img2):
        self._check_pair(img1, img2)
        check(lib.udet_pwc_forward(self._h, _ptr(img1), _ptr(img2), self.ws.data_ptr(), self._stream()))
        return self.buffer("flow_full")

    def forward(self, img1, img2, ncalls=3):
        self._check_pair(img1, img2)
        check(lib.udet_forward(self._h, _ptr(img1), _ptr(img2), ncalls, self.ws.data_ptr(), self._stream()))

    def prefetch_flow(self, img1, img2):
        self._check_pair(img1, img2)
        self._prefetch_keep = (img1, img2)
        check(lib.udet_prefetch_flow(self._h, _ptr(img1), _ptr(img2), self.ws.data_ptr(), self._stream()))

    def prefetch_consume(self):
        check(lib.udet_prefetch_consume(self._h, self.ws.data_ptr(), self._stream()))
        self._prefetch_keep = None

    def forward_in_place(self, ncalls=3):
        check(lib.udet_forward_from_flow(self._h, ncalls, self.ws.data_ptr(), self._stream()))

    def forward_prefetched(self, ncalls=3):
        check(lib.udet_forward_prefetched(self._h, ncalls, self.ws.data_ptr(), self._stream()))
        self._prefetch_keep = None

    def forward_from_flow(self, image, flow, ncalls=3):
        if tuple(image.shape) != tuple(self.buffer("image").shape) or tuple(flow.shape) != tuple(self.buffer("flow").shape):
            raise ValueError("image / flow must be %s / %s" % (tuple(self.buffer("image").shape), tuple(self.buffer("flow").shape)))
        self.buffer("image").copy_(image)
        self.buffer("flow").copy_(flow)
        check(lib.udet_forward_from_flow(self._h, ncalls, self.ws.data_ptr(), self._stream()))

    def losses(self):
        v = self.buffer("losses").view(-1).cpu().tolist()
        return dict(zip(LOSS_KEYS, v))

    def backward(self, which, w_gen, w_rec, g_gen, g_rec):
        check(lib.udet_backward(self._h, which, _ptr(w_gen), _ptr(w_rec), _ptr(g_gen), _ptr(g_rec), self.ws.data_ptr(),
                                self._stream()))

    def apply(self, net, w, g, m, v):
        check(lib.udet_apply(self._h, net, _ptr(w), _ptr(g), _ptr(m), _ptr(v), self.ws.data_ptr(), self._stream()))

    def train_step(self, which, img1, img2, w_gen, w_rec, g_gen, g_rec, m_gen, v_gen, m_rec, v_rec):
        self._check_pair(img1, img2)
        check(lib.udet_train_step(self._h, which, _ptr(img1), _ptr(img2), _ptr(w_gen), _ptr(w_rec), _ptr(g_gen), _ptr(g_rec),
                                  _ptr(m_gen), _ptr(v_gen), _ptr(m_rec), _ptr(v_rec), self.ws.data_ptr(), self._stream()))

    def autotune(self, w_gen, w_rec, g_gen, g_rec):
        check(lib.udet_autotune(self._h, _ptr(w_gen), _ptr(w_rec), _ptr(g_gen), _ptr(g_rec), self.ws.data_ptr(), self._stream()))
        return int(lib.udet_tuned_shapes())

    def profile(self, fn):
        cats = ("conv_fwd", "conv_dgrad", "conv_wgrad", "warp", "cost_volume")
        check(lib.udet_profile_begin(self._h))
        try:
            fn()
        finally:
            out = (ctypes.c_double * (5 * len(cats)))()
            check(lib.udet_profile_end(self._h, out, len(cats), self._stream()))
        return {c: dict(groups=out[5 * i], ms=out[5 * i + 1], flops=out[5 * i + 2], bytes=out[5 * i + 3], bracket_ms=out[5 * i + 4])
                for i, c in enumerate(cats)}

    def set_concurrent(self, on: bool):
        check(lib.udet_plan_set_concurrent(self._h, 1 if on else 0))

    def lane_queues(self):
        q = (c_i * 6)()
        n = int(lib.udet_plan_lane_queues(self._h, self._stream(), q))
        if n < 0:
            check(n)
        return n, [int(v) for v in q]

    def pin_lanes(self, side_streams):
        side_streams = list(side_streams)
# ... 15 lines not shown
```

### unsupervised_detection_amd/trainer.py

```python
from __future__ import annotations

import torch

from . import weights as W
from .engine import BOTH, GEN, REC, Engine


class TrainState:

    def __init__(self, engine: Engine, seed: int = 8964, w_pwc=None, w_gen=None, w_rec=None, autotune: bool = False):
        dev = engine.device
        self.engine = engine
        self.w_pwc = (w_pwc if w_pwc is not None else W.init_flat(W.NET_PWC, seed)).to(dev)
        self.w_gen = (w_gen if w_gen is not None else W.init_flat(W.NET_GEN, seed)).to(dev)
        self.w_rec = (w_rec if w_rec is not None else W.init_flat(W.NET_REC, seed)).to(dev)
        n_gen, n_rec = self.w_gen.numel(), self.w_rec.numel()
        off_rec = (n_gen + 63) // 64 * 64
        self.g_all = torch.zeros(off_rec + n_rec, dtype=torch.float32, device=dev)
        self.g_gen, self.g_rec = self.g_all[:n_gen], self.g_all[off_rec:off_rec + n_rec]
        self.m_gen, self.v_gen = torch.zeros_like(self.w_gen), torch.zeros_like(self.w_gen)
        self.m_rec, self.v_rec = torch.zeros_like(self.w_rec), torch.zeros_like(self.w_rec)
        engine.pack_pwc(self.w_pwc)
        engine.pack_trainable(self.w_gen, self.w_rec)
        self._dirty = 0
        if autotune:
            self.tuned_shapes = self._autotune_shared()

    def _autotune_shared(self) -> int:
        import os
        import tempfile

        import torch.distributed as dist

        from ._ffi import lib
        e = self.engine
        if not (dist.is_available() and dist.is_initialized()) or dist.get_world_size() == 1:
            return e.autotune(self.w_gen, self.w_rec, self.g_gen, self.g_rec)
        text, n = [None], 0
        fd, path = tempfile.mkstemp(prefix="udet_tune_", suffix=".txt")
        os.close(fd)
        try:
            if dist.get_rank() == 0:
                n = e.autotune(self.w_gen, self.w_rec, self.g_gen, self.g_rec)
                lib.udet_tune_save(path.encode())
                with open(path) as f:
                    text[0] = f.read()
            dist.broadcast_object_list(text, src=0)
            if dist.get_rank() != 0:
                with open(path, "w") as f:
                    f.write(text[0])
                n = int(lib.udet_tune_load(path.encode()))
                if n < 0:
                    n = e.autotune(self.w_gen, self.w_rec, self.g_gen, self.g_rec)
        finally:
            os.remove(path)
        return n


def flush_weights(st: TrainState):
    dirty = getattr(st, "_dirty", 0)
    if dirty:
        st.engine.pack_trainable(st.w_gen if dirty & GEN else None, st.w_rec if dirty & REC else None)
    st._dirty = 0


def _dp_active(group) -> bool:
    import os

    import torch.distributed as dist
    if group is False or not (dist.is_available() and dist.is_initialized()):
        return False
    return dist.get_world_size(group) > 1 or os.environ.get("UDET_DP_WORLD1") == "1"


def allreduce_mean_(t: torch.Tensor, group=None, async_op=False):
    import torch.distributed as dist
    if not _dp_active(group):
        return None
    work = dist.all_reduce(t, op=dist.ReduceOp.SUM, group=group, async_op=False)
    t.div_(dist.get_world_size(group))
    return work if async_op else None


def _exchange_gradients(st: TrainState, which: int, group):
    if not _dp_active(group):
        return
    e = st.engine
    if which != BOTH:
        allreduce_mean_(st.g_rec if which & REC else st.g_gen, group)
        return
    from ._ffi import check, lib
    comm = getattr(st, "_comm_stream", None)
    if comm is None:
        comm = st._comm_stream = torch.cuda.Stream(device=e.device)
    main = torch.cuda.current_stream(e.device)
    check(lib.udet_stream_wait_grads(e._h, W.NET_REC, comm.cuda_stream))
    with torch.cuda.stream(comm):
        allreduce_mean_(st.g_rec, group)
        done = comm.record_event()
    allreduce_mean_(st.g_gen, group)
    main.wait_event(done)


def exchange_alone(st: TrainState, group=None):
    if not _dp_active(group):
        return
    e = st.engine
    comm = getattr(st, "_comm_stream", None)
    if comm is None:
        comm = st._comm_stream = torch.cuda.Stream(device=e.device)
    main = torch.cuda.current_stream(e.device)
    comm.wait_stream(main)
    with torch.cuda.stream(comm):
        allreduce_mean_(st.g_rec, group)
        done = comm.record_event()
    allreduce_mean_(st.g_gen, group)
    main.wait_event(done)


def train_step(st: TrainState, img1, img2, which: int = BOTH, group=None, next_pair=None):
    e = st.engine
    flush_weights(st)

    def call(fn, *a):
        if not getattr(e.cfg, "conv_fp16", False):
            return fn(*a)
        from ._ffi import UdetOverflow
        for _ in range(4):
            try:
                return fn(*a)
            except UdetOverflow as ex:
                st.overflow_skipped = getattr(st, "overflow_skipped", 0) + 1
                import sys
                print("[udet] fp16 overflow: an optimizer update was dropped (%d so far): %s" % (st.overflow_skipped, ex), file=sys.stderr)
        return fn(*a)

    if getattr(st, "_prefetched", None) is not None:
        p1, p2 = st._prefetched
        if p1.data_ptr() != img1.data_ptr() or p2.data_ptr() != img2.data_ptr():
            raise ValueError("train_step: this step's pair is not the one prefetched by the previous call")
        e.prefetch_consume()
        st._prefetched = None
        if next_pair is not None:
            e.prefetch_flow(next_pair[0], next_pair[1])
            st._prefetched = (next_pair[0], next_pair[1])
        call(e.forward_in_place, 3)
    else:
        call(e.forward, img1, img2, 3)
        if next_pair is not None:
            e.prefetch_flow(next_pair[0], next_pair[1])
            st._prefetched = (next_pair[0], next_pair[1])
    call(e.backward, which, st.w_gen, st.w_rec, st.g_gen, st.g_rec)
    _exchange_gradients(st, which, group)
    if which & GEN:
        e.apply(W.NET_GEN, st.w_gen, st.g_gen, st.m_gen, st.v_gen)
    if which & REC:
        e.apply(W.NET_REC, st.w_rec, st.g_rec, st.m_rec, st.v_rec)
    st._dirty = which & (GEN | REC)
```

Baseline: 501.5.

## Defer trainable weight packing onto a side lane and flatten pack job grid

Splits the per-step weight re-layout so that only the generator's forward-needed pack jobs run on the main stream. The generator's backward layouts and the recover net's packs run on a side lane, joined by an event before their first consumer. The pack kernel now uses a flat, work-proportional block assignment with binary search over job start blocks instead of a fixed 48 blocks per job, and replaces per-element div/mod with incremental index walking. It also merges two device copies into one kernel and adds a loss-finish and grad-flag debug path. The risk is a missed join leaving a data race if a consumer path skips plan_pack_join.

Result: no change. 502.6, median of 6 (+0.2%).

```diff
diff --git a/include/udet.h b/include/udet.h
--- a/include/udet.h
+++ b/include/udet.h
@@ -214,6 +214,7 @@
 
 int udet_pack_pwc(udet_plan* plan, const float* w_pwc, void* workspace, void* stream);
 int udet_pack_trainable(udet_plan* plan, const float* w_gen, const float* w_rec, void* workspace, void* stream);
+int udet_pack_trainable_deferred(udet_plan* plan, const float* w_gen, const float* w_rec, void* workspace, void* stream);
 
 int udet_pwc_forward(udet_plan* plan, const float* img1, const float* img2, void* workspace, void* stream);
 int udet_forward(udet_plan* plan, const float* img1, const float* img2, int ncalls, void* workspace, void* stream);
diff --git a/include/udet_debug.h b/include/udet_debug.h
--- a/include/udet_debug.h
+++ b/include/udet_debug.h
@@ -1,6 +1,8 @@
 #ifndef UDET_DEBUG_H
 #define UDET_DEBUG_H
 #include <stddef.h>
+
+#include "udet.h"
 #ifdef __cplusplus
 extern "C" {
 #endif
@@ -43,6 +45,11 @@
 int udet_debug_launch_mask_rec_inputs(const float* logits, const float* f, float* mask, float* fin, long p, int ncalls, void* stream);
 int udet_debug_launch_pack_imgin(const float* img, float* imgin, long p, int ncalls, void* stream);
 int udet_debug_launch_mask_bwd(const float* dmask, const float* dfin, const float* f, const float* mask, float* dlogits, long p, void* stream);
+int udet_debug_loss_blocks(void);
+int udet_debug_launch_loss_finish(const float* part, int b, float eps, float num_pixels, float* losses, float* coef, float* sums, void* stream);
+int udet_debug_grad_absmean_split(void);
+int udet_debug_launch_grad_flag(const float* vpart, const long* seg_len, int nvars, float thresh, float* out2, void* stream);
+int udet_debug_pack_job_table(const udet_config* cfg, int net, int* mode, long* dst_off, int cap, int* n_group_a);
 typedef struct udet_debug_conv_ex {
   int form;
   int n, h, wd, cin, cout, k, stride, dilation, up;
diff --git a/unsupervised_detection_amd/_devel.py b/unsupervised_detection_amd/_devel.py
--- a/unsupervised_detection_amd/_devel.py
+++ b/unsupervised_detection_amd/_devel.py
@@ -64,6 +64,16 @@
     _fn.argtypes = _args
 dbg.udet_debug_gen_input_workspace_bytes.restype = ctypes.c_size_t
 dbg.udet_debug_gen_input_workspace_bytes.argtypes = [_i]
+for _name, _args in (("loss_finish", [_p, _i, _f, _f, _p, _p, _p, _p]), ("grad_flag", [_p, _p, _i, _f, _p, _p])):
+    _fn = getattr(dbg, "udet_debug_launch_" + _name)
+    _fn.restype = ctypes.c_int
+    _fn.argtypes = _args
+dbg.udet_debug_loss_blocks.restype = ctypes.c_int
+dbg.udet_debug_loss_blocks.argtypes = []
+dbg.udet_debug_grad_absmean_split.restype = ctypes.c_int
+dbg.udet_debug_grad_absmean_split.argtypes = []
+dbg.udet_debug_pack_job_table.restype = ctypes.c_int
+dbg.udet_debug_pack_job_table.argtypes = [_p, _i, _p, _p, _i, _p]
 
 
 class ConvEx(ctypes.Structure):
@@ -143,3 +153,15 @@
     ns, nt = nseg.value, ntaps.value
     return dict(nseg=ns, seg=[tuple(seg[4 * s:4 * s + 4]) for s in range(ns)], seg_tap=list(seg_tap[:ns + 1]),
                 taps=[tuple(taps[3 * t:3 * t + 3]) for t in range(nt)])
+
+
+def pack_job_table(cfg, net: int):
+    from .engine import _Cfg
+    c = _Cfg(cfg.batch_size, cfg.in_height, cfg.in_width, cfg.img_height, cfg.img_width, cfg.flow_normalizer, cfg.cbn,
+             cfg.epsilon, cfg.lr, cfg.beta1, cfg.beta2, cfg.adam_eps, cfg.clip, cfg.noise_seed, 1 if cfg.conv_fp16 else 0)
+    cap = 1024
+    mode, dst, na = (ctypes.c_int * cap)(), (ctypes.c_long * cap)(), ctypes.c_int(0)
+    n = dbg.udet_debug_pack_job_table(ctypes.addressof(c), net, ctypes.addressof(mode), ctypes.addressof(dst), cap, ctypes.addressof(na))
+    if n < 0:
+        _check(n)
+    return list(mode[:n]), list(dst[:n]), na.value
diff --git a/unsupervised_detection_amd/csrc/api_plan.hip b/unsupervised_detection_amd/csrc/api_plan.hip
--- a/unsupervised_detection_amd/csrc/api_plan.hip
+++ b/unsupervised_detection_amd/csrc/api_plan.hip
@@ -30,7 +30,10 @@
   if (h) { delete h->p; delete h; }
 }
 size_t udet_workspace_bytes(const udet_plan* h) { return h->p->arena_floats * sizeof(float); }
-int udet_plan_init(udet_plan* h, void* ws, void* stream) { return plan_init_workspace(h->p, (float*)ws, (hipStream_t)stream); }
+int udet_plan_init(udet_plan* h, void* ws, void* stream) {
+  plan_pack_join(h->p, (hipStream_t)stream);
+  return plan_init_workspace(h->p, (float*)ws, (hipStream_t)stream);
+}
 
 int udet_param_count(int net) { return (net < 0 || net > 2) ? 0 : (int)net_params(net).p.size(); }
 size_t udet_param_total(int net) { return (net < 0 || net > 2) ? 0 : net_params(net).total; }
@@ -84,7 +87,11 @@
 int udet_pack_trainable(udet_plan* h, const float* w_gen, const float* w_rec, void* ws, void* stream) {
   return plan_pack_trainable(h->p, w_gen, w_rec, (float*)ws, (hipStream_t)stream);
 }
+int udet_pack_trainable_deferred(udet_plan* h, const float* w_gen, const float* w_rec, void* ws, void* stream) {
+  return plan_pack_trainable_deferred(h->p, w_gen, w_rec, (float*)ws, (hipStream_t)stream);
+}
 int udet_pwc_forward(udet_plan* h, const float* img1, const float* img2, void* ws, void* stream) {
+  plan_pack_join(h->p, (hipStream_t)stream);
   return plan_pwc_forward(h->p, img1, img2, (float*)ws, (hipStream_t)stream);
 }
 int udet_forward_from_flow(udet_plan* h, int ncalls, void* ws, void* stream) {
@@ -93,16 +100,19 @@
   return plan_forward(h->p, nullptr, nullptr, ncalls, (float*)ws, (hipStream_t)stream);
 }
 int udet_generator_forward(udet_plan* h, void* ws, void* stream) {
+  plan_pack_join(h->p, (hipStream_t)stream);
   UDET_TRY(plan_generator_forward(h->p, (float*)ws, (hipStream_t)stream));
   return plan_recover_forward(h->p, 0, (float*)ws, (hipStream_t)stream);
 }
 int udet_generator_layers(udet_plan* h, void* ws, void* stream) {
   h->p->ev_next = 0;
+  plan_pack_join(h->p, (hipStream_t)stream);
   UDET_TRY(plan_generator_layers(h->p, (float*)ws, (hipStream_t)stream));
   return plan_recover_forward(h->p, 0, (float*)ws, (hipStream_t)stream);
 }
 int udet_recover_forward(udet_plan* h, int n, void* ws, void* stream) {
   if (n < 1 || n > 3) { set_error("recover_forward: n must be 1..3 (multiples of the plan batch)"); return UDET_ERR_ARG; }
+  plan_pack_join(h->p, (hipStream_t)stream);
   return plan_recover_forward(h->p, n, (float*)ws, (hipStream_t)stream, true);
 }
 int udet_forward(udet_plan* h, const float* img1, const float* img2, int ncalls, void* ws, void* stream) {
@@ -127,9 +137,11 @@
                   void* stream) {
   UDET_TRY(plan_check_overflow(h->p, false));
   if (which < 1 || which > 3) { set_error("backward: which must be 1 (generator), 2 (recover) or 3 (both)"); return UDET_ERR_ARG; }
+  plan_pack_join(h->p, (hipStream_t)stream);
   return plan_backward(h->p, which, w_gen, w_rec, g_gen, g_rec, (float*)ws, (hipStream_t)stream);
 }
 int udet_apply(udet_plan* h, int net, float* w, float* g, float* m, float* v, void* ws, void* stream) {
+  plan_pack_join(h->p, (hipStream_t)stream);
   return plan_apply(h->p, net, w, g, m, v, (float*)ws, (hipStream_t)stream);
 }
 int udet_train_step(udet_plan* h, int which, const float* img1, const float* img2, float* w_gen, float* w_rec, float* g_gen,
@@ -147,6 +159,7 @@
   float* ws = (float*)ws_;
   hipStream_t s = (hipStream_t)stream;
   if (!P->pwc_packed) { set_error("autotune: pack the PWC-Net and trainable weights first"); return UDET_ERR_ARG; }
+  plan_pack_join(P, s);
   const size_t lo = P->packed_floats, hi = P->small_off;
   UDET_TRY(launch_fill_uniform(ws + lo, (long)(hi - lo), 0x5eedull, -0.5f, 0.5f, s));
   const size_t img_floats = (size_t)P->cfg.batch * P->cfg.in_h * P->cfg.in_w * 3;
@@ -240,10 +253,12 @@
 
 int udet_generator_backward(udet_plan* h, const float* w_gen, float* g_gen, void* ws, void* stream) {
   if (!w_gen || !g_gen) { set_error("generator_backward: null argument"); return UDET_ERR_ARG; }
+  plan_pack_join(h->p, (hipStream_t)stream);
   return plan_backward(h->p, 1, w_gen, nullptr, g_gen, nullptr, (float*)ws, (hipStream_t)stream);
 }
 int udet_recover_backward(udet_plan* h, const float* w_rec, float* g_rec, void* ws, void* stream) {
   if (!w_rec || !g_rec) { set_error("recover_backward: null argument"); return UDET_ERR_ARG; }
+  plan_pack_join(h->p, (hipStream_t)stream);
   return plan_backward(h->p, 2, nullptr, w_rec, nullptr, g_rec, (float*)ws, (hipStream_t)stream);
 }
 int udet_grad_absmean(udet_plan* h, int net, const float* g, float* out2, void* ws_, void* stream) {
diff --git a/unsupervised_detection_amd/csrc/common.h b/unsupervised_detection_amd/csrc/common.h
--- a/unsupervised_detection_amd/csrc/common.h
+++ b/unsupervised_detection_amd/csrc/common.h
@@ -166,6 +166,7 @@
 struct PackJob {
   long src_off, dst_off, gamma_off, beta_off;
   long total;
+  int blk0, nblk;
   int T, R, C, Kc, ldw, k_split, k_gap, mode;
 };
 
diff --git a/unsupervised_detection_amd/csrc/conv_host.h b/unsupervised_detection_amd/csrc/conv_host.h
--- a/unsupervised_detection_amd/csrc/conv_host.h
+++ b/unsupervised_detection_amd/csrc/conv_host.h
@@ -48,7 +48,8 @@
                         int mode, const float* scale, hipStream_t stream);
 int launch_pack_taps_into_n(const float* src, float* dst, int T, int R, int C, int Kc, int ldz, int k_split, int k_gap,
                             int transposed, hipStream_t stream);
-int launch_pack_jobs(const PackJob* jobs_dev, int njobs, const float* wsrc, float* ws, float bn_c, hipStream_t stream);
+int launch_pack_jobs(const PackJob* jobs_dev, int njobs, const float* wsrc, float* ws, float bn_c, hipStream_t stream, int nblocks = 0);
+int pack_jobs_assign_blocks(PackJob* jobs, int n);
 int launch_fold_bn(const float* b, const float* gamma, const float* beta, float c, float* scale, float* bias_f, int n,
                    hipStream_t stream);
 int launch_copy_channels(const float* src, int lds, int s_coff, float* dst, int ldd, int d_coff, long P, int C, float mul,
diff --git a/unsupervised_detection_amd/csrc/conv_host.hip b/unsupervised_detection_amd/csrc/conv_host.hip
--- a/unsupervised_detection_amd/csrc/conv_host.hip
+++ b/unsupervised_detection_amd/csrc/conv_host.hip
@@ -89,14 +89,39 @@
   return true;
 }
 
+struct RowWalk {
+  int n, k, t, dn, dk, dt, ldw, Kc;
+  template <typename I>
+  __device__ __forceinline__ void decode(I e0, I step) {
+    const I row = e0 / (I)ldw, srow = step / (I)ldw;
+    n = (int)(e0 - row * (I)ldw);
+    dn = (int)(step - srow * (I)ldw);
+    const I t0 = row / (I)Kc, st = srow / (I)Kc;
+    t = (int)t0; k = (int)(row - t0 * (I)Kc);
+    dt = (int)st; dk = (int)(srow - st * (I)Kc);
+  }
+  __device__ __forceinline__ RowWalk(long e0, long step, long total, int ldw_, int Kc_) : ldw(ldw_), Kc(Kc_) {
+    if (total + step < (1L << 31)) decode<unsigned>((unsigned)e0, (unsigned)step);
+    else decode<long>(e0, step);
+  }
+  __device__ __forceinline__ void next() {
+    n += dn;
+    int c = n >= ldw ? 1 : 0;
+    n -= c ? ldw : 0;
+    k += dk + c;
+    c = k >= Kc ? 1 : 0;
+    k -= c ? Kc : 0;
+    t += dt + c;
+  }
+};
+
 __global__ __launch_bounds__(256) void pack_weights_kernel(const float* __restrict__ src, float* __restrict__ dst, int T,
                                                            int R, int C, int Kc, int ldw, int k_split, int k_gap,
                                                            int mode, const float* __restrict__ scale) {
   const long total = (long)T * Kc * ldw;
-  for (long e = (long)blockIdx.x * 256 + threadIdx.x; e < total; e += (long)gridDim.x * 256) {
-    const int n = (int)(e % ldw);
-    const int k = (int)((e / ldw) % Kc);
-    const int t = (int)(e / ((long)ldw * Kc));
+  RowWalk rw((long)blockIdx.x * 256 + threadIdx.x, (long)gridDim.x * 256, total, ldw, Kc);
+  for (long e = (long)blockIdx.x * 256 + threadIdx.x; e < total; e += (long)gridDim.x * 256, rw.next()) {
+    const int n = rw.n, k = rw.k, t = rw.t;
     float v = 0.f;
     int ks = k;
     if (k >= k_split) ks = (k < k_split + k_gap) ? -1 : k - k_gap;
@@ -128,21 +153,35 @@
      {{1.f, 1.f, 0.f, 0.f}, {0.f, 0.f, 0.f, 0.f}, {0.f, 0.f, 0.f, 0.f}},
      {{0.f, .5f, 0.f, 0.f}, {0.f, -.5f, -1.f, -.5f}, {0.f, 0.f, 0.f, -.5f}}}};
 
-__global__ __launch_bounds__(256) void pack_jobs_kernel(const PackJob* __restrict__ jobs, const float* __restrict__ wsrc,
+__global__ __launch_bounds__(256) void pack_jobs_kernel(const PackJob* __restrict__ jobs, int njobs, const float* __restrict__ wsrc,
                                                         float* __restrict__ ws, float bn_c) {
-  const PackJob j = jobs[blockIdx.y];
+  int jb = blockIdx.y;
+  long bx = blockIdx.x, nbx = gridDim.x;
+  if (njobs > 0) {
+    const int b = (int)blockIdx.x + jobs[0].blk0;
+    int lo = 0, hi = njobs - 1;
+    while (lo < hi) {
+      const int mid = (lo + hi + 1) >> 1;
+      if (jobs[mid].blk0 <= b) lo = mid;
+      else hi = mid - 1;
+    }
+    jb = lo;
+  }
+  const PackJob j = jobs[jb];
+  if (njobs > 0) { bx = (int)blockIdx.x + jobs[0].blk0 - j.blk0; nbx = j.nblk; }
   const float* src = wsrc + j.src_off;
   float* dst = ws + j.dst_off;
   const float* gamma = j.gamma_off >= 0 ? wsrc + j.gamma_off : nullptr;
   if (j.mode == 2) {
-    for (long e = (long)blockIdx.x * 256 + threadIdx.x; e < j.total; e += (long)gridDim.x * 256)
+    for (long e = bx * 256 + threadIdx.x; e < j.total; e += nbx * 256)
       dst[e] = gamma ? src[e] * (gamma[e] * bn_c) + wsrc[j.beta_off + e] : src[e];
     return;
   }
   if (j.mode == 9 || j.mode == 10) {
     const int rv = (int)(j.beta_off / 3), cv = (int)(j.beta_off % 3);
-    for (long e = (long)blockIdx.x * 256 + threadIdx.x; e < j.total; e += (long)gridDim.x * 256) {
-      const int n = (int)(e % j.ldw), k = (int)(e / j.ldw);
+    RowWalk rw(bx * 256 + threadIdx.x, nbx * 256, j.total, j.ldw, j.Kc);
+    for (long e = bx * 256 + threadIdx.x; e < j.total; e += nbx * 256, rw.next()) {
+      const int n = rw.n, k = rw.k;
       int ks = k;
       if (k >= j.k_split) ks = (k < j.k_split + j.k_gap) ? -1 : k - j.k_gap;
       const int ci = j.mode == 9 ? ks : n, co = j.mode == 9 ? n : ks;
@@ -181,13 +220,13 @@
     return;
   }
   if (j.mode == 7 || j.mode == 8) {
-    for (long e = (long)blockIdx.x * 256 + threadIdx.x; e < j.total; e += (long)gridDim.x * 256) wino_pack_item(j, src, gamma, bn_c, dst, e);
+    for (long e = bx * 256 + threadIdx.x; e < j.total; e += nbx * 256) wino_pack_item(j, src, gamma, bn_c, dst, e);
     return;
   }
-  for (long e = (long)blockIdx.x * 256 + threadIdx.x; e < j.total; e += (long)gridDim.x * 256) {
-    const int n = (int)(e % j.ldw);
-    const int k = (int)((e / j.ldw) % j.Kc);
-    int t = (int)(e / ((long)j.ldw * j.Kc));
+  RowWalk rw(bx * 256 + threadIdx.x, nbx * 256, j.total, j.ldw, j.Kc);
+  for (long e = bx * 256 + threadIdx.x; e < j.total; e += nbx * 256, rw.next()) {
+    const int n = rw.n, k = rw.k;
+    int t = rw.t;
     float v = 0.f;
     int ks = k;
     if (k >= j.k_split) ks = (k < j.k_split + j.k_gap) ? -1 : k - j.k_gap;
@@ -218,11 +257,26 @@
     dst[e] = v;
   }
 }
-int launch_pack_jobs(const PackJob* jobs_dev, int njobs, const float* wsrc, float* ws, float bn_c, hipStream_t stream) {
+int launch_pack_jobs(const PackJob* jobs_dev, int njobs, const float* wsrc, float* ws, float bn_c, hipStream_t stream, int nblocks) {
   if (njobs < 1) return UDET_OK;
-  UDET_LAUNCH(pack_jobs_kernel, dim3(48, njobs), dim3(256), 0, stream, jobs_dev, wsrc, ws, bn_c);
-  UDET_HIP(hipGetLastError());
-  return UDET_OK;
+  if (nblocks > 0) UDET_LAUNCH(pack_jobs_kernel, dim3(nblocks), dim3(256), 0, stream, jobs_dev, njobs, wsrc, ws, bn_c);
+  else UDET_LAUNCH(pack_jobs_kernel, dim3(48, njobs), dim3(256), 0, stream, jobs_dev, 0, wsrc, ws, bn_c);
+  UDET_HIP(hipGetLastError());
+  return UDET_OK;
+}
+#define PACK_ITEMS 8
+int pack_jobs_assign_blocks(PackJob* jobs, int n) {
+  int b = 0;
+  for (int i = 0; i < n; ++i) {
+    const long per_block = jobs[i].mode >= 7 ? 256 : 256 * PACK_ITEMS;
+    long nb = (jobs[i].total + per_block - 1) / per_block;
+    if (nb < 1) nb = 1;
+    if (nb > 4096) nb = 4096;
+    jobs[i].blk0 = b;
+    jobs[i].nblk = (int)nb;
+    b += (int)nb;
+  }
+  return b;
 }
 
 __global__ __launch_bounds__(256) void pack_job_kernel(const PackJob j, const float* __restrict__ wsrc, float* __restrict__ ws) {
diff --git a/unsupervised_detection_amd/csrc/devel/api_debug.hip b/unsupervised_detection_amd/csrc/devel/api_debug.hip
--- a/unsupervised_detection_amd/csrc/devel/api_debug.hip
+++ b/unsupervised_detection_amd/csrc/devel/api_debug.hip
@@ -543,6 +543,36 @@
   UDET_TRY(glue_align(who, "f", f, 8));
   return launch_mask_bwd(dmask, dfin, f, mask, dlogits, p, (hipStream_t)stream);
 }
+int udet_debug_loss_blocks(void) { return (int)(loss_part_floats(1) / 5); }
+int udet_debug_launch_loss_finish(const float* part, int b, float eps, float num_pixels, float* losses, float* coef, float* sums, void* stream) {
+  const char* who = "debug_launch_loss_finish";
+  if (!part || !losses || !coef || !sums || b < 1 || b > 1024) { set_error("%s: bad argument (b 1..1024)", who); return UDET_ERR_ARG; }
+  return launch_loss_finish(part, b, eps, num_pixels, losses, coef, sums, (hipStream_t)stream);
+}
+int udet_debug_grad_absmean_split(void) { return grad_absmean_split(); }
+int udet_debug_launch_grad_flag(const float* vpart, const long* seg_len, int nvars, float thresh, float* out2, void* stream) {
+  const char* who = "debug_launch_grad_flag";
+  if (!vpart || !seg_len || !out2 || nvars < 1 || nvars > 8192) { set_error("%s: bad argument (nvars 1..8192)", who); return UDET_ERR_ARG; }
+  return launch_grad_flag(vpart, seg_len, nvars, thresh, out2, (hipStream_t)stream);
+}
+int udet_debug_pack_job_table(const udet_config* c, int net, int* mode, long* dst_off, int cap, int* n_group_a) {
+  const char* who = "debug_pack_job_table";
+  if (!c || !mode || !dst_off || !n_group_a || (net != NET_GEN && net != NET_REC)) { set_error("%s: bad argument (net 1 or 2)", who); return UDET_ERR_ARG; }
+  Config k;
+  k.batch = c->batch; k.in_h = c->in_h; k.in_w = c->in_w; k.img_h = c->img_h; k.img_w = c->img_w;
+  k.flow_normalizer = c->flow_normalizer; k.cbn = c->cbn; k.epsilon = c->epsilon;
+  k.lr = c->lr; k.beta1 = c->beta1; k.beta2 = c->beta2; k.adam_eps = c->adam_eps; k.clip = c->clip;
+  k.noise_seed = c->noise_seed;
+  k.conv_fp16 = c->conv_fp16 ? 1 : 0;
+  Plan* P = plan_build(k);
+  if (!P) return UDET_ERR_SHAPE;
+  std::vector<PackJob> jobs;
+  plan_pack_job_table(P, net, jobs, n_group_a);
+  delete P;
+  if ((int)jobs.size() > cap) { set_error("%s: %zu jobs, room for %d", who, jobs.size(), cap); return UDET_ERR_ARG; }
+  for (size_t i = 0; i < jobs.size(); ++i) { mode[i] = jobs[i].mode; dst_off[i] = jobs[i].dst_off; }
+  return (int)jobs.size();
+}
 
 void udet_debug_set_tuning(int on) {
   conv_set_tuning(on);
diff --git a/unsupervised_detection_amd/csrc/elementwise.h b/unsupervised_detection_amd/csrc/elementwise.h
--- a/unsupervised_detection_amd/csrc/elementwise.h
+++ b/unsupervised_detection_amd/csrc/elementwise.h
@@ -18,6 +18,8 @@
 int launch_losses(const float* f, const float* mask, const float* pred, long HW, int B, float cbn, float eps,
                   float num_pixels, float* part, float* losses, float* coef, float* sums, hipStream_t s);
 size_t loss_part_floats(int B);
+int launch_loss_finish(const float* part, int B, float eps, float num_pixels, float* losses, float* coef, float* sums, hipStream_t s);
+int launch_copy2(float* d0, const float* s0, long n0, float* d1, const float* s1, long n1, hipStream_t s);
 int launch_rec_loss_bwd(const float* f, const float* mask, const float* pred, float* dpred, long BHW, float cbn,
                         float inv_np, hipStream_t s);
 int launch_gen_loss_bwd(const float* f, const float* mask, const float* pred, const float* coef, float* dpred,
@@ -26,6 +28,8 @@
                     hipStream_t s);
 int launch_grad_absmean(const float* g, const long* seg_off, const long* seg_len, int nvars, float* vmean, float thresh,
                         float* out, hipStream_t s);
+int launch_grad_flag(const float* vpart, const long* seg_len, int nvars, float thresh, float* out, hipStream_t s);
+int grad_absmean_split(void);
 int launch_adam(float* w, float* g, float* m, float* v, long n, float lr_t, float b1, float b2, float eps, float clip,
                 const float* flag, uint64_t seed, uint64_t step, hipStream_t s, int mode = 0, const int* skip = nullptr);
 int launch_nonfinite_count(const float* g, long n, int* out, hipStream_t s);
diff --git a/unsupervised_detection_amd/csrc/elementwise.hip b/unsupervised_detection_amd/csrc/elementwise.hip
--- a/unsupervised_detection_amd/csrc/elementwise.hip
+++ b/unsupervised_detection_amd/csrc/elementwise.hip
@@ -482,6 +482,27 @@
   UDET_HIP(hipGetLastError());
   return UDET_OK;
 }
+template <typename V>
+__global__ __launch_bounds__(256) void copy2_kernel(V* __restrict__ d0, const V* __restrict__ s0, long n0, V* __restrict__ d1,
+                                                    const V* __restrict__ s1, long n1) {
+  for (long i = (long)blockIdx.x * 256 + threadIdx.x; i < n0 + n1; i += (long)gridDim.x * 256) {
+    if (i < n0) d0[i] = s0[i];
+    else d1[i - n0] = s1[i - n0];
+  }
+}
+int launch_copy2(float* d0, const float* s0, long n0, float* d1, const float* s1, long n1, hipStream_t s) {
+  if (n0 < 0 || n1 < 0) { set_error("copy2: negative length"); return UDET_ERR_ARG; }
+  if (n0 + n1 == 0) return UDET_OK;
+  const bool v4 = ((reinterpret_cast<uintptr_t>(d0) | reinterpret_cast<uintptr_t>(s0) | reinterpret_cast<uintptr_t>(d1) |
+                    reinterpret_cast<uintptr_t>(s1)) & 15) == 0 && n0 % 4 == 0 && n1 % 4 == 0;
+  if (v4)
+    hipLaunchKernelGGL(copy2_kernel<float4>, dim3(grid_for((n0 + n1) / 4)), dim3(256), 0, s, reinterpret_cast<float4*>(d0),
+                       reinterpret_cast<const float4*>(s0), n0 / 4, reinterpret_cast<float4*>(d1), reinterpret_cast<const float4*>(s1), n1 / 4);
+  else
+    hipLaunchKernelGGL(copy2_kernel<float>, dim3(grid_for(n0 + n1)), dim3(256), 0, s, d0, s0, n0, d1, s1, n1);
+  UDET_HIP(hipGetLastError());
+  return UDET_OK;
+}
 
 __device__ __forceinline__ float charb(float e, float cbn) {
   const float s = e * e + 0.001f * 0.001f;
@@ -516,14 +537,25 @@
     o[0] = R; o[1] = Rc; o[2] = Pp; o[3] = Dr; o[4] = Dc;
   }
 }
-__global__ void loss_finish_kernel(const float* __restrict__ part, int B, float eps, float num_pixels,
-                                   float* __restrict__ losses, float* __restrict__ coef, float* __restrict__ sums) {
-  if (threadIdx.x != 0 || blockIdx.x != 0) return;
+__global__ __launch_bounds__(64) void loss_finish_kernel(const float* __restrict__ part, int B, float eps, float num_pixels,
+                                                         float* __restrict__ losses, float* __restrict__ coef, float* __restrict__ sums) {
+  extern __shared__ float sv[];
+  for (int c = threadIdx.x; c < 5 * B; c += 64) {
+    const int b = c / 5, j = c - b * 5;
+    float p[LS_BLOCKS];
+#pragma unroll
+    for (int k = 0; k < LS_BLOCKS; ++k) p[k] = part[((long)b * LS_BLOCKS + k) * 5 + j];
+    float a = 0.f;
+#pragma unroll
+    for (int k = 0; k < LS_BLOCKS; ++k) a += p[k];
+    sv[c] = a;
+  }
+  __syncthreads();
+  if (threadIdx.x != 0) return;
   float red = 0.f, redc = 0.f, rs = 0.f;
   for (int b = 0; b < B; ++b) {
-    float v[5] = {0, 0, 0, 0, 0};
-    for (int k = 0; k < LS_BLOCKS; ++k)
-      for (int j = 0; j < 5; ++j) v[j] += part[((long)b * LS_BLOCKS + k) * 5 + j];
+    float v[5];
+    for (int j = 0; j < 5; ++j) v[j] = sv[b * 5 + j];
     const float D = v[3] + eps, Dc = v[4] + eps;
     red += 1.f - v[0] / D;
     redc += 1.f - v[1] / Dc;
@@ -544,7 +576,10 @@
 int launch_losses(const float* f, const float* mask, const float* pred, long HW, int B, float cbn, float eps,
                   float num_pixels, float* part, float* losses, float* coef, float* sums, hipStream_t s) {
   hipLaunchKernelGGL(loss_sums_kernel, dim3(LS_BLOCKS, B), dim3(256), 0, s, f, mask, pred, HW, B, cbn, part);
-  hipLaunchKernelGGL(loss_finish_kernel, dim3(1), dim3(64), 0, s, part, B, eps, num_pixels, losses, coef, sums);
+  return launch_loss_finish(part, B, eps, num_pixels, losses, coef, sums, s);
+}
+int launch_loss_finish(const float* part, int B, float eps, float num_pixels, float* losses, float* coef, float* sums, hipStream_t s) {
+  hipLaunchKernelGGL(loss_finish_kernel, dim3(1), dim3(64), 5 * (size_t)B * sizeof(float), s, part, B, eps, num_pixels, losses, coef, sums);
   UDET_HIP(hipGetLastError());
   return UDET_OK;
 }
@@ -672,26 +707,38 @@
   const float s = block_sum((s0 + s1) + (s2 + s3), sm);
   if (threadIdx.x == 0) vpart[blockIdx.x * GA_SPLIT + blockIdx.y] = s;
 }
-__global__ void grad_flag_kernel(const float* __restrict__ vpart, const long* __restrict__ seg_len, int nvars, float thresh,
-                                 float* __restrict__ out ) {
-  if (threadIdx.x == 0 && blockIdx.x == 0) {
+#define GF_THREADS 128
+__global__ __launch_bounds__(GF_THREADS) void grad_flag_kernel(const float* __restrict__ vpart, const long* __restrict__ seg_len, int nvars,
+                                                               float thresh, float* __restrict__ out ) {
+  extern __shared__ float vm[];
+  for (int i = threadIdx.x; i < nvars; i += GF_THREADS) {
+    float p[GA_SPLIT];
+#pragma unroll
+    for (int j = 0; j < GA_SPLIT; ++j) p[j] = vpart[i * GA_SPLIT + j];
+    float v = 0.f;
+#pragma unroll
+    for (int j = 0; j < GA_SPLIT; ++j) v += p[j];
+    vm[i] = v / (float)seg_len[i];
+  }
+  __syncthreads();
+  if (threadIdx.x == 0) {
     float s = 0.f;
-    for (int i = 0; i < nvars; ++i) {
-      float v = 0.f;
-      for (int j = 0; j < GA_SPLIT; ++j) v += vpart[i * GA_SPLIT + j];
-      s += v / (float)seg_len[i];
-    }
+    for (int i = 0; i < nvars; ++i) s += vm[i];
     s /= (float)nvars;
     out[0] = s;
     out[1] = s < thresh ? 1.f : 0.f;
   }
 }
+int launch_grad_flag(const float* vpart, const long* seg_len, int nvars, float thresh, float* out, hipStream_t s) {
+  hipLaunchKernelGGL(grad_flag_kernel, dim3(1), dim3(GF_THREADS), (size_t)nvars * sizeof(float), s, vpart, seg_len, nvars, thresh, out);
+  UDET_HIP(hipGetLastError());
+  return UDET_OK;
+}
+int grad_absmean_split(void) { return GA_SPLIT; }
 int launch_grad_absmean(const float* g, const long* seg_off, const long* seg_len, int nvars, float* vmean, float thresh,
                         float* out, hipStream_t s) {
   hipLaunchKernelGGL(grad_absmean_kernel, dim3(nvars, GA_SPLIT), dim3(256), 0, s, g, seg_off, seg_len, vmean);
-  hipLaunchKernelGGL(grad_flag_kernel, dim3(1), dim3(64), 0, s, vmean, seg_len, nvars, thresh, out);
-  UDET_HIP(hipGetLastError());
-  return UDET_OK;
+  return launch_grad_flag(vmean, seg_len, nvars, thresh, out, s);
 }
 
 __device__ __host__ __forceinline__ float udet_uniform01(uint64_t seed, uint64_t step, uint64_t idx) {
diff --git a/unsupervised_detection_amd/csrc/plan.h b/unsupervised_detection_amd/csrc/plan.h
--- a/unsupervised_detection_amd/csrc/plan.h
+++ b/unsupervised_detection_amd/csrc/plan.h
@@ -119,6 +119,8 @@
   hipEvent_t prefetch_ev = nullptr;
   hipEvent_t grad_ev[3] = {nullptr, nullptr, nullptr};
   bool prefetch_pending = false;
+  hipEvent_t pack_ev = nullptr, pack_fork_ev = nullptr;
+  bool pack_pending = false;
   std::vector<hipEvent_t> ev_pool, ev_pool_prefetch;
   size_t ev_next = 0, ev_next_prefetch = 0;
   bool in_prefetch = false;
@@ -132,6 +134,8 @@
   size_t seg_off[3] = {0, 0, 0};
   size_t jobs_off[3] = {0, 0, 0};
   int njobs[3] = {0, 0, 0};
+  std::vector<int> job_blk0[3];
+  int njobs_fwd[3] = {0, 0, 0};
   struct ProfRec {
     int cat; double flops, bytes; hipEvent_t a, b; std::string name;
     double mfma_scale = 1.0;
@@ -173,6 +177,9 @@
 int plan_init_workspace(Plan* P, float* ws, hipStream_t s);
 int plan_pack_pwc(Plan* P, const float* w_pwc, float* ws, hipStream_t s);
 int plan_pack_trainable(Plan* P, const float* w_gen, const float* w_rec, float* ws, hipStream_t s);
+int plan_pack_trainable_deferred(Plan* P, const float* w_gen, const float* w_rec, float* ws, hipStream_t s);
+void plan_pack_join(Plan* P, hipStream_t s);
+void plan_pack_job_table(const Plan* P, int net, std::vector<PackJob>& jobs, int* n_fwd);
 int plan_pwc_forward(Plan* P, const float* img1, const float* img2, float* ws, hipStream_t s);
 int plan_forward(Plan* P, const float* img1, const float* img2, int ncalls, float* ws, hipStream_t s, bool prefetched = false);
 int plan_prefetch(Plan* P, const float* img1, const float* img2, float* ws, hipStream_t s);
diff --git a/unsupervised_detection_amd/csrc/plan_build.hip b/unsupervised_detection_amd/csrc/plan_build.hip
--- a/unsupervised_detection_amd/csrc/plan_build.hip
+++ b/unsupervised_detection_amd/csrc/plan_build.hip
@@ -167,6 +167,8 @@
   for (auto& e : ev_pool) (void)hipEventDestroy(e);
   for (auto& e : ev_pool_prefetch) (void)hipEventDestroy(e);
   if (prefetch_ev) (void)hipEventDestroy(prefetch_ev);
+  if (pack_ev) (void)hipEventDestroy(pack_ev);
+  if (pack_fork_ev) (void)hipEventDestroy(pack_fork_ev);
   for (auto* r : prof) delete r;
   for (auto& ev : grad_ev)
     if (ev) (void)hipEventDestroy(ev);
diff --git a/unsupervised_detection_amd/csrc/plan_pack.hip b/unsupervised_detection_amd/csrc/plan_pack.hip
--- a/unsupervised_detection_amd/csrc/plan_pack.hip
+++ b/unsupervised_detection_amd/csrc/plan_pack.hip
@@ -20,6 +20,61 @@
   }
 }
 
+static bool gen_forward_mode(int mode) { return mode == 0 || mode == 3 || mode == 5 || mode == 7 || mode == 2; }
+void plan_pack_job_table(const Plan* P, int net, std::vector<PackJob>& jobs, int* n_fwd) {
+  const NetParams& np = net_params(net);
+  const std::vector<Layer>& layers = net == NET_GEN ? P->gen : P->rec;
+  jobs.clear();
+  for (const auto& L : layers) {
+    const int T = L.kh * L.kw;
+    const long goff = L.g_idx >= 0 ? (long)np.p[L.g_idx].offset : -1, beoff = L.be_idx >= 0 ? (long)np.p[L.be_idx].offset : -1;
+    PackJob j;
+    memset(&j, 0, sizeof(j));
+    j.src_off = (long)np.p[L.w_idx].offset; j.gamma_off = goff; j.beta_off = beoff;
+    j.T = T;
+    j.dst_off = (long)L.wp_off; j.R = L.cin; j.C = L.cout; j.Kc = L.Kc; j.ldw = L.ldw; j.k_split = L.k_split; j.k_gap = L.k_gap;
+    j.mode = 0; j.total = (long)T * L.Kc * L.ldw;
+    jobs.push_back(j);
+    j.dst_off = (long)L.wpT_off; j.Kc = L.KcT; j.ldw = L.ldwT; j.k_split = L.KcT; j.k_gap = 0;
+    j.mode = 1; j.total = (long)T * L.KcT * L.ldwT;
+    jobs.push_back(j);
+    if (L.col2im) {
+      j.dst_off = (long)L.wz_off; j.R = L.cin; j.C = L.cout; j.Kc = L.Kc; j.ldw = L.ldz; j.k_split = L.k_split; j.k_gap = L.k_gap;
+      j.mode = 3; j.total = (long)L.Kc * L.ldz;
+      jobs.push_back(j);
+    }
+    if (L.up) {
+      j.T = 16;
+      j.dst_off = (long)L.wu_off; j.R = L.cin; j.C = L.cout; j.Kc = L.Kc; j.ldw = L.ldw; j.k_split = L.Kc; j.k_gap = 0;
+      j.mode = 5; j.total = (long)16 * L.Kc * L.ldw;
+      jobs.push_back(j);
+      j.dst_off = (long)L.wuT_off; j.Kc = L.KcT; j.ldw = L.ldwT; j.k_split = L.KcT; j.k_gap = 0;
+      j.mode = 6; j.total = (long)16 * L.KcT * L.ldwT;
+      jobs.push_back(j);
+      j.T = T;
+    }
+    if (L.upb) upb_pack_jobs(L, j, jobs);
+    if (L.wino_off) {
+      j.dst_off = (long)L.wino_off; j.R = L.cin; j.C = L.cout; j.Kc = L.Kc; j.ldw = L.wino_np; j.k_split = L.k_split; j.k_gap = L.k_gap;
+      j.mode = 7; j.total = (long)(L.Kc / 8) * 2 * L.wino_np;
+      jobs.push_back(j);
+    }
+    if (L.winoT_off) {
+      j.dst_off = (long)L.winoT_off; j.R = L.cin; j.C = L.cout; j.Kc = L.KcT; j.ldw = L.winoT_np; j.k_split = L.KcT; j.k_gap = 0;
+      j.mode = 8; j.total = (long)(L.KcT / 8) * 2 * L.winoT_np;
+      jobs.push_back(j);
+    }
+    j.src_off = (long)np.p[L.b_idx].offset; j.dst_off = (long)L.bias_f_off; j.mode = 2; j.total = L.cout;
+    jobs.push_back(j);
+  }
+  std::vector<PackJob> a, b;
+  for (const auto& j : jobs) (net == NET_GEN && gen_forward_mode(j.mode) ? a : b).push_back(j);
+  *n_fwd = (int)a.size();
+  jobs = a;
+  jobs.insert(jobs.end(), b.begin(), b.end());
+  (void)pack_jobs_assign_blocks(jobs.data(), (int)jobs.size());
+}
+
 int plan_init_workspace(Plan* P, float* ws, hipStream_t s) {
   UDET_HIP(hipMemsetAsync(ws, 0, P->arena_floats * sizeof(float), s));
   for (int net = 1; net <= 2; ++net) {
@@ -33,57 +88,18 @@
     UDET_HIP(hipStreamSynchronize(s));
   }
   for (int net = 1; net <= 2; ++net) {
-    const NetParams& np = net_params(net);
     const std::vector<Layer>& layers = net == NET_GEN ? P->gen : P->rec;
     std::vector<PackJob> jobs;
-    for (const auto& L : layers) {
-      const int T = L.kh * L.kw;
-      const long goff = L.g_idx >= 0 ? (long)np.p[L.g_idx].offset : -1, beoff = L.be_idx >= 0 ? (long)np.p[L.be_idx].offset : -1;
-      PackJob j;
-      memset(&j, 0, sizeof(j));
-      j.src_off = (long)np.p[L.w_idx].offset; j.gamma_off = goff; j.beta_off = beoff;
-      j.T = T;
-      j.dst_off = (long)L.wp_off; j.R = L.cin; j.C = L.cout; j.Kc = L.Kc; j.ldw = L.ldw; j.k_split = L.k_split; j.k_gap = L.k_gap;
-      j.mode = 0; j.total = (long)T * L.Kc * L.ldw;
-      jobs.push_back(j);
-      j.dst_off = (long)L.wpT_off; j.Kc = L.KcT; j.ldw = L.ldwT; j.k_split = L.KcT; j.k_gap = 0;
-      j.mode = 1; j.total = (long)T * L.KcT * L.ldwT;
-      jobs.push_back(j);
-      if (L.col2im) {
-        j.dst_off = (long)L.wz_off; j.R = L.cin; j.C = L.cout; j.Kc = L.Kc; j.ldw = L.ldz; j.k_split = L.k_split; j.k_gap = L.k_gap;
-        j.mode = 3; j.total = (long)L.Kc * L.ldz;
-        jobs.push_back(j);
-      }
-      if (L.up) {
-        j.T = 16;
-        j.dst_off = (long)L.wu_off; j.R = L.cin; j.C = L.cout; j.Kc = L.Kc; j.ldw = L.ldw; j.k_split = L.Kc; j.k_gap = 0;
-        j.mode = 5; j.total = (long)16 * L.Kc * L.ldw;
-        jobs.push_back(j);
-        j.dst_off = (long)L.wuT_off; j.Kc = L.KcT; j.ldw = L.ldwT; j.k_split = L.KcT; j.k_gap = 0;
-        j.mode = 6; j.total = (long)16 * L.KcT * L.ldwT;
-        jobs.push_back(j);
-        j.T = T;
-      }
-      if (L.upb) upb_pack_jobs(L, j, jobs);
-      if (L.wino_off) {
-        j.dst_off = (long)L.wino_off; j.R = L.cin; j.C = L.cout; j.Kc = L.Kc; j.ldw = L.wino_np; j.k_split = L.k_split; j.k_gap = L.k_gap;
-        j.mode = 7; j.total = (long)(L.Kc / 8) * 2 * L.wino_np;
-        jobs.push_back(j);
-      }
-      if (L.winoT_off) {
-        j.dst_off = (long)L.winoT_off; j.R = L.cin; j.C = L.cout; j.Kc = L.KcT; j.ldw = L.winoT_np; j.k_split = L.KcT; j.k_gap = 0;
-        j.mode = 8; j.total = (long)(L.KcT / 8) * 2 * L.winoT_np;
-        jobs.push_back(j);
-      }
-      j.src_off = (long)np.p[L.b_idx].offset; j.dst_off = (long)L.bias_f_off; j.mode = 2; j.total = L.cout;
-      jobs.push_back(j);
-    }
+    plan_pack_job_table(P, net, jobs, &P->njobs_fwd[net]);
     if (jobs.size() > UDET_PACKJOB_CAP(layers.size())) {
       set_error("plan_init: %zu weight re-layout jobs for %zu layers exceed the table's %zu entries", jobs.size(), layers.size(),
                 (size_t)UDET_PACKJOB_CAP(layers.size()));
       return UDET_ERR_ARG;
     }
     P->njobs[net] = (int)jobs.size();
+    P->job_blk0[net].clear();
+    for (const auto& j : jobs) P->job_blk0[net].push_back(j.blk0);
+    P->job_blk0[net].push_back(jobs.empty() ? 0 : jobs.back().blk0 + jobs.back().nblk);
     UDET_HIP(hipMemcpyAsync(ws + P->jobs_off[net], jobs.data(), jobs.size() * sizeof(PackJob), hipMemcpyHostToDevice, s));
     UDET_HIP(hipStreamSynchronize(s));
   }
@@ -114,7 +130,14 @@
   return UDET_OK;
 }
 
+void plan_pack_join(Plan* P, hipStream_t s) {
+  if (!P->pack_pending) return;
+  (void)hipStreamWaitEvent(s, P->pack_ev, 0);
+  P->pack_pending = false;
+}
+
 int plan_pack_pwc(Plan* P, const float* w, float* ws, hipStream_t s) {
+  plan_pack_join(P, s);
   const NetParams& np = net_params(NET_PWC);
   for (const auto& L : P->pwc) {
     UDET_TRY(pack_layer(L, w, ws, nullptr, false, s));
@@ -124,11 +147,38 @@
   return UDET_OK;
 }
 
+static int pack_range(Plan* P, int net, int a, int b, const float* w, float* ws, hipStream_t s) {
+  if (b <= a) return UDET_OK;
+  const PackJob* jobs = reinterpret_cast<const PackJob*>(ws + P->jobs_off[net]);
+  return launch_pack_jobs(jobs + a, b - a, w, ws, BN_C, s, P->job_blk0[net][b] - P->job_blk0[net][a]);
+}
+
 int plan_pack_trainable(Plan* P, const float* w_gen, const float* w_rec, float* ws, hipStream_t s) {
-  if (w_gen)
-    UDET_TRY(launch_pack_jobs(reinterpret_cast<const PackJob*>(ws + P->jobs_off[NET_GEN]), P->njobs[NET_GEN], w_gen, ws, BN_C, s));
-  if (w_rec)
-    UDET_TRY(launch_pack_jobs(reinterpret_cast<const PackJob*>(ws + P->jobs_off[NET_REC]), P->njobs[NET_REC], w_rec, ws, BN_C, s));
+  plan_pack_join(P, s);
+  if (w_gen) UDET_TRY(pack_range(P, NET_GEN, 0, P->njobs[NET_GEN], w_gen, ws, s));
+  if (w_rec) UDET_TRY(pack_range(P, NET_REC, 0, P->njobs[NET_REC], w_rec, ws, s));
+  return UDET_OK;
+}
+
+int plan_pack_trainable_deferred(Plan* P, const float* w_gen, const float* w_rec, float* ws, hipStream_t s) {
+  plan_pack_join(P, s);
+  const Lane LB = lane_of(P, s, 3);
+  if (LB.s != s) {
+    if (!P->pack_fork_ev) UDET_HIP(hipEventCreateWithFlags(&P->pack_fork_ev, hipEventDisableTiming));
+    UDET_HIP(hipEventRecord(P->pack_fork_ev, s));
+    UDET_HIP(hipStreamWaitEvent(LB.s, P->pack_fork_ev, 0));
+  }
+  const int na = P->njobs_fwd[NET_GEN];
+  if (w_gen) {
+    UDET_TRY(pack_range(P, NET_GEN, 0, na, w_gen, ws, s));
+    UDET_TRY(pack_range(P, NET_GEN, na, P->njobs[NET_GEN], w_gen, ws, LB.s));
+  }
+  if (w_rec) UDET_TRY(pack_range(P, NET_REC, 0, P->njobs[NET_REC], w_rec, ws, LB.s));
+  if (LB.s != s) {
+    if (!P->pack_ev) UDET_HIP(hipEventCreateWithFlags(&P->pack_ev, hipEventDisableTiming));
+    UDET_HIP(hipEventRecord(P->pack_ev, LB.s));
+    P->pack_pending = true;
+  }
   return UDET_OK;
 }
 
diff --git a/unsupervised_detection_amd/csrc/plan_step.hip b/unsupervised_detection_amd/csrc/plan_step.hip
--- a/unsupervised_detection_amd/csrc/plan_step.hip
+++ b/unsupervised_detection_amd/csrc/plan_step.hip
@@ -181,9 +181,7 @@
   (void)hipStreamWaitEvent(s, P->prefetch_ev, 0);
   P->prefetch_pending = false;
   const Buf &fn = P->buf(P->R.flow_next), &in = P->buf(P->R.image_next);
-  UDET_HIP(hipMemcpyAsync(ws + P->buf(P->R.flow).off, ws + fn.off, fn.floats() * sizeof(float), hipMemcpyDeviceToDevice, s));
-  UDET_HIP(hipMemcpyAsync(ws + P->buf(P->R.image).off, ws + in.off, in.floats() * sizeof(float), hipMemcpyDeviceToDevice, s));
-  return UDET_OK;
+  return launch_copy2(ws + P->buf(P->R.flow).off, ws + fn.off, (long)fn.floats(), ws + P->buf(P->R.image).off, ws + in.off, (long)in.floats(), s);
 }
 
 int plan_forward(Plan* P, const float* img1, const float* img2, int ncalls, float* ws, hipStream_t s, bool prefetched) {
@@ -203,6 +201,7 @@
     (void)hipEventRecord(e_img, LI.s);
   }
   const bool paired = pairs_on(P);
+  if (P->pack_pending && !paired && ncalls >= 1) (void)hipStreamWaitEvent(LI.s, P->pack_ev, 0);
   UDET_TRY(plan_rec_image_branch(P, ncalls, ws, LI, !paired));
   if (img1) {
     UDET_TRY(pwc_forward_on(P, img1, img2, ws, L0, lane_of(P, s, 2)));
@@ -211,6 +210,7 @@
   if (e_img) (void)hipStreamWaitEvent(s, e_img, 0);
   UDET_TRY(plan_generator_forward(P, ws, s));
   order_after(P, LI, L0);
+  plan_pack_join(P, s);
   UDET_TRY(plan_recover_forward(P, ncalls, ws, s, false, !paired, paired));
   if (ncalls == 3) UDET_TRY(plan_losses(P, ws, s));
   return UDET_OK;
diff --git a/unsupervised_detection_amd/engine.py b/unsupervised_detection_amd/engine.py
--- a/unsupervised_detection_amd/engine.py
+++ b/unsupervised_detection_amd/engine.py
@@ -51,6 +51,10 @@
     getattr(lib, _n).restype = c_i
     getattr(lib, _n).argtypes = _a
 
+_HAS_DEFERRED_PACK = hasattr(lib, "udet_pack_trainable_deferred")
+if _HAS_DEFERRED_PACK:
+    lib.udet_pack_trainable_deferred.restype = c_i
+    lib.udet_pack_trainable_deferred.argtypes = [c_p, c_p, c_p, c_p, c_p]
 lib.udet_autotune.restype = c_i
 lib.udet_autotune.argtypes = [c_p] * 7
 lib.udet_tuned_shapes.restype = c_i
@@ -138,6 +142,11 @@
     def pack_trainable(self, w_gen=None, w_rec=None):
         check(lib.udet_pack_trainable(self._h, _ptr(w_gen), _ptr(w_rec), self.ws.data_ptr(), self._stream()))
 
+    def pack_trainable_deferred(self, w_gen=None, w_rec=None):
+        if not _HAS_DEFERRED_PACK:
+            return self.pack_trainable(w_gen, w_rec)
+        check(lib.udet_pack_trainable_deferred(self._h, _ptr(w_gen), _ptr(w_rec), self.ws.data_ptr(), self._stream()))
+
     def _check_pair(self, img1, img2):
         c = self.cfg
         want = (c.batch_size, c.in_height, c.in_width, 3)
diff --git a/unsupervised_detection_amd/trainer.py b/unsupervised_detection_amd/trainer.py
--- a/unsupervised_detection_amd/trainer.py
+++ b/unsupervised_detection_amd/trainer.py
@@ -57,10 +57,11 @@
         return n
 
 
-def flush_weights(st: TrainState):
+def flush_weights(st: TrainState, deferred: bool = False):
     dirty = getattr(st, "_dirty", 0)
     if dirty:
-        st.engine.pack_trainable(st.w_gen if dirty & GEN else None, st.w_rec if dirty & REC else None)
+        pack = st.engine.pack_trainable_deferred if deferred else st.engine.pack_trainable
+        pack(st.w_gen if dirty & GEN else None, st.w_rec if dirty & REC else None)
     st._dirty = 0
 
 
@@ -120,7 +121,7 @@
 
 def train_step(st: TrainState, img1, img2, which: int = BOTH, group=None, next_pair=None):
     e = st.engine
-    flush_weights(st)
+    flush_weights(st, deferred=True)
 
     def call(fn, *a):
         if not getattr(e.cfg, "conv_fp16", False):
```
